# saihv/coloc

Hardware: AMD Instinct MI355X
Metric: Mmatches/s (512-bit Hamming comparisons) at 10k kp/img, describe+match step (higher is better)
Workload: dtype fp4 (+-1) x fp4 -> f32 accumulate, exact integers (matrix pipe); fp32 sample coords

## Files before the change

### coloc_amd/abi.py

```python
import ctypes as C
import os

import numpy as np

_PKG = os.path.dirname(os.path.abspath(__file__))

KP_DTYPE = np.dtype(
    {"names": ["x", "y", "score", "angle", "scale"],
     "formats": ["<i4", "<i4", "u1", "<f4", "u1"],
     "offsets": [0, 4, 8, 12, 16], "itemsize": 20})

CLC_OK, CLC_ERR_BAD_ARG, CLC_ERR_CAPACITY, CLC_ERR_HIP, CLC_ERR_NO_DEVICE, CLC_ERR_STATE = range(6)


class CLCError(RuntimeError):
    def __init__(self, status, msg):
        super().__init__("coloc_hip status %d: %s" % (status, msg))
        self.status = status


class DetectorOptions(C.Structure):
    _fields_ = [("scale_factor", C.c_float), ("scale_levels", C.c_uint8), ("width", C.c_uint32),
                ("height", C.c_uint32), ("maxkp", C.c_uint32), ("thresh", C.c_uint8)]


class MatcherOptions(C.Structure):
    _fields_ = [("distRatio", C.c_float), ("thresh", C.c_int), ("maxkp", C.c_uint32)]


class McShare(C.Structure):
    _fields_ = [("first", C.c_int32), ("second", C.c_int32), ("q_begin", C.c_uint32), ("nq", C.c_uint32), ("out_offset", C.c_uint32)]


class MatchJob(C.Structure):
    _fields_ = [("q_offset", C.c_uint32), ("nq", C.c_uint32), ("t_offset", C.c_uint32), ("nt", C.c_uint32),
                ("out_offset", C.c_uint32), ("threshold", C.c_uint32)]


class PoseJob(C.Structure):
    _fields_ = [("X", C.c_void_p), ("x", C.c_void_p), ("K", C.c_void_p), ("n", C.c_int), ("max_iteration", C.c_int), ("seed", C.c_uint64),
                ("precision", C.c_double), ("refine", C.c_int), ("huber_a", C.c_double),
                ("Rt", C.c_void_p), ("cov", C.c_void_p), ("inlier_mask", C.c_void_p), ("inliers", C.c_void_p),
                ("n_inliers", C.c_int), ("iterations", C.c_int), ("status", C.c_int), ("error_max", C.c_double), ("rmse", C.c_double)]


class CameraK3(C.Structure):
    _fields_ = [("focal", C.c_double), ("ppx", C.c_double), ("ppy", C.c_double), ("k1", C.c_double), ("k2", C.c_double), ("k3", C.c_double)]


class TrackJob(C.Structure):
    _fields_ = [("d_match", C.c_void_p), ("nq", C.c_int), ("d_count", C.c_void_p), ("d_kps", C.c_void_p), ("d_feat", C.c_void_p),
                ("feat_stride", C.c_int), ("cam", CameraK3), ("after_stream", C.c_void_p), ("max_iteration", C.c_int), ("seed", C.c_uint64),
                ("precision", C.c_double), ("refine", C.c_int), ("huber_a", C.c_double),
                ("Rt", C.c_void_p), ("cov", C.c_void_p), ("track_query", C.c_void_p), ("track_map", C.c_void_p), ("inliers", C.c_void_p),
                ("inlier_mask", C.c_void_p), ("n_tracks", C.c_int), ("n_inliers", C.c_int), ("iterations", C.c_int), ("status", C.c_int),
                ("error_max", C.c_double), ("rmse", C.c_double)]


class PairJob(C.Structure):
    _fields_ = [("d_match", C.c_void_p), ("nq", C.c_int), ("nt", C.c_int), ("d_count_a", C.c_void_p), ("d_count_b", C.c_void_p),
                ("d_kps_a", C.c_void_p), ("d_feat_a", C.c_void_p), ("feat_stride_a", C.c_int),
                ("d_kps_b", C.c_void_p), ("d_feat_b", C.c_void_p), ("feat_stride_b", C.c_int),
                ("cam_a", CameraK3), ("cam_b", CameraK3), ("after_stream", C.c_void_p),
                ("img_w", C.c_int), ("img_h", C.c_int), ("max_iteration", C.c_int), ("seed", C.c_uint64), ("precision", C.c_double),
                ("M", C.c_void_p), ("F", C.c_void_p), ("pair_q", C.c_void_p), ("pair_t", C.c_void_p), ("x1", C.c_void_p), ("x2", C.c_void_p),
                ("inliers", C.c_void_p), ("inlier_mask", C.c_void_p),
                ("n_pairs", C.c_int), ("n_inliers", C.c_int), ("iterations", C.c_int), ("status", C.c_int),
                ("error_max", C.c_double), ("min_nfa", C.c_double)]


ABI_VERSION = 4
DESC_CACHE_OFF, DESC_CACHE_VERIFY, DESC_CACHE_TRUST = 0, 1, 2

class DescHandle(C.Structure):
    _fields_ = [("host", C.c_void_p), ("generation", C.c_uint64), ("count", C.c_uint32), ("slot", C.c_uint32)]


class TwoViewJob(C.Structure):
    _fields_ = [("x1", C.c_void_p), ("x2", C.c_void_p), ("K1", C.c_void_p), ("K2", C.c_void_p), ("n", C.c_int), ("img_w", C.c_int), ("img_h", C.c_int),
                ("max_iteration", C.c_int), ("seed", C.c_uint64), ("precision", C.c_double),
                ("E", C.c_void_p), ("F", C.c_void_p), ("inlier_mask", C.c_void_p), ("inliers", C.c_void_p),
                ("n_inliers", C.c_int), ("iterations", C.c_int), ("status", C.c_int), ("error_max", C.c_double), ("min_nfa", C.c_double)]


class InterPoseJob(C.Structure):
    _fields_ = [("tv", TwoViewJob), ("map_index", C.c_void_p), ("map_X", C.c_void_p), ("map_n", C.c_int), ("Rt_source", C.c_void_p), ("huber_a", C.c_double),
                ("d_first_desc", C.c_void_p), ("first_feature", C.c_void_p), ("d_map_desc", C.c_void_p), ("match_threshold", C.c_int),
                ("Rt", C.c_double * 12), ("cov", C.c_double * 36), ("rmse", C.c_double), ("scale", C.c_double),
                ("n_front", C.c_int), ("n_common", C.c_int), ("n_refined", C.c_int), ("stage", C.c_int), ("n_map_matches", C.c_int)]


EXPORTS = [
    "clc_abi_version", "clc_status_string", "clc_ctx_create", "clc_ctx_destroy", "clc_last_error_string",
    "clc_sync", "clc_stream", "clc_pyramid_build", "clc_pyramid_build_dev", "clc_pyramid_level",
    "clc_pyramid_download", "clc_describe", "clc_describe_dev", "clc_keypoints_to_features",
    "clc_match_2nn", "clc_match_2nn_dev", "clc_match_jobs_dev", "clc_set_map", "clc_match_map",
    "clc_pnp_residuals", "clc_pnp_score", "clc_profile_enable", "clc_profile_reset", "clc_profile_read",
    "clc_kernel_name", "clc_detect", "clc_detect_dev", "clc_detect_buffers", "clc_describe_detected_dev",
    "clc_detect_and_describe", "clc_detect_batch_dev", "clc_desc_cache_publish", "clc_desc_cache_clear", "clc_desc_cache_stats", "clc_desc_cache_mode", "clc_desc_handle_live", "clc_detect_and_describe_view", "clc_detect_store_descriptors", "clc_describe_match_pair_dev", "clc_essential_acransac_batch", "clc_inter_pose_batch", "clc_pnp_localize_ac_batch", "clc_match_pairs", "clc_pnp_ransac", "clc_pnp_p3p", "clc_pnp_refine", "clc_pnp_localize", "clc_epipolar_residuals", "clc_epipolar_score", "clc_cov_intersection", "clc_essential_ransac",
    "clc_essential_fivepoint", "clc_describe_batch_dev", "clc_match_map_dev", "clc_k2nn_set_formulation",
    "clc_k2nn_queries_per_block", "clc_k2nn_plan_query", "clc_k2nn_device_info", "clc_pnp_acransac", "clc_pnp_localize_ac", "clc_essential_acransac", "clc_k2nn_clock_check", "clc_ctx_device", "clc_mc_plan", "clc_mc_unique_id",
    "clc_mc_create", "clc_mc_destroy", "clc_mc_last_error_string", "clc_mc_arena", "clc_mc_gather_dev", "clc_mc_match_dev", "clc_mc_virtual_put", "clc_mc_open_peers",
    "clc_mc_gather_enqueue_dev", "clc_mc_match_enqueue_dev", "clc_mc_counts", "clc_mc_set_overlap", "clc_mc_comm_info", "clc_match_jobs_counted_dev",
    "clc_two_view_acransac", "clc_two_view_acransac_batch", "clc_two_view_minimal",
    "clc_match_ratio_2nn", "clc_match_ratio_2nn_dev", "clc_match_ratio_pairs", "clc_match_map_ratio", "clc_match_map_ratio_dev",
    "clc_ratio_matches_to_pairs", "clc_detect_set_selection", "clc_detect_selection",
    "clc_set_map_points", "clc_track_build_dev", "clc_track_localize_dev", "clc_track_localize_batch_dev",
    "clc_pair_build_dev", "clc_pair_filter_dev", "clc_pair_filter_batch_dev",
]
SELECT_FIRST, SELECT_STRONGEST = 0, 1
KERNELS = ["pyramid_kernel", "clatch_kernel", "k2nn_sweep_kernel", "k2nn_merge_kernel", "pnp_residual_kernel",
           "pnp_score_kernel", "detect_kernels"]

_lib = None


def lib_path():
    return os.environ.get("COLOC_HIP_LIB", os.path.join(_PKG, "lib", "libcoloc_hip.so"))


def _share_torch_hip_runtime():
    if os.environ.get("COLOC_HIP_SYSTEM_RUNTIME"):
        return
    import importlib.util
    try:
        spec = importlib.util.find_spec("torch")
    except (ImportError, ValueError):
        spec = None
    if spec is None or not spec.origin:
        return
    cand = os.path.join(os.path.dirname(spec.origin), "lib", "libamdhip64.so")
    if os.path.exists(cand):
        try:
            C.CDLL(cand, mode=C.RTLD_GLOBAL)
        except OSError:
            pass


def load_library():
    global _lib
    if _lib is not None:
        return _lib
    path = lib_path()
    if not os.path.exists(path):
        raise CLCError(-1, "%s not found: build it with `python -c 'import __graft_entry__ as g; g.build()'` "
                           "(hipcc --offload-arch=gfx950); there is no CPU fallback" % path)
    _share_torch_hip_runtime()
    lib = C.CDLL(path)
    got = lib.clc_abi_version() if hasattr(lib, "clc_abi_version") else 0
    if got != ABI_VERSION:
        raise CLCError(-1, "%s reports ABI version %d, this binding needs %d: rebuild it (python -c 'import __graft_entry__ as g; g.build()')"
                       % (path, got, ABI_VERSION))
    lib.clc_status_string.restype = C.c_char_p
    lib.clc_last_error_string.restype = C.c_char_p
    lib.clc_last_error_string.argtypes = [C.c_void_p]
    lib.clc_stream.restype = C.c_void_p
    lib.clc_stream.argtypes = [C.c_void_p]
    lib.clc_ctx_create.argtypes = [C.c_int, C.c_void_p, C.c_void_p, C.POINTER(C.c_void_p)]
    lib.clc_ctx_destroy.argtypes = [C.c_void_p]
    lib.clc_sync.argtypes = [C.c_void_p]
    vp, ci, u32, sz = C.c_void_p, C.c_int, C.c_uint32, C.c_size_t
    lib.clc_pyramid_build.argtypes = [vp, vp, u32, u32]
    lib.clc_pyramid_build_dev.argtypes = [vp, vp, u32, u32, sz, vp]
    lib.clc_pyramid_level.argtypes = [vp, ci, C.POINTER(u32), C.POINTER(u32), C.POINTER(sz), C.POINTER(vp)]
    lib.clc_pyramid_download.argtypes = [vp, ci, vp]
    lib.clc_describe.argtypes = [vp, vp, ci, vp]
    lib.clc_describe_dev.argtypes = [vp, vp, ci, vp, vp]
    lib.clc_describe_batch_dev.argtypes = [vp, ci, vp, C.c_uint32, C.c_uint32, C.c_size_t, vp, vp, vp, vp]
    lib.clc_detect_batch_dev.argtypes = [vp, ci, vp, C.c_uint32, C.c_uint32, C.c_size_t, vp, vp, vp, vp]
    lib.clc_desc_cache_publish.argtypes = [vp, vp, vp, ci, vp]
    lib.clc_desc_handle_live.argtypes = [vp]
    lib.clc_detect_and_describe_view.argtypes = [vp, vp, u32, u32, C.POINTER(vp), C.POINTER(vp), C.POINTER(ci), C.POINTER(ci)]
    lib.clc_detect_store_descriptors.argtypes = [vp, vp, ci, vp]
    lib.clc_desc_cache_clear.argtypes = []
    lib.clc_desc_cache_stats.argtypes = [vp, vp]
    lib.clc_desc_cache_mode.argtypes = [vp, ci]
    lib.clc_essential_acransac_batch.argtypes = [vp, vp, ci]
    lib.clc_inter_pose_batch.argtypes = [vp, vp, ci]
    lib.clc_describe_match_pair_dev.argtypes = [vp, vp, C.c_uint32, C.c_uint32, C.c_size_t, vp, vp, vp, ci, vp, vp]
    lib.clc_pnp_localize_ac_batch.argtypes = [vp, vp, ci]
    lib.clc_keypoints_to_features.argtypes = [vp, ci, vp]
    lib.clc_match_2nn.argtypes = [vp, vp, ci, vp, ci, ci, vp, vp, vp]
    lib.clc_match_2nn_dev.argtypes = [vp, vp, ci, vp, ci, ci, vp, vp]
    lib.clc_match_jobs_dev.argtypes = [vp, vp, vp, ci, vp, vp]
    lib.clc_match_pairs.argtypes = [vp, vp, vp, ci, vp, ci, ci, vp]
    lib.clc_set_map.argtypes = [vp, vp, ci]
    lib.clc_match_map_dev.argtypes = [vp, vp, ci, ci, vp, vp]
    lib.clc_match_map.argtypes = [vp, vp, ci, ci, vp]
    cf = C.c_float
    lib.clc_match_ratio_2nn.argtypes = [vp, vp, ci, vp, ci, cf, vp, vp, vp]
    lib.clc_match_ratio_2nn_dev.argtypes = [vp, vp, ci, vp, ci, cf, vp, vp]
    lib.clc_match_ratio_pairs.argtypes = [vp, vp, vp, ci, vp, vp, ci, cf, vp, vp]
    lib.clc_match_map_ratio.argtypes = [vp, vp, ci, vp, vp, cf, vp, vp]
    lib.clc_match_map_ratio_dev.argtypes = [vp, vp, ci, cf, vp, vp]
    lib.clc_ratio_matches_to_pairs.argtypes = [vp, ci, vp, vp, vp, vp]
    lib.clc_pnp_residuals.argtypes = [vp, vp, ci, vp, vp, ci, vp, vp]
    lib.clc_pnp_score.argtypes = [vp, vp, ci, vp, vp, ci, vp, C.c_double, vp, vp]
    lib.clc_detect.argtypes = [vp, vp, ci, C.POINTER(ci), C.POINTER(ci)]
    lib.clc_detect_dev.argtypes = [vp, vp]
    lib.clc_detect_set_selection.argtypes = [vp, ci]
    lib.clc_detect_selection.argtypes = [vp]
    lib.clc_detect_buffers.argtypes = [vp, C.POINTER(vp), C.POINTER(vp), C.POINTER(vp)]
    lib.clc_describe_detected_dev.argtypes = [vp, vp, vp]
    lib.clc_detect_and_describe.argtypes = [vp, vp, u32, u32, vp, vp, ci, C.POINTER(ci), C.POINTER(ci)]
    lib.clc_pnp_ransac.argtypes = [vp, vp, vp, ci, vp, vp, ci, C.c_uint64, C.c_double, vp, vp, C.POINTER(ci), C.POINTER(C.c_double)]
    lib.clc_pnp_p3p.argtypes = [vp, vp, vp, ci, vp, vp, ci, vp]
    lib.clc_essential_ransac.argtypes = [vp, vp, vp, ci, vp, vp, vp, ci, C.c_uint64, C.c_double, vp, vp, vp, C.POINTER(ci)]
    lib.clc_essential_fivepoint.argtypes = [vp, vp, vp, ci, vp, vp, vp, ci, vp]
    lib.clc_epipolar_residuals.argtypes = [vp, vp, ci, vp, vp, ci, vp]
    lib.clc_epipolar_score.argtypes = [vp, vp, ci, vp, vp, ci, C.c_double, vp, vp]
    lib.clc_pnp_localize.argtypes = [vp, vp, vp, ci, vp, vp, ci, C.c_uint64, C.c_double, C.c_double, vp, vp, vp, C.POINTER(ci),
                                     C.POINTER(C.c_double)]
    lib.clc_pnp_refine.argtypes = [vp, vp, vp, ci, vp, vp, vp, C.c_double, ci, vp, vp, C.POINTER(C.c_double), C.POINTER(ci)]
    lib.clc_profile_enable.argtypes = [vp, ci]
    lib.clc_profile_reset.argtypes = [vp]
    lib.clc_profile_read.argtypes = [vp, ci, C.POINTER(C.c_double), C.POINTER(ci)]
    lib.clc_kernel_name.restype = C.c_char_p
    dp, ip = C.POINTER(C.c_double), C.POINTER(ci)
    lib.clc_pnp_acransac.argtypes = [vp, vp, vp, ci, vp, ci, C.c_uint64, C.c_double, vp, vp, vp, ip, dp, dp, ip]
    lib.clc_pnp_localize_ac.argtypes = [vp, vp, vp, ci, vp, ci, C.c_uint64, C.c_double, C.c_double, vp, vp, vp, vp, ip, dp, dp]
    lib.clc_essential_acransac.argtypes = [vp, vp, vp, ci, vp, vp, ci, ci, ci, C.c_uint64, C.c_double, vp, vp, vp, vp, ip, dp, dp, ip]
    lib.clc_two_view_acransac.argtypes = [vp, ci, vp, vp, ci, vp, vp, ci, ci, ci, C.c_uint64, C.c_double, vp, vp, vp, vp, ip, dp, dp, ip]
    lib.clc_two_view_acransac_batch.argtypes = [vp, ci, vp, ci]
    lib.clc_two_view_minimal.argtypes = [vp, ci, vp, vp, ci, ci, ci, vp, ci, vp]
    lib.clc_mc_plan.argtypes = [vp, ci, ci, ci, ci, vp, ci, ip]
    lib.clc_mc_unique_id.argtypes = [vp]
    lib.clc_mc_create.argtypes = [vp, vp, ci, ci, ci, C.POINTER(vp)]
    lib.clc_mc_destroy.argtypes = [vp]
    lib.clc_mc_last_error_string.argtypes = [vp]
    lib.clc_mc_last_error_string.restype = C.c_char_p
    lib.clc_mc_arena.argtypes = [vp, C.POINTER(vp), ip, ip]
    lib.clc_mc_gather_dev.argtypes = [vp, vp, ci, ci, vp, vp]
    lib.clc_mc_virtual_put.argtypes = [vp, ci, vp, ci, vp]
    lib.clc_mc_open_peers.argtypes = [vp, vp]
    lib.clc_mc_match_dev.argtypes = [vp, ci, vp, ci, vp, ci, ip, vp]
    lib.clc_mc_gather_enqueue_dev.argtypes = [vp, vp, ci, vp, ci, vp]
    lib.clc_mc_match_enqueue_dev.argtypes = [vp, ci, vp, ci, vp, ci, ip, vp]
    lib.clc_mc_counts.argtypes = [vp, vp, vp]
    lib.clc_mc_set_overlap.argtypes = [vp, ci]
    lib.clc_mc_comm_info.argtypes = [vp, ip, ip]
    lib.clc_match_jobs_counted_dev.argtypes = [vp, vp, vp, ci, vp, vp, vp, vp, vp]
    lib.clc_k2nn_clock_check.argtypes = [vp, vp, ci, vp, ci, vp, vp, dp, dp, dp, ip]
    lib.clc_k2nn_set_formulation.argtypes = [vp, ci]
    lib.clc_k2nn_queries_per_block.argtypes = [vp]
    lib.clc_k2nn_plan_query.argtypes = [vp, ci, ci, vp]
    lib.clc_k2nn_device_info.argtypes = [vp, vp, vp]
    lib.clc_set_map_points.argtypes = [vp, vp, ci]
    lib.clc_track_build_dev.argtypes = [vp, vp, vp, vp, vp, vp, vp, vp]
    lib.clc_track_localize_dev.argtypes = [vp, vp]
    lib.clc_track_localize_batch_dev.argtypes = [vp, vp, ci]
    lib.clc_pair_build_dev.argtypes = [vp, vp, vp, vp, vp, vp, vp, vp]
    lib.clc_pair_filter_dev.argtypes = [vp, ci, vp]
    lib.clc_pair_filter_batch_dev.argtypes = [vp, ci, vp, ci]
    _lib = lib
    return lib


def _p(a):
    return None if a is None else C.c_void_p(a.ctypes.data)


def cov_intersection(CA, CB, ca, cb):
    lib = load_library()
    CA = np.ascontiguousarray(CA, dtype=np.float64).reshape(9); CB = np.ascontiguousarray(CB, dtype=np.float64).reshape(9)
    ca = np.ascontiguousarray(ca, dtype=np.float64).reshape(3); cb = np.ascontiguousarray(cb, dtype=np.float64).reshape(3)
    om = C.c_double(); cov = np.zeros(9); pos = np.zeros(3)
    lib.clc_cov_intersection.argtypes = [C.c_void_p] * 4 + [C.POINTER(C.c_double), C.c_void_p, C.c_void_p]
    rc = lib.clc_cov_intersection(_p(CA), _p(CB), _p(ca), _p(cb), C.byref(om), _p(cov), _p(pos))
    if rc != CLC_OK:
        raise CLCError(rc, lib.clc_status_string(rc).decode())
    return om.value, cov.reshape(3, 3), pos


def _xy(xy, n):
    if xy is None:
        return None
    xy = np.ascontiguousarray(xy, dtype=np.float32).reshape(-1, 2)
    if xy.shape[0] != n:
        raise ValueError("positions: %d rows for a set of %d descriptors" % (xy.shape[0], n))
    return xy


def ratio_matches_to_pairs(match, xy_db=None, xy_q=None):
    lib = load_library()
    match = np.ascontiguousarray(match, dtype=np.int32).reshape(-1)
    if xy_db is not None:
        xy_db = np.ascontiguousarray(xy_db, dtype=np.float32).reshape(-1, 2)
    xy_q = _xy(xy_q, match.shape[0])
    out = np.empty((max(match.shape[0], 1), 2), dtype=np.int32)
    n = C.c_int(0)
    rc = lib.clc_ratio_matches_to_pairs(_p(match), match.shape[0], _p(xy_db), _p(xy_q), _p(out), C.byref(n))
    if rc != CLC_OK:
        raise CLCError(rc, "clc_ratio_matches_to_pairs: " + lib.clc_status_string(rc).decode())
    return out[:n.value].copy()


def _two_view_fill(tv, keep, x1, x2, K1, K2, img_wh, max_iteration, seed, precision):
    x1 = np.ascontiguousarray(x1, dtype=np.float64).reshape(-1, 2); x2 = np.ascontiguousarray(x2, dtype=np.float64).reshape(-1, 2)
    K1 = np.ascontiguousarray(K1, dtype=np.float64).reshape(9); K2 = np.ascontiguousarray(K2, dtype=np.float64).reshape(9)
    n = x1.shape[0]
    E, F = np.zeros(9), np.zeros(9)
    mask, inl = np.zeros(max(n, 1), dtype=np.uint8), np.zeros(max(n, 1), dtype=np.int32)
    keep.append((x1, x2, K1, K2, E, F, mask, inl))
    tv.x1, tv.x2, tv.K1, tv.K2, tv.n = x1.ctypes.data, x2.ctypes.data, K1.ctypes.data, K2.ctypes.data, n
    tv.img_w, tv.img_h, tv.max_iteration, tv.seed, tv.precision = int(img_wh[0]), int(img_wh[1]), int(max_iteration), int(seed), float(precision)
    tv.E, tv.F, tv.inlier_mask, tv.inliers = E.ctypes.data, F.ctypes.data, mask.ctypes.data, inl.ctypes.data
    return E, F, mask, inl


def _two_view_result(tv, E, F, mask, inl):
    ok = tv.n_inliers > 0
    return dict(E=E.reshape(3, 3).copy() if ok else None, F=F.reshape(3, 3).copy() if ok else None, mask=mask[:tv.n].astype(bool),
                inliers=inl[:tv.n_inliers].copy(), error_max=tv.error_max, min_nfa=tv.min_nfa, iterations=tv.iterations, status=tv.status)


def essential_acransac_batch(ctxs, problems, max_iteration=256, precision=float("inf")):
    lib = load_library()
    n = len(problems)
    jobs = (TwoViewJob * n)()
    keep, outs = [], []
    for j, (x1, x2, K1, K2, wh, seed) in zip(jobs, problems):
        outs.append(_two_view_fill(j, keep, x1, x2, K1, K2, wh, max_iteration, seed, precision))
    hs = (C.c_void_p * n)(*[c.h for c in ctxs])
    rc = lib.clc_essential_acransac_batch(hs, jobs, n)
    if rc != CLC_OK:
        raise CLCError(rc, lib.clc_status_string(rc).decode())
    return [_two_view_result(j, *o) for j, o in zip(jobs, outs)]


def two_view_acransac_batch(ctxs, model, problems, max_iteration=256, precision=float("inf")):
    lib = load_library()
    n = len(problems)
    jobs = (TwoViewJob * n)()
    keep, outs = [], []
    for j, (x1, x2, K1, K2, wh, seed) in zip(jobs, problems):
        outs.append(_two_view_fill(j, keep, x1, x2, np.eye(3) if K1 is None else K1, np.eye(3) if K2 is None else K2, wh, max_iteration, seed, precision))
    hs = (C.c_void_p * n)(*[c.h for c in ctxs])
    rc = lib.clc_two_view_acransac_batch(hs, ord(model), jobs, n)
    if rc != CLC_OK:
        raise CLCError(rc, lib.clc_status_string(rc).decode())
    return [_two_view_result(j, *o) for j, o in zip(jobs, outs)]


def inter_pose_batch(ctxs, problems, map_X, max_iteration=256, huber_a=16.0):
    lib = load_library()
    n = len(problems)
    jobs = (InterPoseJob * n)()
    map_X = np.ascontiguousarray(map_X, dtype=np.float64).reshape(-1, 3)
    keep, outs = [map_X], []
    for j, p in zip(jobs, problems):
        outs.append(_two_view_fill(j.tv, keep, p["x1"], p["x2"], p["K"], p["K"], p["wh"], max_iteration, p["seed"], float("inf")))
        rs = np.ascontiguousarray(p["Rt_source"], dtype=np.float64).reshape(12)
        keep.append(rs)
        j.map_X, j.map_n, j.Rt_source, j.huber_a = map_X.ctypes.data, int(map_X.shape[0]), rs.ctypes.data, float(huber_a)
        if p.get("d_first_desc") is not None:
            ff = np.ascontiguousarray(p["first_feature"], dtype=np.int32)
            keep.append(ff)
            j.d_first_desc, j.first_feature, j.d_map_desc = int(p["d_first_desc"]), ff.ctypes.data, int(p["d_map_desc"])
            j.match_threshold = int(p.get("match_threshold", 60))
        elif p.get("map_index") is not None:
            mi = np.ascontiguousarray(p["map_index"], dtype=np.int32)
            keep.append(mi)
            j.map_index = mi.ctypes.data
    hs = (C.c_void_p * n)(*[c.h for c in ctxs])
    rc = lib.clc_inter_pose_batch(hs, jobs, n)
    if rc != CLC_OK:
        raise CLCError(rc, lib.clc_status_string(rc).decode())
    res = []
    for j, o in zip(jobs, outs):
        d = _two_view_result(j.tv, *o)
        d.update(Rt=np.array(j.Rt).reshape(3, 4), cov=np.array(j.cov).reshape(6, 6), rmse=j.rmse, scale=j.scale, n_front=j.n_front,
                 n_common=j.n_common, n_refined=j.n_refined, stage=j.stage, n_map_matches=j.n_map_matches)
        res.append(d)
    return res


def mc_plan(counts, world, rank, grain):
    lib = load_library()
    cnt = (C.c_int * len(counts))(*[int(c) for c in counts])
    cap = len(counts) * len(counts) + 2
    out = (McShare * cap)()
    n = C.c_int()
    rc = lib.clc_mc_plan(cnt, len(counts), int(world), int(rank), int(grain), out, cap, C.byref(n))
    if rc != CLC_OK:
        raise CLCError(rc, lib.clc_status_string(rc).decode())
    return [(s.first, s.second, s.q_begin, s.nq, s.out_offset) for s in out[:n.value]]


class MultiCam:

    def __init__(self, ctx, world=1, rank=0, maxkp=10000, unique_id=None):
        self.lib, self.ctx = load_library(), ctx
        h = C.c_void_p()
        idbuf = (C.c_uint8 * 128)(*unique_id) if unique_id is not None else None
        rc = self.lib.clc_mc_create(ctx.h, idbuf, world, rank, maxkp, C.byref(h))
        if rc != CLC_OK:
            raise CLCError(rc, "clc_mc_create: " + self.lib.clc_status_string(rc).decode())
        self.h, self.world, self.maxkp = h, world, maxkp
# ... 46 lines not shown

    def set_overlap(self, on=True):
        self._chk(self.lib.clc_mc_set_overlap(self.h, 1 if on else 0))

    def comm_info(self):
        n, r = C.c_int(), C.c_int()
        self._chk(self.lib.clc_mc_comm_info(self.h, C.byref(n), C.byref(r)))
        return int(n.value), int(r.value)

    def counts(self, stream=None):
        cnt = (C.c_int * self.world)()
        self._chk(self.lib.clc_mc_counts(self.h, cnt, stream))
        return [int(c) for c in cnt]

    def close(self):
        if getattr(self, "h", None):
            self.lib.clc_mc_destroy(self.h)
            self.h = None


def pnp_localize_batch(ctxs, problems, max_iteration=256, seeds=None, precision=float("inf"), refine=True, huber_a=16.0):
    lib = load_library()
    n = len(problems)
    assert len(ctxs) == n
    jobs = (PoseJob * n)()
    keep = []
    for i, (X, x, K) in enumerate(problems):
        X = np.ascontiguousarray(X, dtype=np.float64); x = np.ascontiguousarray(x, dtype=np.float64)
        K = np.ascontiguousarray(K, dtype=np.float64).reshape(9)
        N = X.shape[0]
        Rt, cov = np.zeros(12), np.zeros(36)
        mask, inl = np.zeros(max(N, 1), dtype=np.uint8), np.zeros(max(N, 1), dtype=np.int32)
        keep.append((X, x, K, Rt, cov, mask, inl))
        j = jobs[i]
        j.X, j.x, j.K, j.n = X.ctypes.data, x.ctypes.data, K.ctypes.data, N
        j.max_iteration, j.seed, j.precision = int(max_iteration), int(seeds[i] if seeds is not None else 1), float(precision)
        j.refine, j.huber_a = (1 if refine else 0), float(huber_a)
        j.Rt, j.cov, j.inlier_mask, j.inliers = Rt.ctypes.data, cov.ctypes.data, mask.ctypes.data, inl.ctypes.data
    hs = (C.c_void_p * n)(*[c.h for c in ctxs])
    rc = lib.clc_pnp_localize_ac_batch(hs, jobs, n)
    if rc != CLC_OK:
        raise CLCError(rc, "clc_pnp_localize_ac_batch: " + lib.clc_status_string(rc).decode())
    out = []
    for i in range(n):
        X, x, K, Rt, cov, mask, inl = keep[i]
        j = jobs[i]
        found = j.n_inliers > 0
        out.append(dict(Rt=Rt.reshape(3, 4) if found else None, cov=cov.reshape(6, 6) if (found and refine) else None,
                        mask=mask[:X.shape[0]].astype(bool), inliers=inl[:j.n_inliers].copy(), error_max=j.error_max, rmse=j.rmse,
                        iterations=j.iterations))
    return out


def _track_fill(j, keep, d_match, nq, cam, d_kps=None, d_feat=None, feat_stride=4, d_count=None, after_stream=None, max_iteration=256,
                seed=1, precision=float("inf"), refine=True, huber_a=16.0, outputs=True):
    j.d_match, j.nq, j.d_count, j.d_kps, j.d_feat, j.feat_stride = d_match, int(nq), d_count, d_kps, d_feat, int(feat_stride)
    j.cam = CameraK3(*[float(v) for v in cam])
    j.after_stream = after_stream
    j.max_iteration, j.seed, j.precision, j.refine, j.huber_a = int(max_iteration), int(seed), float(precision), (1 if refine else 0), float(huber_a)
    if not outputs:
        return None
    n = max(int(nq), 1)
    Rt, cov = np.zeros(12), np.zeros(36)
    tq, tm, inl, mask = np.zeros(n, dtype=np.int32), np.zeros(n, dtype=np.int32), np.zeros(n, dtype=np.int32), np.zeros(n, dtype=np.uint8)
    keep.append((Rt, cov, tq, tm, inl, mask))
    j.Rt, j.cov, j.track_query, j.track_map, j.inliers, j.inlier_mask = (a.ctypes.data for a in (Rt, cov, tq, tm, inl, mask))
    return Rt, cov, tq, tm, inl, mask


def _track_result(j, Rt, cov, tq, tm, inl, mask):
    found = j.n_inliers > 0
    nt = max(min(j.n_tracks, len(tq)), 0)
    return dict(Rt=Rt.reshape(3, 4).copy() if found else None, cov=cov.reshape(6, 6).copy() if (found and j.refine) else None,
                n_tracks=j.n_tracks, track_query=tq[:nt].copy(), track_map=tm[:nt].copy(), inliers=inl[:j.n_inliers].copy(),
                mask=mask[:nt].astype(bool), error_max=j.error_max, rmse=j.rmse, iterations=j.iterations, status=j.status)


def track_localize_batch_dev(ctxs, jobs):
    lib = load_library()
    n = len(jobs)
    assert len(ctxs) == n
    arr = (TrackJob * n)()
    keep = []
    outs = [_track_fill(arr[i], keep, **jobs[i]) for i in range(n)]
    hs = (C.c_void_p * n)(*[c.h for c in ctxs])
    rc = lib.clc_track_localize_batch_dev(hs, arr, n)
    if rc != CLC_OK:
        raise CLCError(rc, "clc_track_localize_batch_dev: %s: %s" % (lib.clc_status_string(rc).decode(), lib.clc_last_error_string(ctxs[0].h).decode()))
    return [_track_result(arr[i], *outs[i]) for i in range(n)]


def _pair_fill(j, keep, d_match, nq, nt, cam_a, cam_b, d_kps_a=None, d_feat_a=None, feat_stride_a=4, d_kps_b=None, d_feat_b=None,
               feat_stride_b=4, d_count_a=None, d_count_b=None, after_stream=None, img_wh=(0, 0), max_iteration=256, seed=1,
               precision=float("inf"), outputs=True):
    j.d_match, j.nq, j.nt, j.d_count_a, j.d_count_b = d_match, int(nq), int(nt), d_count_a, d_count_b
    j.d_kps_a, j.d_feat_a, j.feat_stride_a = d_kps_a, d_feat_a, int(feat_stride_a)
    j.d_kps_b, j.d_feat_b, j.feat_stride_b = d_kps_b, d_feat_b, int(feat_stride_b)
    j.cam_a, j.cam_b = CameraK3(*[float(v) for v in cam_a]), CameraK3(*[float(v) for v in cam_b])
    j.after_stream = after_stream
    j.img_w, j.img_h, j.max_iteration, j.seed, j.precision = int(img_wh[0]), int(img_wh[1]), int(max_iteration), int(seed), float(precision)
    if not outputs:
        return None
    n = max(int(nq), 1)
    M, F, x1, x2 = np.zeros(9), np.zeros(9), np.zeros((n, 2)), np.zeros((n, 2))
    pq, pt, inl, mask = np.zeros(n, dtype=np.int32), np.zeros(n, dtype=np.int32), np.zeros(n, dtype=np.int32), np.zeros(n, dtype=np.uint8)
    keep.append((M, F, pq, pt, x1, x2, inl, mask))
    j.M, j.F, j.pair_q, j.pair_t, j.x1, j.x2, j.inliers, j.inlier_mask = (a.ctypes.data for a in (M, F, pq, pt, x1, x2, inl, mask))
    return M, F, pq, pt, x1, x2, inl, mask


def _pair_result(j, M, F, pq, pt, x1, x2, inl, mask):
    found = j.n_inliers > 0
    n = max(min(j.n_pairs, len(pq)), 0)
    return dict(M=M.reshape(3, 3).copy() if found else None, F=F.reshape(3, 3).copy() if found else None, n_pairs=j.n_pairs,
                pair_q=pq[:n].copy(), pair_t=pt[:n].copy(), x1=x1[:n].copy(), x2=x2[:n].copy(), inliers=inl[:j.n_inliers].copy(),
                mask=mask[:n].astype(bool), error_max=j.error_max, min_nfa=j.min_nfa, iterations=j.iterations, status=j.status)


def pair_filter_batch_dev(ctxs, model, jobs):
    lib = load_library()
    n = len(jobs)
    assert len(ctxs) == n
    arr = (PairJob * n)()
    keep = []
    outs = [_pair_fill(arr[i], keep, **jobs[i]) for i in range(n)]
    hs = (C.c_void_p * n)(*[c.h for c in ctxs])
    rc = lib.clc_pair_filter_batch_dev(hs, ord(model), arr, n)
    if rc != CLC_OK:
        raise CLCError(rc, "clc_pair_filter_batch_dev: %s: %s" % (lib.clc_status_string(rc).decode(), lib.clc_last_error_string(ctxs[0].h).decode()))
    return [_pair_result(arr[i], *outs[i]) for i in range(n)]


def desc_handle_live(handle):
    return bool(load_library().clc_desc_handle_live(C.byref(handle)))


def desc_cache_stats():
    lib = load_library()
    h, m = C.c_ulonglong(), C.c_ulonglong()
    lib.clc_desc_cache_stats(C.byref(h), C.byref(m))
    return int(h.value), int(m.value)


def keypoints_to_features(kps):
    lib = load_library()
    kps = np.ascontiguousarray(kps, dtype=KP_DTYPE)
    out = np.zeros((len(kps), 4), dtype=np.float32)
    rc = lib.clc_keypoints_to_features(_p(kps), len(kps), _p(out))
    if rc != CLC_OK:
        raise CLCError(rc, lib.clc_status_string(rc).decode())
    return out


class Context:

    def __init__(self, device=0, width=640, height=480, maxkp=10000, scale_factor=1.2, scale_levels=8,
                 fast_thresh=40, match_thresh=60, detector=True, matcher=True):
        self.lib = load_library()
        self.dopts = DetectorOptions(scale_factor, scale_levels, width, height, maxkp, fast_thresh)
        self.mopts = MatcherOptions(0.8, match_thresh, maxkp)
        h = C.c_void_p()
        rc = self.lib.clc_ctx_create(device, C.byref(self.dopts) if detector else None,
                                     C.byref(self.mopts) if matcher else None, C.byref(h))
        if rc != CLC_OK:
            raise CLCError(rc, "clc_ctx_create: " + self.lib.clc_status_string(rc).decode())
        self.h = h
        self.device = device

    def _chk(self, rc):
        if rc != CLC_OK:
            raise CLCError(rc, "%s: %s" % (self.lib.clc_status_string(rc).decode(),
                                           self.lib.clc_last_error_string(self.h).decode()))

    def close(self):
        if getattr(self, "h", None):
            self.lib.clc_ctx_destroy(self.h)
            self.h = None

    def __del__(self):
        try:
            self.close()
        except Exception:
            pass

    def sync(self):
        self._chk(self.lib.clc_sync(self.h))

    @property
    def stream(self):
        return self.lib.clc_stream(self.h)

    def profile_enable(self, on=True, only=None):
        v = 1 if on else 0
        if on and only:
            v = 0
            for name in only:
                v |= 1 << (KERNELS.index(name) + 1)
        self._chk(self.lib.clc_profile_enable(self.h, v))

    def profile_reset(self):
        self._chk(self.lib.clc_profile_reset(self.h))

    def profile_read(self):
        out = {}
        for k, name in enumerate(KERNELS):
            ms, cnt = C.c_double(), C.c_int()
            self._chk(self.lib.clc_profile_read(self.h, k, C.byref(ms), C.byref(cnt)))
            out[name] = (ms.value, cnt.value)
        return out

    def pyramid_build(self, img):
        img = np.ascontiguousarray(img, dtype=np.uint8)
        self._chk(self.lib.clc_pyramid_build(self.h, _p(img), img.shape[1], img.shape[0]))

    def pyramid_build_dev(self, d_ptr, width, height, pitch, stream=None):
        self._chk(self.lib.clc_pyramid_build_dev(self.h, d_ptr, width, height, pitch, stream))

    def pyramid_level(self, level):
        w, h, p, d = C.c_uint32(), C.c_uint32(), C.c_size_t(), C.c_void_p()
        self._chk(self.lib.clc_pyramid_level(self.h, level, C.byref(w), C.byref(h), C.byref(p), C.byref(d)))
        return w.value, h.value, p.value, d.value

    def pyramid_download(self, level):
        w, h, _, _ = self.pyramid_level(level)
        out = np.zeros((h, w), dtype=np.uint8)
        self._chk(self.lib.clc_pyramid_download(self.h, level, _p(out)))
        return out

    def detect(self, capacity=None):
        cap = int(capacity if capacity is not None else self.dopts.maxkp)
        kps = np.zeros(cap, dtype=KP_DTYPE)
        n, found = C.c_int(), C.c_int()
        self._chk(self.lib.clc_detect(self.h, _p(kps), cap, C.byref(n), C.byref(found)))
        return kps[:n.value], found.value

    def set_keypoint_selection(self, mode):
        self._chk(self.lib.clc_detect_set_selection(self.h, int(mode)))

    @property
    def keypoint_selection(self):
        return self.lib.clc_detect_selection(self.h)

    def detect_dev(self, stream=None):
        self._chk(self.lib.clc_detect_dev(self.h, stream))

    def detect_buffers(self):
        k, c, d = C.c_void_p(), C.c_void_p(), C.c_void_p()
        self._chk(self.lib.clc_detect_buffers(self.h, C.byref(k), C.byref(c), C.byref(d)))
        return k.value, c.value, d.value

    def describe_detected_dev(self, d_desc=None, stream=None):
        self._chk(self.lib.clc_describe_detected_dev(self.h, d_desc, stream))

    def detect_and_describe(self, img, capacity=None):
        img = np.ascontiguousarray(img, dtype=np.uint8)
        cap = int(capacity if capacity is not None else self.dopts.maxkp)
        kps = np.zeros(cap, dtype=KP_DTYPE)
        desc = np.zeros((cap, 64), dtype=np.uint8)
        n, found = C.c_int(), C.c_int()
        self._chk(self.lib.clc_detect_and_describe(self.h, _p(img), img.shape[1], img.shape[0], _p(kps), _p(desc), cap,
                                                   C.byref(n), C.byref(found)))
        return kps[:n.value], desc[:n.value], found.value

    def detect_and_describe_published(self, img):
        img = np.ascontiguousarray(img, dtype=np.uint8)
        pk, pd, n, found = C.c_void_p(), C.c_void_p(), C.c_int(), C.c_int()
        self._chk(self.lib.clc_detect_and_describe_view(self.h, _p(img), img.shape[1], img.shape[0], C.byref(pk), C.byref(pd), C.byref(n), C.byref(found)))
        kps = np.zeros(n.value, dtype=KP_DTYPE)
        if n.value:
            C.memmove(_p(kps), pk, n.value * 20)
        desc = np.zeros((n.value, 64), dtype=np.uint8)
        handle = DescHandle()
        self._chk(self.lib.clc_detect_store_descriptors(self.h, _p(desc) if n.value else None, n.value, C.byref(handle)))
        return kps, desc, found.value, handle

    def detect_batch_dev(self, d_imgs, width, height, pitch, d_kps, d_counts, d_desc=None, stream=None):
        n = len(d_imgs)
        imgs = (C.c_void_p * n)(*d_imgs)
        kps = (C.c_void_p * n)(*d_kps)
        cnt = (C.c_void_p * n)(*d_counts)
        out = (C.c_void_p * n)(*d_desc) if d_desc is not None else None
        self._chk(self.lib.clc_detect_batch_dev(self.h, n, imgs, width, height, pitch, kps, cnt, out, stream))

    def describe_match_pair_dev(self, d_imgs, width, height, pitch, d_kps, counts, d_desc, threshold, d_match, stream=None):
        imgs = (C.c_void_p * 2)(*d_imgs)
        kps = (C.c_void_p * 2)(*d_kps)
        cnt = (C.c_int * 2)(*[int(c) for c in counts])
        out = (C.c_void_p * 2)(*d_desc)
        self._chk(self.lib.clc_describe_match_pair_dev(self.h, imgs, width, height, pitch, kps, cnt, out, int(threshold), d_match, stream))

    def desc_cache_mode(self, mode):
        self._chk(self.lib.clc_desc_cache_mode(self.h, {"off": DESC_CACHE_OFF, "verify": DESC_CACHE_VERIFY, "trust": DESC_CACHE_TRUST}[mode]))

    def desc_cache_publish(self, h_desc, d_src=None):
        assert h_desc.dtype == np.uint8 and h_desc.flags["C_CONTIGUOUS"]
        handle = DescHandle()
        self._chk(self.lib.clc_desc_cache_publish(self.h, d_src, _p(h_desc), int(h_desc.shape[0]), C.byref(handle)))
        return handle

    def describe(self, kps):
        kps = np.ascontiguousarray(kps, dtype=KP_DTYPE)
        desc = np.zeros((len(kps), 64), dtype=np.uint8)
        self._chk(self.lib.clc_describe(self.h, _p(kps), len(kps), _p(desc)))
        return desc

    def describe_dev(self, d_kps, n, d_desc, stream=None):
        self._chk(self.lib.clc_describe_dev(self.h, d_kps, n, d_desc, stream))

    def describe_batch_dev(self, d_imgs, width, height, pitch, d_kps, counts, d_desc, stream=None):
        n = len(d_imgs)
        imgs = (C.c_void_p * n)(*d_imgs)
        kps = (C.c_void_p * n)(*d_kps)
        cnt = (C.c_int * n)(*counts)
        out = (C.c_void_p * n)(*d_desc)
        self._chk(self.lib.clc_describe_batch_dev(self.h, n, imgs, width, height, pitch, kps, cnt, out, stream))

    def set_k2nn_formulation(self, name):
        self._chk(self.lib.clc_k2nn_set_formulation(self.h, {"matrix": 0, "popcount": 1}[name]))

    @property
    def k2nn_queries_per_block(self):
        return int(self.lib.clc_k2nn_queries_per_block(self.h))

    def k2nn_device_info(self):
        info = (C.c_int32 * 8)()
        us = (C.c_float * 4)()
        self._chk(self.lib.clc_k2nn_device_info(self.h, info, us))
        d = dict(zip(("xcds", "cus", "default_target_blocks", "bias_a", "bias_b", "bias_source", "kernel_xcds", "target_blocks_env"), [int(v) for v in info]))
        d["bias_source"] = ("default", "CLC_K2NN_BIAS", "probe")[d["bias_source"]]
        d["probe_us"] = dict(zip(("295:264", "311:256", "326:249", "326:233"), [float(v) for v in us]))
        return d

    def k2nn_plan_query(self, nq, nt):
        info = (C.c_int32 * 8)()
        self._chk(self.lib.clc_k2nn_plan_query(self.h, int(nq), int(nt), info))
        return dict(zip(("qblocks", "splits", "t_per_split", "atomic_merge", "bias_a_tiles", "bias_b_tiles", "queries_per_block", "target_blocks"),
                        [int(v) for v in info]))

    def k2nn_clock_check(self, d_q, nq, d_t, nt, d_match, stream=None):
        med, lo, hi, n = C.c_double(), C.c_double(), C.c_double(), C.c_int()
        self._chk(self.lib.clc_k2nn_clock_check(self.h, d_q, nq, d_t, nt, d_match, stream, C.byref(med), C.byref(lo), C.byref(hi), C.byref(n)))
        return med.value, lo.value, hi.value, n.value

    def match_2nn(self, Q, T, threshold=40, want_dist=False):
        Q = np.ascontiguousarray(Q, dtype=np.uint8).reshape(-1, 64)
        T = np.ascontiguousarray(T, dtype=np.uint8).reshape(-1, 64)
        m = np.full(Q.shape[0], -2, dtype=np.int32)
        b = np.zeros(Q.shape[0], dtype=np.uint16) if want_dist else None
        s = np.zeros(Q.shape[0], dtype=np.uint16) if want_dist else None
        self._chk(self.lib.clc_match_2nn(self.h, _p(Q), Q.shape[0], _p(T), T.shape[0], int(threshold), _p(m), _p(b), _p(s)))
        return (m, b, s) if want_dist else m

    def match_2nn_dev(self, d_q, nq, d_t, nt, threshold, d_match, stream=None):
        self._chk(self.lib.clc_match_2nn_dev(self.h, d_q, nq, d_t, nt, int(threshold), d_match, stream))

    def match_jobs_dev(self, d_desc_base, jobs, d_match, stream=None):
        arr = (MatchJob * len(jobs))(*[MatchJob(*j) for j in jobs])
        self._chk(self.lib.clc_match_jobs_dev(self.h, d_desc_base, arr, len(jobs), d_match, stream))

    def match_jobs_counted_dev(self, d_desc_base, jobs, d_cnt_q, d_cnt_t, q_row0, d_match, stream=None):
        n = len(jobs)
        arr = (MatchJob * n)(*[MatchJob(*j) for j in jobs])
        cq = (C.c_void_p * n)(*d_cnt_q)
        ct = (C.c_void_p * n)(*d_cnt_t)
        r0 = (C.c_uint32 * n)(*q_row0)
        self._chk(self.lib.clc_match_jobs_counted_dev(self.h, d_desc_base, arr, n, cq, ct, r0, d_match, stream))

    def match_pairs(self, descs, pairs, threshold=40):
        descs = [np.ascontiguousarray(d, dtype=np.uint8).reshape(-1, 64) for d in descs]
        counts = (C.c_int * len(descs))(*[d.shape[0] for d in descs])
        dptr = (C.c_void_p * len(descs))(*[d.ctypes.data for d in descs])
        flat = (C.c_int * (2 * len(pairs)))(*[v for p in pairs for v in p])
        outs = [np.full(descs[a].shape[0], -2, dtype=np.int32) for a, _ in pairs]
        optr = (C.c_void_p * len(pairs))(*[o.ctypes.data for o in outs])
        self._chk(self.lib.clc_match_pairs(self.h, dptr, counts, len(descs), flat, len(pairs), int(threshold), optr))
        return outs

    def match_ratio(self, Q, T, ratio=0.8, want_dist=False):
        Q = np.ascontiguousarray(Q, dtype=np.uint8).reshape(-1, 64)
        T = np.ascontiguousarray(T, dtype=np.uint8).reshape(-1, 64)
        m = np.full(Q.shape[0], -2, dtype=np.int32)
        b = np.zeros(Q.shape[0], dtype=np.uint16) if want_dist else None
        s = np.zeros(Q.shape[0], dtype=np.uint16) if want_dist else None
        self._chk(self.lib.clc_match_ratio_2nn(self.h, _p(Q), Q.shape[0], _p(T), T.shape[0], float(ratio), _p(m), _p(b), _p(s)))
        return (m, b, s) if want_dist else m

    def match_ratio_dev(self, d_q, nq, d_t, nt, ratio, d_match, stream=None):
        self._chk(self.lib.clc_match_ratio_2nn_dev(self.h, d_q, nq, d_t, nt, float(ratio), d_match, stream))

    def match_ratio_pairs(self, descs, pairs, ratio=0.8, xys=None):
        descs = [np.ascontiguousarray(d, dtype=np.uint8).reshape(-1, 64) for d in descs]
        ncams = len(descs)
        counts = (C.c_int * ncams)(*[d.shape[0] for d in descs])
        dptr = (C.c_void_p * ncams)(*[d.ctypes.data for d in descs])
        xyp = None
        if xys is not None:
            xys = [_xy(x, d.shape[0]) for x, d in zip(xys, descs)]
            xyp = (C.c_void_p * ncams)(*[None if x is None else x.ctypes.data for x in xys])
        flat = (C.c_int * max(2 * len(pairs), 1))(*[v for p in pairs for v in p])
        outs = [np.empty((max(descs[b].shape[0] if 0 <= b < ncams else 0, 1), 2), dtype=np.int32) for _, b in pairs]
        optr = (C.c_void_p * max(len(pairs), 1))(*[o.ctypes.data for o in outs])
        n = (C.c_int * max(len(pairs), 1))()
        self._chk(self.lib.clc_match_ratio_pairs(self.h, dptr, counts, ncams, xyp, flat, len(pairs), float(ratio), optr, n))
        return [o[:n[p]].copy() for p, o in enumerate(outs)]

    def match_map_ratio(self, Q, ratio=0.8, xy_map=None, xy_q=None):
        Q = np.ascontiguousarray(Q, dtype=np.uint8).reshape(-1, 64)
        xy_map = None if xy_map is None else np.ascontiguousarray(xy_map, dtype=np.float32).reshape(-1, 2)
        xy_q = _xy(xy_q, Q.shape[0])
        out = np.empty((max(Q.shape[0], 1), 2), dtype=np.int32)
        n = C.c_int(0)
        self._chk(self.lib.clc_match_map_ratio(self.h, _p(Q), Q.shape[0], _p(xy_map), _p(xy_q), float(ratio), _p(out), C.byref(n)))
        return out[:n.value].copy()

    def match_map_ratio_dev(self, d_q, nq, ratio, d_match, stream=None):
        self._chk(self.lib.clc_match_map_ratio_dev(self.h, d_q, nq, float(ratio), d_match, stream))

    def set_map(self, desc):
        desc = np.ascontiguousarray(desc, dtype=np.uint8).reshape(-1, 64)
        self._chk(self.lib.clc_set_map(self.h, _p(desc), desc.shape[0]))

    def set_map_points(self, X):
        X = np.ascontiguousarray(X, dtype=np.float64).reshape(-1, 3)
        self._chk(self.lib.clc_set_map_points(self.h, _p(X) if X.shape[0] else None, X.shape[0]))

    def track_build_dev(self, d_X, d_x, d_query, d_map, d_n, stream=None, **job):
        j = TrackJob()
        _track_fill(j, None, outputs=False, **job)
        self._chk(self.lib.clc_track_build_dev(self.h, C.byref(j), d_X, d_x, d_query, d_map, d_n, stream))

    def track_localize_dev(self, **job):
        j = TrackJob()
        keep = []
        out = _track_fill(j, keep, **job)
        self._chk(self.lib.clc_track_localize_dev(self.h, C.byref(j)))
        return _track_result(j, *out)

    def pair_build_dev(self, d_x1, d_x2, d_pair_q, d_pair_t, d_n, stream=None, **job):
        j = PairJob()
        _pair_fill(j, None, outputs=False, **job)
        self._chk(self.lib.clc_pair_build_dev(self.h, C.byref(j), d_x1, d_x2, d_pair_q, d_pair_t, d_n, stream))

    def pair_filter_dev(self, model, **job):
        j = PairJob()
        keep = []
        out = _pair_fill(j, keep, **job)
        self._chk(self.lib.clc_pair_filter_dev(self.h, ord(model), C.byref(j)))
        return _pair_result(j, *out)

    def match_map_dev(self, d_q, nq, threshold, d_match, stream=None):
        self._chk(self.lib.clc_match_map_dev(self.h, d_q, nq, int(threshold), d_match, stream))

    def match_map(self, Q, threshold=60):
        Q = np.ascontiguousarray(Q, dtype=np.uint8).reshape(-1, 64)
        m = np.full(Q.shape[0], -2, dtype=np.int32)
        self._chk(self.lib.clc_match_map(self.h, _p(Q), Q.shape[0], int(threshold), _p(m)))
        return m

    def pnp_residuals(self, Rt, X, x, K):
        Rt = np.ascontiguousarray(Rt, dtype=np.float64).reshape(-1, 12)
        X = np.ascontiguousarray(X, dtype=np.float64).reshape(-1, 3)
        x = np.ascontiguousarray(x, dtype=np.float64).reshape(-1, 2)
        K = np.ascontiguousarray(K, dtype=np.float64).reshape(9)
        err = np.zeros((Rt.shape[0], X.shape[0]), dtype=np.float64)
        self._chk(self.lib.clc_pnp_residuals(self.h, _p(Rt), Rt.shape[0], _p(X), _p(x), X.shape[0], _p(K), _p(err)))
        return err

    def pnp_ransac(self, X, x, K, samples=None, n_samples=256, seed=1, thr2=16.0):
        X = np.ascontiguousarray(X, dtype=np.float64).reshape(-1, 3)
        x = np.ascontiguousarray(x, dtype=np.float64).reshape(-1, 2)
        K = np.ascontiguousarray(K, dtype=np.float64).reshape(9)
        if samples is not None:
            samples = np.ascontiguousarray(samples, dtype=np.int32).reshape(-1, 3)
            n_samples = samples.shape[0]
        Rt = np.zeros(12, dtype=np.float64)
        mask = np.zeros(X.shape[0], dtype=np.uint8)
        n, cost = C.c_int(), C.c_double()
        self._chk(self.lib.clc_pnp_ransac(self.h, _p(X), _p(x), X.shape[0], _p(K), _p(samples), int(n_samples), int(seed),
                                          float(thr2), _p(Rt), _p(mask), C.byref(n), C.byref(cost)))
        return (Rt.reshape(3, 4) if n.value > 0 else None), mask.astype(bool), cost.value

    def essential_ransac(self, x1, x2, K1, K2, samples=None, n_samples=256, seed=1, thr2=4.0):
        x1 = np.ascontiguousarray(x1, dtype=np.float64).reshape(-1, 2)
        x2 = np.ascontiguousarray(x2, dtype=np.float64).reshape(-1, 2)
        K1 = np.ascontiguousarray(K1, dtype=np.float64).reshape(9); K2 = np.ascontiguousarray(K2, dtype=np.float64).reshape(9)
        if samples is not None:
            samples = np.ascontiguousarray(samples, dtype=np.int32).reshape(-1, 5)
            n_samples = samples.shape[0]
        E = np.zeros(9); F = np.zeros(9)
        mask = np.zeros(x1.shape[0], dtype=np.uint8)
# ... 142 lines not shown
```

### coloc_amd/csrc/capi_core.hip

```cpp
#include "clc_ctx.h"
#include "desc_cache.h"

#include <chrono>
#include <cmath>
#include <cstdio>
#include <cstdlib>
#include <cstring>
#include <new>

using namespace clc;

namespace clc {
void prof_mark(Profiler* prof, int kernel, bool begin, hipStream_t stream)
{
    if (!prof || !prof->on || !((prof->mask >> kernel) & 1u)) return;
    if (begin) {
        Profiler::Pair p;
        p.a = prof->get(); p.b = prof->get(); p.kernel = kernel; p.stream = stream; p.open = true;
        if (p.a) (void)hipEventRecord(p.a, stream);
        prof->pending.push_back(p);
    } else {
        for (size_t i = prof->pending.size(); i-- > 0;) {
            Profiler::Pair& p = prof->pending[i];
            if (p.open && p.kernel == kernel && p.stream == stream) {
                if (p.b) (void)hipEventRecord(p.b, stream);
                p.open = false;
                break;
            }
        }
    }
}

int fail(clc_ctx* ctx, int code, const char* what, hipError_t e)
{
    if (ctx) {
        char buf[512];
        if (e != hipSuccess) snprintf(buf, sizeof buf, "%s: %s (%s)", what, hipGetErrorName(e), hipGetErrorString(e));
        else snprintf(buf, sizeof buf, "%s", what);
        ctx->err = buf;
        if (code == CLC_ERR_HIP) ctx->partial_dirty = true;
    }
    return code;
}


int ensure_partial(clc_ctx* ctx, size_t elems)
{
    if (elems <= ctx->partial_cap) return CLC_OK;
    CLC_HIP(ctx, hipStreamSynchronize(ctx->stream));
    if (ctx->d_partial) CLC_HIP(ctx, hipFree(ctx->d_partial));
    ctx->d_partial = nullptr;
    ctx->partial_cap = 0;
    size_t cap = elems + elems / 4;
    CLC_HIP(ctx, hipMalloc((void**)&ctx->d_partial, cap * sizeof(uint2)));
    CLC_HIP(ctx, hipMemsetAsync(ctx->d_partial, 0xFF, cap * sizeof(uint2), ctx->stream));
    CLC_HIP(ctx, hipStreamSynchronize(ctx->stream));
    ctx->partial_cap = cap;
    return CLC_OK;
}

int ensure_pnp(clc_ctx* ctx, size_t doubles)
{
    if (doubles <= ctx->pnp_cap) return CLC_OK;
    CLC_HIP(ctx, hipStreamSynchronize(ctx->stream));
    if (ctx->d_pnp) CLC_HIP(ctx, hipFree(ctx->d_pnp));
    ctx->d_pnp = nullptr;
    ctx->pnp_cap = 0;
    const size_t cap = doubles + doubles / 2;
    CLC_HIP(ctx, hipMalloc((void**)&ctx->d_pnp, cap * sizeof(double)));
    ctx->pnp_cap = cap;
    return CLC_OK;
}

int ensure_pinned(clc_ctx* ctx, size_t bytes)
{
    if (bytes <= ctx->pin_cap) return CLC_OK;
    CLC_HIP(ctx, hipStreamSynchronize(ctx->stream));
    if (ctx->h_pin) CLC_HIP(ctx, hipHostFree(ctx->h_pin));
    ctx->h_pin = nullptr; ctx->pin_cap = 0;
    const size_t cap = bytes + bytes / 2;
    CLC_HIP(ctx, hipHostMalloc(&ctx->h_pin, cap, hipHostMallocDefault));
    ctx->pin_cap = cap;
    return CLC_OK;
}

int ensure_slots(clc_ctx* ctx, int n, hipStream_t st)
{
    if (n <= ctx->arena_slots) return CLC_OK;
    CLC_HIP(ctx, hipStreamSynchronize(ctx->stream));
    if (st != ctx->stream) CLC_HIP(ctx, hipStreamSynchronize(st));
    uint8_t *arena = nullptr, *score = nullptr;
    uint64_t* kpmask = nullptr;
    uint32_t* tcount = nullptr;
    hipError_t e = hipMalloc((void**)&arena, ctx->arena_bytes * (size_t)n);
    if (e == hipSuccess) e = hipMalloc((void**)&score, ctx->arena_bytes * (size_t)n);
    if (e == hipSuccess) e = hipMalloc((void**)&kpmask, (size_t)n * ctx->n_tiles * 16 * sizeof(uint64_t));
    if (e == hipSuccess) e = hipMalloc((void**)&tcount, (size_t)n * ctx->n_tiles * sizeof(uint32_t));
    if (e == hipSuccess) e = hipMemsetAsync(arena, 0, ctx->arena_bytes * (size_t)n, st);
    if (e == hipSuccess) e = hipStreamSynchronize(st);
    if (e != hipSuccess) {
        (void)hipFree(arena); (void)hipFree(score); (void)hipFree(kpmask); (void)hipFree(tcount);
        return fail(ctx, CLC_ERR_HIP, "growing the pyramid arena", e);
    }
    ctx->pyramid_valid = false;
    ctx->detected = false;
    (void)hipFree(ctx->d_arena); (void)hipFree(ctx->d_score); (void)hipFree(ctx->d_kpmask); (void)hipFree(ctx->d_tcount);
    ctx->d_arena = arena; ctx->d_score = score; ctx->d_kpmask = kpmask; ctx->d_tcount = tcount;
    ctx->arena_slots = n;
    return CLC_OK;
}


int ensure_results(clc_ctx* ctx, size_t bytes)
{
    if (bytes <= ctx->res_cap) return CLC_OK;
    CLC_HIP(ctx, hipStreamSynchronize(ctx->stream));
    if (ctx->h_res) CLC_HIP(ctx, hipHostFree(ctx->h_res));
    ctx->h_res = nullptr; ctx->res_cap = 0;
    CLC_HIP(ctx, hipHostMalloc((void**)&ctx->h_res, bytes, hipHostMallocDefault));
    ctx->res_cap = bytes;
    return CLC_OK;
}

}

namespace {

uint32_t align_up(uint32_t v, uint32_t a) { return (v + a - 1) / a * a; }

void plan_pyramid(const clc_detector_opts& o, PyramidDesc& pd, size_t& bytes)
{
    pd.levels = o.scale_levels;
    float f = 1.0f;
    uint32_t off = 0, blk = 0;
    for (int i = 0; i < pd.levels; ++i) {
        if (i) f *= o.scale_factor;
        const uint32_t w = i ? (uint32_t)((float)o.width / f + 0.5f) : o.width;
        const uint32_t h = i ? (uint32_t)((float)o.height / f + 0.5f) : o.height;
        pd.f[i] = f;
        pd.lv[i].w = w;
        pd.lv[i].h = h;
        pd.lv[i].pitch = align_up(w ? w : 1, 64);
        pd.lv[i].offset = off;
        off += align_up(pd.lv[i].pitch * (h ? h : 1), 256);
        pd.blk_begin[i] = blk;
        if (i) blk += (pd.lv[i].pitch / 4 * h + 255) / 256;
    }
    for (int i = pd.levels; i <= CLC_MAX_LEVELS; ++i) pd.blk_begin[i] = blk;
    bytes = off + 256;
}

int cache_mode_default()
{
    const char* v = getenv("CLC_DESC_CACHE");
    if (!v || !v[0]) return CLC_DESC_CACHE_VERIFY;
    if (v[0] == '0' || v[0] == 'o' || v[0] == 'O') return CLC_DESC_CACHE_OFF;
    if (v[0] == 't' || v[0] == 'T' || v[0] == '2') return CLC_DESC_CACHE_TRUST;
    return CLC_DESC_CACHE_VERIFY;
}


__global__ __launch_bounds__(256) void frontend_mirror_kernel(const uint32_t* __restrict__ d_kps, const uint4* __restrict__ d_desc,
                                                              const uint32_t* __restrict__ d_count, uint32_t* __restrict__ h_kps,
                                                              uint4* __restrict__ h_desc, uint32_t* __restrict__ h_count)
{
    const uint32_t n = d_count[0];
    const uint32_t i = blockIdx.x * 256u + threadIdx.x;
    if (i == 0u) { h_count[0] = n; h_count[1] = d_count[1]; }
    if (i < n * 4u) h_desc[i] = d_desc[i];
    if (i < n * 4u) h_kps[i] = d_kps[i];
    if (i < n) h_kps[n * 4u + i] = d_kps[n * 4u + i];
}

static int ensure_stage(clc_ctx* ctx)
{
    if (ctx->h_stage) return CLC_OK;
    const size_t img = ((size_t)ctx->dopts.width * ctx->dopts.height + 255) & ~(size_t)255;
    const size_t kps = ((size_t)ctx->dopts.maxkp * sizeof(clc_keypoint) + 255) & ~(size_t)255;
    const size_t desc = (size_t)ctx->dopts.maxkp * CLC_DESC_BYTES;
    ctx->stage_img = 0; ctx->stage_kps = img; ctx->stage_desc = img + kps; ctx->stage_cnt = img + kps + desc;
    CLC_HIP(ctx, hipHostMalloc((void**)&ctx->h_stage, img + kps + desc + 256, hipHostMallocDefault));
    memset(ctx->h_stage + ctx->stage_cnt, 0, 256);
    return CLC_OK;
}

}

extern "C" {

int clc_abi_version(void) { return CLC_ABI_VERSION; }

const char* clc_status_string(int status)
{
    switch (status) {
        case CLC_OK: return "ok";
        case CLC_ERR_BAD_ARG: return "bad argument";
        case CLC_ERR_CAPACITY: return "capacity exceeded";
        case CLC_ERR_HIP: return "HIP runtime error";
        case CLC_ERR_NO_DEVICE: return "no usable device";
        case CLC_ERR_STATE: return "invalid call order";
        default: return "unknown status";
    }
}

const char* clc_last_error_string(const clc_ctx* ctx) { return ctx ? ctx->err.c_str() : "null context"; }

int clc_ctx_create(int device_id, const clc_detector_opts* dopts, const clc_matcher_opts* mopts, clc_ctx** out_ctx)
{
    if (!out_ctx) return CLC_ERR_BAD_ARG;
    *out_ctx = nullptr;
    if (dopts) {
        if (dopts->scale_levels < 1 || dopts->scale_levels > CLC_MAX_LEVELS || dopts->width < 8 || dopts->height < 8 ||
            !(dopts->scale_factor > 1.0f) || dopts->maxkp == 0)
            return CLC_ERR_BAD_ARG;
        if (dopts->width > CLC_DETECT_MAX_WIDTH) {
            fprintf(stderr, "coloc_hip: DetectorOptions.width %u exceeds CLC_DETECT_MAX_WIDTH %d (the GPU detector keeps a row's pre-test bits in LDS)\n",
                    dopts->width, CLC_DETECT_MAX_WIDTH);
            return CLC_ERR_CAPACITY;
        }
    }
    if (mopts && mopts->maxkp == 0) return CLC_ERR_BAD_ARG;
    int ndev = 0;
    if (hipGetDeviceCount(&ndev) != hipSuccess || device_id < 0 || device_id >= ndev) return CLC_ERR_NO_DEVICE;
    clc_ctx* ctx = new (std::nothrow) clc_ctx;
    if (!ctx) return CLC_ERR_HIP;
    ctx->device = device_id;
#define CREATE_HIP(call)                                     \
    do {                                                     \
        hipError_t e__ = (call);                             \
        if (e__ != hipSuccess) {                             \
            fprintf(stderr, "coloc_hip: %s failed: %s\n", #call, hipGetErrorString(e__)); \
            clc_ctx_destroy(ctx);                            \
            return CLC_ERR_HIP;                              \
        }                                                    \
    } while (0)
    CREATE_HIP(hipSetDevice(device_id));
    CREATE_HIP(hipStreamCreateWithFlags(&ctx->stream, hipStreamNonBlocking));
    {
        int v = 0;
        if (hipDeviceGetAttribute(&v, hipDeviceAttributeMultiprocessorCount, device_id) == hipSuccess && v > 0) ctx->k2dev.n_cu = (uint32_t)v;
        if (hipDeviceGetAttribute(&v, hipDeviceAttributeNumberOfXccs, device_id) == hipSuccess && v > 0) ctx->k2dev.n_xcd = (uint32_t)v;
    }
    if (const char* e = getenv("CLC_K2NN_TARGET_BLOCKS")) {
        const int v = atoi(e);
        if (v > 0) ctx->target_blocks = v;
    }
    if (const char* e = getenv("CLC_K2NN_XCD_MAP")) ctx->xcd_map = atoi(e) != 0;
    ctx->cache_mode = cache_mode_default();
    if (const char* e = getenv("CLC_K2NN_BIAS")) {
        int a = 0, b = 0;
        if (sscanf(e, "%d,%d", &a, &b) == 2 && a >= 0 && b >= 0 && a < 1024 && b < 1024) { ctx->bias_a = a; ctx->bias_b = b; ctx->bias_source = 1; }
    }
    if (const char* e = getenv("CLC_K2NN_FORMULATION"))
        ctx->formulation = (e[0] == 'p' || e[0] == '1') ? K2NN_POPCOUNT : K2NN_MATRIX;
    if (dopts) {
        ctx->has_det = true;
        ctx->dopts = *dopts;
        plan_pyramid(*dopts, ctx->pd, ctx->arena_bytes);
        CREATE_HIP(hipMalloc((void**)&ctx->d_arena, ctx->arena_bytes));
        CREATE_HIP(hipMemsetAsync(ctx->d_arena, 0, ctx->arena_bytes, ctx->stream));
        CREATE_HIP(hipMalloc((void**)&ctx->d_kps, (size_t)dopts->maxkp * sizeof(clc_keypoint)));
        CREATE_HIP(hipMalloc((void**)&ctx->d_desc, (size_t)dopts->maxkp * CLC_DESC_BYTES));
        CREATE_HIP(hipMalloc((void**)&ctx->d_score, ctx->arena_bytes));
        ctx->n_tiles = detect_total_tiles(ctx->pd);
        CREATE_HIP(hipMalloc((void**)&ctx->d_kpmask, (size_t)ctx->n_tiles * 16 * sizeof(uint64_t)));
        CREATE_HIP(hipMalloc((void**)&ctx->d_tcount, (size_t)ctx->n_tiles * sizeof(uint32_t)));
        {
            const size_t sel_bytes = (size_t)CLC_MAX_BATCH * detect_select_words(ctx->pd) * sizeof(uint32_t);
            CREATE_HIP(hipMalloc((void**)&ctx->d_select, sel_bytes));
            CREATE_HIP(hipMemsetAsync(ctx->d_select, 0, sel_bytes, ctx->stream));
        }
        CREATE_HIP(hipMalloc((void**)&ctx->d_count, 4 * sizeof(uint32_t)));
        CREATE_HIP(hipMemsetAsync(ctx->d_count, 0, 4 * sizeof(uint32_t), ctx->stream));
    }
    if (mopts) {
        ctx->has_mat = true;
        ctx->mopts = *mopts;
        const size_t cap = (size_t)mopts->maxkp;
        CREATE_HIP(hipMalloc((void**)&ctx->d_q, cap * CLC_DESC_BYTES));
        CREATE_HIP(hipMalloc((void**)&ctx->d_t, cap * CLC_DESC_BYTES));
        CREATE_HIP(hipMalloc((void**)&ctx->d_m, cap * CLC_DESC_BYTES));
        CREATE_HIP(hipMalloc((void**)&ctx->d_match, cap * sizeof(int32_t)));
        CREATE_HIP(hipMalloc((void**)&ctx->d_best, cap * sizeof(uint16_t)));
        CREATE_HIP(hipMalloc((void**)&ctx->d_second, cap * sizeof(uint16_t)));
    }
    {
        const size_t cap = dopts || mopts ? (size_t)(mopts ? mopts->maxkp : dopts->maxkp) : 16384;
        const size_t elems = ((cap + 63) & ~(size_t)63) * 8 + 4096;
        CREATE_HIP(hipMalloc((void**)&ctx->d_partial, elems * sizeof(uint2)));
        CREATE_HIP(hipMemsetAsync(ctx->d_partial, 0xFF, elems * sizeof(uint2), ctx->stream));
        ctx->partial_cap = elems;
    }
    CREATE_HIP(hipStreamSynchronize(ctx->stream));
#undef CREATE_HIP
    if (ctx->bias_source == 0) k2nn_probe_bias(ctx);
    *out_ctx = ctx;
    return CLC_OK;
}

int clc_ctx_destroy(clc_ctx* ctx)
{
    if (!ctx) return CLC_ERR_BAD_ARG;
    (void)hipSetDevice(ctx->device);
    if (ctx->stream) (void)hipStreamSynchronize(ctx->stream);
    void* bufs[] = { ctx->d_arena, ctx->d_kps, ctx->d_desc, ctx->d_score, ctx->d_kpmask, ctx->d_tcount, ctx->d_select, ctx->d_count, ctx->d_q, ctx->d_t, ctx->d_m, ctx->d_match,
                     ctx->d_best, ctx->d_second, ctx->d_partial, ctx->d_pnp, ctx->d_pairs, ctx->d_map_X, ctx->d_trk, ctx->d_pair };
    for (void* b : bufs)
        if (b) (void)hipFree(b);
    if (ctx->h_trk) (void)hipHostFree(ctx->h_trk);
    if (ctx->h_pair) (void)hipHostFree(ctx->h_pair);
    if (ctx->ev_track) (void)hipEventDestroy(ctx->ev_track);
    desc_drop_owner(ctx);
    if (ctx->h_pin) (void)hipHostFree(ctx->h_pin);
    if (ctx->h_stage) (void)hipHostFree(ctx->h_stage);
    if (ctx->h_res) (void)hipHostFree(ctx->h_res);
    if (ctx->ev_group) (void)hipEventDestroy(ctx->ev_group);
    if (ctx->stream) (void)hipStreamDestroy(ctx->stream);
    delete ctx;
    return CLC_OK;
}

int clc_sync(clc_ctx* ctx)
{
    if (!ctx) return CLC_ERR_BAD_ARG;
    CLC_HIP(ctx, hipSetDevice(ctx->device));
    CLC_HIP(ctx, hipStreamSynchronize(ctx->stream));
    return CLC_OK;
}

void* clc_stream(clc_ctx* ctx) { return ctx ? (void*)ctx->stream : nullptr; }

int clc_ctx_device(const clc_ctx* ctx) { return ctx ? ctx->device : -1; }

int clc_profile_enable(clc_ctx* ctx, int on)
{
    if (!ctx) return CLC_ERR_BAD_ARG;
    (void)hipSetDevice(ctx->device);
    if (!on) ctx->prof.drain();
    ctx->prof.on = on != 0;
    ctx->prof.mask = (on == 1 || on == 0) ? 0xFFFFFFFFu : ((unsigned)on >> 1);
    return CLC_OK;
}

int clc_profile_reset(clc_ctx* ctx)
{
    if (!ctx) return CLC_ERR_BAD_ARG;
    (void)hipSetDevice(ctx->device);
    ctx->prof.drain();
    for (int k = 0; k < CLC_KERNEL_COUNT; ++k) { ctx->prof.total_ms[k] = 0.0; ctx->prof.launches[k] = 0; }
    return CLC_OK;
}

int clc_profile_read(clc_ctx* ctx, int kernel, double* total_ms, int* launches)
{
    if (!ctx || kernel < 0 || kernel >= CLC_KERNEL_COUNT) return CLC_ERR_BAD_ARG;
    (void)hipSetDevice(ctx->device);
    ctx->prof.drain();
    if (total_ms) *total_ms = ctx->prof.total_ms[kernel];
    if (launches) *launches = ctx->prof.launches[kernel];
    return CLC_OK;
}

const char* clc_kernel_name(int kernel)
{
    static const char* names[CLC_KERNEL_COUNT] = { "pyramid_kernel", "clatch_kernel", "k2nn_sweep_kernel",
                                                    "k2nn_merge_kernel", "pnp_residual_kernel", "pnp_score_kernel",
                                                    "detect_kernels" };
    return (kernel >= 0 && kernel < CLC_KERNEL_COUNT) ? names[kernel] : "?";
}


int clc_pyramid_build_dev(clc_ctx* ctx, const void* d_img, uint32_t width, uint32_t height, size_t pitch, void* stream)
{
    if (!ctx || !d_img) return fail(ctx, CLC_ERR_BAD_ARG, "pyramid_build: null argument");
    if (!ctx->has_det) return fail(ctx, CLC_ERR_STATE, "pyramid_build: context created without detector options");
    if (width != ctx->dopts.width || height != ctx->dopts.height || pitch < width)
        return fail(ctx, CLC_ERR_BAD_ARG, "pyramid_build: image size differs from DetectorOptions width/height");
    CLC_HIP(ctx, hipSetDevice(ctx->device));
    hipStream_t st = pick(ctx, stream);
    if (pitch > 0xFFFFFFFFull) return fail(ctx, CLC_ERR_BAD_ARG, "pyramid_build: pitch too large");
    CLC_HIP(ctx, launch_pyramid(ctx->pd, ctx->d_arena, (const uint8_t*)d_img, (uint32_t)pitch, st, &ctx->prof));
    ctx->pyramid_valid = true;
    return CLC_OK;
}

int clc_pyramid_build(clc_ctx* ctx, const uint8_t* h_img, uint32_t width, uint32_t height)
{
    if (!ctx || !h_img) return fail(ctx, CLC_ERR_BAD_ARG, "pyramid_build: null argument");
    if (!ctx->has_det) return fail(ctx, CLC_ERR_STATE, "pyramid_build: context created without detector options");
    if (width != ctx->dopts.width || height != ctx->dopts.height)
        return fail(ctx, CLC_ERR_BAD_ARG, "pyramid_build: image size differs from DetectorOptions width/height");
    CLC_HIP(ctx, hipSetDevice(ctx->device));
    const LevelDesc& L0 = ctx->pd.lv[0];
    CLC_HIP(ctx, hipMemcpy2DAsync(ctx->d_arena + L0.offset, L0.pitch, h_img, width, width, height,
                                  hipMemcpyHostToDevice, ctx->stream));
    CLC_HIP(ctx, launch_pyramid(ctx->pd, ctx->d_arena, ctx->d_arena + L0.offset, L0.pitch, ctx->stream, &ctx->prof));
    CLC_HIP(ctx, hipStreamSynchronize(ctx->stream));
    ctx->pyramid_valid = true;
    return CLC_OK;
}

int clc_pyramid_level(const clc_ctx* ctx, int level, uint32_t* w, uint32_t* h, size_t* pitch, const void** d_ptr)
{
    if (!ctx || !ctx->has_det || level < 0 || level >= ctx->pd.levels) return CLC_ERR_BAD_ARG;
    const LevelDesc& L = ctx->pd.lv[level];
    if (w) *w = L.w;
    if (h) *h = L.h;
    if (pitch) *pitch = L.pitch;
    if (d_ptr) *d_ptr = ctx->d_arena + L.offset;
    return CLC_OK;
}

int clc_pyramid_download(clc_ctx* ctx, int level, uint8_t* h_out)
{
    if (!ctx || !h_out) return fail(ctx, CLC_ERR_BAD_ARG, "pyramid_download: null argument");
    if (!ctx->has_det || level < 0 || level >= ctx->pd.levels) return fail(ctx, CLC_ERR_BAD_ARG, "pyramid_download: bad level");
    if (!ctx->pyramid_valid) return fail(ctx, CLC_ERR_STATE, "pyramid_download before pyramid_build");
    CLC_HIP(ctx, hipSetDevice(ctx->device));
    const LevelDesc& L = ctx->pd.lv[level];
    CLC_HIP(ctx, hipMemcpy2DAsync(h_out, L.w, ctx->d_arena + L.offset, L.pitch, L.w, L.h, hipMemcpyDeviceToHost, ctx->stream));
    CLC_HIP(ctx, hipStreamSynchronize(ctx->stream));
    return CLC_OK;
}


static uint32_t* count_ptr(clc_ctx* ctx) { return ctx->d_count; }
static uint32_t* select_ptr(clc_ctx* ctx) { return ctx->selection == CLC_SELECT_STRONGEST ? ctx->d_select : nullptr; }

int clc_detect_set_selection(clc_ctx* ctx, int mode)
{
    if (!ctx) return CLC_ERR_BAD_ARG;
    if (mode != CLC_SELECT_FIRST && mode != CLC_SELECT_STRONGEST) return fail(ctx, CLC_ERR_BAD_ARG, "detect_set_selection: unknown mode");
    if (!ctx->has_det) return fail(ctx, CLC_ERR_STATE, "detect_set_selection: context created without detector options");
    ctx->selection = mode;
    return CLC_OK;
}

int clc_detect_selection(const clc_ctx* ctx) { return ctx ? ctx->selection : -1; }

int clc_detect_dev(clc_ctx* ctx, void* stream)
{
    if (!ctx) return CLC_ERR_BAD_ARG;
    if (!ctx->has_det) return fail(ctx, CLC_ERR_STATE, "detect: context created without detector options");
    if (!ctx->pyramid_valid) return fail(ctx, CLC_ERR_STATE, "detect before pyramid_build");
    if (ctx->rows_at == ROWS_OWN && ctx->own_rows < 0) ctx->rows_at = ROWS_NONE;
    CLC_HIP(ctx, hipSetDevice(ctx->device));
    clc_keypoint* kps[1] = { ctx->d_kps };
    uint32_t* cnt[1] = { ctx->d_count };
    CLC_HIP(ctx, launch_detect(ctx->pd, ctx->d_arena, ctx->arena_bytes, 1, ctx->d_score, ctx->d_kpmask, ctx->d_tcount, ctx->dopts.thresh,
                               ctx->dopts.maxkp, kps, cnt, pick(ctx, stream), &ctx->prof, select_ptr(ctx), &ctx->select_dirty));
    ctx->detected = true;
    return CLC_OK;
}

int clc_detect_batch_dev(clc_ctx* ctx, int n_images, const void* const* d_imgs, uint32_t width, uint32_t height, size_t pitch,
// ... 260 lines not shown
```

### coloc_amd/csrc/capi_match.hip

```cpp
#include "clc_ctx.h"
#include "desc_cache.h"

#include <algorithm>
#include <cmath>
#include <cstdio>
#include <cstdlib>
#include <cstring>
#include <mutex>
#include <string>
#include <vector>

using namespace clc;

namespace clc {

int default_target_blocks(int formulation, const K2nnDevice& dev) { return (int)((formulation == K2NN_POPCOUNT ? 10u : 3u) * dev.n_cu); }

int run_jobs(clc_ctx* ctx, std::vector<K2nnJobDev>& jobs, hipStream_t st, bool probe)
{
    const int target = ctx->target_blocks > 0 ? ctx->target_blocks : default_target_blocks(ctx->formulation, ctx->k2dev);
    const K2nnPlan plan = k2nn_plan(jobs.data(), (int)jobs.size(), target, ctx->xcd_map, ctx->formulation, ctx->bias_a, ctx->bias_b, ctx->k2dev);
    const int rc = ensure_partial(ctx, plan.partial_elems);
    if (rc != CLC_OK) return rc;
    if (!plan.atomic_merge) ctx->partial_dirty = true;
    else if (ctx->partial_dirty) {
        CLC_HIP(ctx, hipMemsetAsync(ctx->d_partial, 0xFF, ctx->partial_cap * sizeof(uint2), st));
        ctx->partial_dirty = false;
    }
    const hipError_t e = launch_k2nn(jobs.data(), (int)jobs.size(), ctx->d_partial, st, probe ? nullptr : &ctx->prof, ctx->formulation, nullptr, probe);
    if (e != hipSuccess) { ctx->partial_dirty = true; return fail(ctx, CLC_ERR_HIP, "launch_k2nn", e); }
    return CLC_OK;
}


__global__ void k2nn_probe_fill_kernel(uint32_t* p, const size_t n, const uint32_t salt)
{
    const size_t i = (size_t)blockIdx.x * blockDim.x + threadIdx.x;
    if (i >= n) return;
    uint32_t x = (uint32_t)i * 2654435761u + salt;
    x ^= x >> 16; x *= 0x7feb352du; x ^= x >> 15; x *= 0x846ca68bu; x ^= x >> 16;
    p[i] = x;
}
struct K2nnProbeCache { std::mutex mu; bool done[64] = {}; int a[64] = {}, b[64] = {}; float us[64][4] = {}; };
static K2nnProbeCache& probe_cache() { static K2nnProbeCache c; return c; }
static constexpr int kProbeCand[4][2] = { { 295, 264 }, { 311, 256 }, { 326, 249 }, { 326, 233 } };

void k2nn_probe_bias(clc_ctx* ctx)
{
    const int N = 10000;
    if (!ctx->has_mat || ctx->mopts.maxkp < (uint32_t)N || ctx->formulation == K2NN_POPCOUNT || ctx->device < 0 || ctx->device >= 64) return;
    if (ctx->k2dev.n_xcd != kK2nnXcds || ctx->target_blocks > 0) return;
    if (const char* e = getenv("CLC_K2NN_PROBE")) if (e[0] == '0') return;
    K2nnProbeCache& pc = probe_cache();
    std::lock_guard<std::mutex> lk(pc.mu);
    const int d = ctx->device;
    if (!pc.done[d]) {
        pc.done[d] = true; pc.a[d] = ctx->bias_a; pc.b[d] = ctx->bias_b;
        hipEvent_t e0 = nullptr, e1 = nullptr;
        if (hipEventCreate(&e0) != hipSuccess || hipEventCreate(&e1) != hipSuccess) { if (e0) (void)hipEventDestroy(e0); return; }
        const size_t words = (size_t)N * CLC_DESC_BYTES / 4;
        hipLaunchKernelGGL(k2nn_probe_fill_kernel, dim3((unsigned)((words + 255) / 256)), dim3(256), 0, ctx->stream, (uint32_t*)ctx->d_q, words, 1u);
        hipLaunchKernelGGL(k2nn_probe_fill_kernel, dim3((unsigned)((words + 255) / 256)), dim3(256), 0, ctx->stream, (uint32_t*)ctx->d_t, words, 2u);
        std::vector<K2nnJobDev> jobs(1);
        auto sweep = [&](const int a, const int b, const int reps) -> bool {
            const int sa = ctx->bias_a, sb = ctx->bias_b;
            ctx->bias_a = a; ctx->bias_b = b;
            bool ok = true;
            for (int r = 0; r < reps && ok; ++r) {
                jobs[0] = K2nnJobDev{};
                jobs[0].q = (const uint4*)ctx->d_q; jobs[0].t = (const uint4*)ctx->d_t; jobs[0].out = ctx->d_match;
                jobs[0].nq = (uint32_t)N; jobs[0].nt = (uint32_t)N; jobs[0].thr = 40u;
                ok = run_jobs(ctx, jobs, ctx->stream, true) == CLC_OK;
            }
            ctx->bias_a = sa; ctx->bias_b = sb;
            return ok;
        };
        bool ok = sweep(ctx->bias_a, ctx->bias_b, 160);
        float best = 0.f; int best_i = -1;
        for (int pass = 0; pass < 2 && ok; ++pass)
            for (int c = 0; c < 4 && ok; ++c) {
                ok = hipEventRecord(e0, ctx->stream) == hipSuccess && sweep(kProbeCand[c][0], kProbeCand[c][1], 40) && hipEventRecord(e1, ctx->stream) == hipSuccess &&
                     hipEventSynchronize(e1) == hipSuccess;
                float ms = 0.f;
                if (ok && hipEventElapsedTime(&ms, e0, e1) == hipSuccess) {
                    const float us = ms * 1000.f / 40.f;
                    if (pc.us[d][c] == 0.f || us < pc.us[d][c]) pc.us[d][c] = us;
                }
            }
        if (ok)
            for (int c = 0; c < 4; ++c) if (pc.us[d][c] > 0.f && (best_i < 0 || pc.us[d][c] < best)) { best = pc.us[d][c]; best_i = c; }
        if (ok && best_i >= 0 && pc.us[d][2] > 0.f && best < 0.99f * pc.us[d][2]) { pc.a[d] = kProbeCand[best_i][0]; pc.b[d] = kProbeCand[best_i][1]; }
        (void)hipStreamSynchronize(ctx->stream);
        (void)hipEventDestroy(e0); (void)hipEventDestroy(e1);
        if (!ok) { ctx->partial_dirty = true; for (int c = 0; c < 4; ++c) pc.us[d][c] = 0.f; }
    }
    ctx->bias_a = pc.a[d]; ctx->bias_b = pc.b[d];
    for (int c = 0; c < 4; ++c) ctx->bias_probe_us[c] = pc.us[d][c];
    if (pc.us[d][0] > 0.f) ctx->bias_source = 2;
}


}

extern "C" {

int clc_k2nn_set_formulation(clc_ctx* ctx, int formulation)
{
    if (!ctx || (formulation != CLC_K2NN_MATRIX && formulation != CLC_K2NN_POPCOUNT))
        return fail(ctx, CLC_ERR_BAD_ARG, "k2nn_set_formulation: bad argument");
    ctx->formulation = formulation == CLC_K2NN_POPCOUNT ? K2NN_POPCOUNT : K2NN_MATRIX;
    return CLC_OK;
}

int clc_k2nn_queries_per_block(const clc_ctx* ctx)
{
    return k2nn_queries_per_block(ctx ? ctx->formulation : K2NN_MATRIX);
}

int clc_k2nn_plan_query(const clc_ctx* ctx, int nq, int nt, int32_t* info)
{
    if (!ctx || nq < 0 || nt < 0 || !info) return CLC_ERR_BAD_ARG;
    K2nnJobDev jb{};
    jb.nq = (uint32_t)nq; jb.nt = (uint32_t)nt;
    const int target = ctx->target_blocks > 0 ? ctx->target_blocks : default_target_blocks(ctx->formulation, ctx->k2dev);
    const K2nnPlan plan = k2nn_plan(&jb, 1, target, ctx->xcd_map, ctx->formulation, ctx->bias_a, ctx->bias_b, ctx->k2dev);
    info[0] = (int32_t)jb.qblocks; info[1] = (int32_t)jb.splits; info[2] = (int32_t)jb.t_per_split; info[3] = plan.atomic_merge ? 1 : 0;
    info[4] = (int32_t)jb.bias_a; info[5] = (int32_t)jb.bias_b; info[6] = k2nn_queries_per_block(ctx->formulation); info[7] = target;
    return CLC_OK;
}

int clc_k2nn_device_info(const clc_ctx* ctx, int32_t* info, float* probe_us)
{
    if (!ctx || !info) return CLC_ERR_BAD_ARG;
    info[0] = (int32_t)ctx->k2dev.n_xcd; info[1] = (int32_t)ctx->k2dev.n_cu; info[2] = default_target_blocks(ctx->formulation, ctx->k2dev);
    info[3] = ctx->bias_a; info[4] = ctx->bias_b; info[5] = ctx->bias_source; info[6] = (int32_t)kK2nnXcds; info[7] = ctx->target_blocks;
    if (probe_us) for (int c = 0; c < 4; ++c) probe_us[c] = ctx->bias_probe_us[c];
    return CLC_OK;
}

int clc_k2nn_clock_check(clc_ctx* ctx, const void* d_q, int nq, const void* d_t, int nt, int32_t* d_match, void* stream,
                         double* ghz_median, double* ghz_min, double* ghz_max, int* workgroups)
{
    if (!ctx || nq <= 0 || nt <= 0 || !d_q || !d_t || !d_match) return fail(ctx, CLC_ERR_BAD_ARG, "k2nn_clock_check: bad argument");
    if (((uintptr_t)d_q & 15u) || ((uintptr_t)d_t & 15u)) return fail(ctx, CLC_ERR_BAD_ARG, "k2nn_clock_check: misaligned device pointer");
    if (ctx->formulation == K2NN_POPCOUNT) return fail(ctx, CLC_ERR_STATE, "k2nn_clock_check: matrix formulation only");
    CLC_HIP(ctx, hipSetDevice(ctx->device));
    hipStream_t st = pick(ctx, stream);
    std::vector<K2nnJobDev> jobs(1);
    jobs[0] = K2nnJobDev{};
    jobs[0].q = (const uint4*)d_q; jobs[0].t = (const uint4*)d_t; jobs[0].out = d_match;
    jobs[0].nq = (uint32_t)nq; jobs[0].nt = (uint32_t)nt; jobs[0].thr = 40u;
    const int target = ctx->target_blocks > 0 ? ctx->target_blocks : default_target_blocks(ctx->formulation, ctx->k2dev);
    const K2nnPlan plan = k2nn_plan(jobs.data(), 1, target, ctx->xcd_map, ctx->formulation, ctx->bias_a, ctx->bias_b, ctx->k2dev);
    if (!plan.atomic_merge) return fail(ctx, CLC_ERR_CAPACITY, "k2nn_clock_check: train set too large");
    int rc = ensure_partial(ctx, plan.partial_elems);
    if (rc != CLC_OK) return rc;
    if (ctx->partial_dirty) {
        CLC_HIP(ctx, hipMemsetAsync(ctx->d_partial, 0xFF, ctx->partial_cap * sizeof(uint2), st));
        ctx->partial_dirty = false;
    }
    const size_t nwg = (size_t)((jobs[0].qblocks + 7u) & ~7u) * jobs[0].splits;
    uint64_t* d_stamps = nullptr;
    CLC_HIP(ctx, hipMalloc((void**)&d_stamps, nwg * 8 * sizeof(uint64_t)));
    std::vector<uint64_t> h(nwg * 8);
    hipError_t e = hipMemsetAsync(d_stamps, 0, nwg * 8 * sizeof(uint64_t), st);
    if (e == hipSuccess) e = launch_k2nn(jobs.data(), 1, ctx->d_partial, st, nullptr, ctx->formulation, d_stamps);
    if (e == hipSuccess) e = hipMemcpyAsync(h.data(), d_stamps, nwg * 8 * sizeof(uint64_t), hipMemcpyDeviceToHost, st);
    if (e == hipSuccess) e = hipStreamSynchronize(st);
    (void)hipFree(d_stamps);
    if (e != hipSuccess) return fail(ctx, CLC_ERR_HIP, "k2nn_clock_check", e);
    if (const char* dump = getenv("CLC_K2NN_STAMP_DUMP")) {
        if (FILE* f = fopen(dump, "wb")) { fwrite(h.data(), sizeof(uint64_t), h.size(), f); fclose(f); }
    }
    std::vector<double> ghz;
    for (size_t w = 0; w < nwg; ++w) {
        const uint64_t dc = h[8 * w + 2] - h[8 * w], dr = h[8 * w + 3] - h[8 * w + 1];
        if (dr > 20) ghz.push_back((double)dc / (double)dr * 0.1);
    }
    if (ghz.empty()) return fail(ctx, CLC_ERR_STATE, "k2nn_clock_check: sweep too short to stamp");
    std::sort(ghz.begin(), ghz.end());
    if (ghz_median) *ghz_median = ghz[ghz.size() / 2];
    if (ghz_min) *ghz_min = ghz.front();
    if (ghz_max) *ghz_max = ghz.back();
    if (workgroups) *workgroups = (int)ghz.size();
    return CLC_OK;
}

}

namespace {

struct Rule {
    uint32_t rule = K2NN_RULE_K2NN;
    uint32_t thr = 0;
    float    r2 = 0.f;
    void apply(K2nnJobDev& jb) const { jb.rule = rule; jb.thr = thr; jb.r2 = r2; }
};
Rule k2nn_rule(int threshold) { Rule r; r.thr = (uint32_t)(uint8_t)threshold; return r; }
Rule ratio_rule(float ratio) { Rule r; r.rule = K2NN_RULE_RATIO; r.r2 = ratio * ratio; return r; }
bool bad_ratio(float ratio) { return !(ratio > 0.f) || !std::isfinite(ratio); }

int match_dev(clc_ctx* ctx, const void* d_q, int nq, const void* d_t, int nt, const Rule& rule, int32_t* d_match, void* stream)
{
    if (nq == 0) return CLC_OK;
    CLC_HIP(ctx, hipSetDevice(ctx->device));
    std::vector<K2nnJobDev> jobs(1);
    jobs[0] = K2nnJobDev{};
    jobs[0].q = (const uint4*)d_q;
    jobs[0].t = (const uint4*)d_t;
    jobs[0].out = d_match;
    jobs[0].nq = (uint32_t)nq;
    jobs[0].nt = (uint32_t)nt;
    rule.apply(jobs[0]);
    return run_jobs(ctx, jobs, pick(ctx, stream));
}

}

extern "C" {

int clc_match_2nn_dev(clc_ctx* ctx, const void* d_q, int nq, const void* d_t, int nt, int threshold,
                      int32_t* d_match, void* stream)
{
    if (!ctx || nq < 0 || nt < 0 || (nq > 0 && (!d_q || !d_match)) || (nt > 0 && !d_t))
        return fail(ctx, CLC_ERR_BAD_ARG, "match_2nn: bad argument");
    if (((uintptr_t)d_q & 15u) || ((uintptr_t)d_t & 15u) || ((uintptr_t)d_match & 3u))
        return fail(ctx, CLC_ERR_BAD_ARG, "match_2nn: device pointers must be 16-byte aligned");
    return match_dev(ctx, d_q, nq, d_t, nt, k2nn_rule(threshold), d_match, stream);
}

int clc_match_ratio_2nn_dev(clc_ctx* ctx, const void* d_q, int nq, const void* d_t, int nt, float ratio, int32_t* d_match, void* stream)
{
    if (!ctx || nq < 0 || nt < 0 || (nq > 0 && (!d_q || !d_match)) || (nt > 0 && !d_t) || bad_ratio(ratio))
        return fail(ctx, CLC_ERR_BAD_ARG, "match_ratio_2nn: bad argument");
    if (((uintptr_t)d_q & 15u) || ((uintptr_t)d_t & 15u) || ((uintptr_t)d_match & 3u))
        return fail(ctx, CLC_ERR_BAD_ARG, "match_ratio_2nn: device pointers must be 16-byte aligned");
    return match_dev(ctx, d_q, nq, d_t, nt, ratio_rule(ratio), d_match, stream);
}

int clc_describe_match_pair_dev(clc_ctx* ctx, const void* const* d_imgs, uint32_t width, uint32_t height, size_t pitch,
                                const clc_keypoint* const* d_kps, const int* counts, void* const* d_desc, int threshold,
                                int32_t* d_match, void* stream)
{
    if (ctx) rows_leave(ctx);
    if (!ctx || !d_imgs || !d_kps || !counts || !d_desc || !d_imgs[0] || !d_imgs[1] || counts[0] < 0 || counts[1] < 0 ||
        (counts[0] > 0 && (!d_kps[0] || !d_desc[0] || !d_match)) || (counts[1] > 0 && (!d_kps[1] || !d_desc[1])))
        return fail(ctx, CLC_ERR_BAD_ARG, "describe_match_pair: bad argument");
    if (!ctx->has_det) return fail(ctx, CLC_ERR_STATE, "describe_match_pair: context created without detector options");
    if (width != ctx->dopts.width || height != ctx->dopts.height || pitch < width || pitch > 0xFFFFFFFFull)
        return fail(ctx, CLC_ERR_BAD_ARG, "describe_match_pair: image size differs from DetectorOptions width/height");
    for (int b = 0; b < 2; ++b)
        if (((uintptr_t)d_desc[b] & 15u) || ((uintptr_t)d_kps[b] & 3u)) return fail(ctx, CLC_ERR_BAD_ARG, "describe_match_pair: misaligned device pointer");
    if ((uintptr_t)d_match & 3u) return fail(ctx, CLC_ERR_BAD_ARG, "describe_match_pair: misaligned device pointer");
    CLC_HIP(ctx, hipSetDevice(ctx->device));
    hipStream_t st = pick(ctx, stream);
    { const int rc = ensure_slots(ctx, 2, st); if (rc != CLC_OK) return rc; }
    const uint8_t* srcs[2] = { (const uint8_t*)d_imgs[1], (const uint8_t*)d_imgs[0] };
    ClatchBatch batch{};
    batch.kps[0] = d_kps[1]; batch.desc[0] = (uint64_t*)d_desc[1]; batch.n[0] = counts[1];
    batch.kps[1] = d_kps[0]; batch.desc[1] = (uint64_t*)d_desc[0]; batch.n[1] = counts[0];
    ctx->pyramid_valid = false;
    CLC_HIP(ctx, launch_pyramid_batch(ctx->pd, ctx->d_arena, ctx->arena_bytes, srcs, 2, (uint32_t)pitch, st, &ctx->prof));
    ctx->pyramid_valid = true;
    CLC_HIP(ctx, launch_clatch_batch(ctx->pd, ctx->d_arena, ctx->arena_bytes, batch, 2, st, &ctx->prof));
    if (counts[0] == 0) return CLC_OK;
    std::vector<K2nnJobDev> jobs(1);
    jobs[0] = K2nnJobDev{};
    jobs[0].q = (const uint4*)d_desc[0]; jobs[0].t = (const uint4*)d_desc[1]; jobs[0].out = d_match;
    jobs[0].nq = (uint32_t)counts[0]; jobs[0].nt = (uint32_t)counts[1]; jobs[0].thr = (uint32_t)(uint8_t)threshold;
    return run_jobs(ctx, jobs, st);
}

int clc_match_jobs_dev(clc_ctx* ctx, const void* d_desc_base, const clc_match_job* h_jobs, int njobs,
                       int32_t* d_match, void* stream)
{
    if (!ctx || njobs < 0 || (njobs > 0 && (!d_desc_base || !h_jobs || !d_match)))
        return fail(ctx, CLC_ERR_BAD_ARG, "match_jobs: bad argument");
    if (((uintptr_t)d_desc_base & 15u) || ((uintptr_t)d_match & 3u))
        return fail(ctx, CLC_ERR_BAD_ARG, "match_jobs: device pointers must be 16-byte aligned");
    if (njobs == 0) return CLC_OK;
    CLC_HIP(ctx, hipSetDevice(ctx->device));
    std::vector<K2nnJobDev> jobs;
    jobs.reserve(njobs);
    for (int j = 0; j < njobs; ++j) {
        if (h_jobs[j].nq == 0) continue;
        K2nnJobDev jb{};
        jb.q = (const uint4*)((const uint8_t*)d_desc_base + (size_t)h_jobs[j].q_offset * CLC_DESC_BYTES);
        jb.t = (const uint4*)((const uint8_t*)d_desc_base + (size_t)h_jobs[j].t_offset * CLC_DESC_BYTES);
        jb.out = d_match + h_jobs[j].out_offset;
        jb.nq = h_jobs[j].nq;
        jb.nt = h_jobs[j].nt;
        jb.thr = (uint32_t)(uint8_t)h_jobs[j].threshold;
        jobs.push_back(jb);
    }
    if (jobs.empty()) return CLC_OK;
    return run_jobs(ctx, jobs, pick(ctx, stream));
}

int clc_match_jobs_counted_dev(clc_ctx* ctx, const void* d_desc_base, const clc_match_job* h_jobs, int njobs,
                               const int32_t* const* d_cnt_q, const int32_t* const* d_cnt_t, const uint32_t* q_row0,
                               int32_t* d_match, void* stream)
{
    if (!ctx || njobs < 0 || (njobs > 0 && (!d_desc_base || !h_jobs || !d_match || !d_cnt_q || !d_cnt_t || !q_row0)))
        return fail(ctx, CLC_ERR_BAD_ARG, "match_jobs_counted: bad argument");
    if (((uintptr_t)d_desc_base & 15u) || ((uintptr_t)d_match & 3u))
        return fail(ctx, CLC_ERR_BAD_ARG, "match_jobs_counted: device pointers must be 16-byte aligned");
// ... 384 lines not shown
```

### coloc_amd/csrc/clc_ctx.h

```cpp
#ifndef CLC_CTX_H
#define CLC_CTX_H

#include "clc_internal.h"

#include <string>
#include <vector>

namespace clc {
struct Profiler {
    bool on = false;
    unsigned mask = 0xFFFFFFFFu;
    struct Pair { hipEvent_t a = nullptr, b = nullptr; int kernel = 0; hipStream_t stream = nullptr; bool open = false; };
    std::vector<Pair> pending;
    std::vector<hipEvent_t> pool;
    double total_ms[CLC_KERNEL_COUNT] = {};
    int launches[CLC_KERNEL_COUNT] = {};
    hipEvent_t get()
    {
        if (!pool.empty()) { hipEvent_t e = pool.back(); pool.pop_back(); return e; }
        hipEvent_t e = nullptr;
        if (hipEventCreateWithFlags(&e, hipEventDisableSystemFence) != hipSuccess) (void)hipEventCreate(&e);
        return e;
    }
    void drain()
    {
        for (Pair& p : pending) {
            if (!p.a || !p.b || p.open) continue;
            (void)hipEventSynchronize(p.b);
            float ms = 0.f;
            if (hipEventElapsedTime(&ms, p.a, p.b) == hipSuccess) { total_ms[p.kernel] += ms; launches[p.kernel] += 1; }
            pool.push_back(p.a);
            pool.push_back(p.b);
        }
        pending.clear();
    }
    ~Profiler()
    {
        for (Pair& p : pending) { if (p.a) (void)hipEventDestroy(p.a); if (p.b) (void)hipEventDestroy(p.b); }
        for (hipEvent_t e : pool) (void)hipEventDestroy(e);
    }
};
}

namespace clc {
struct DescEntry;
enum { ROWS_NONE = 0, ROWS_STAGED = 1, ROWS_OWN = 2 };
}

struct clc_ctx {
    int device = 0;
    std::vector<float> acr_lg;
    hipStream_t stream = nullptr;
    std::string err;
    bool has_det = false, has_mat = false;
    clc_detector_opts dopts{};
    clc_matcher_opts mopts{};
    clc::PyramidDesc pd{};
    uint8_t* d_arena = nullptr;
    size_t arena_bytes = 0;
    int arena_slots = 1;
    bool pyramid_valid = false;
    clc_keypoint* d_kps = nullptr;
    uint64_t* d_desc = nullptr;
    uint8_t* d_score = nullptr;
    uint64_t* d_kpmask = nullptr;
    uint32_t* d_tcount = nullptr;
    uint32_t* d_count = nullptr;
    uint32_t n_tiles = 0;
    int selection = CLC_SELECT_FIRST;
    uint32_t* d_select = nullptr;
    bool select_dirty = false;
    bool detected = false;
    uint8_t* d_q = nullptr;
    uint8_t* d_t = nullptr;
    uint8_t* d_m = nullptr;
    int map_n = -1;
    int32_t* d_match = nullptr;
    uint16_t* d_best = nullptr;
    uint16_t* d_second = nullptr;
    uint2* d_partial = nullptr;
    size_t partial_cap = 0;
    bool partial_dirty = false;
    int formulation = clc::K2NN_MATRIX;
    int target_blocks = 0;
    int bias_a = 326, bias_b = 249;
    bool xcd_map = true;
    clc::K2nnDevice k2dev{};
    int bias_source = 0;
    float bias_probe_us[4] = {};
    hipEvent_t ev_group = nullptr;
    int cache_mode = CLC_DESC_CACHE_VERIFY;
    uint8_t* d_pairs = nullptr;
    size_t pairs_cap = 0;
    double* d_pnp = nullptr;
    size_t pnp_cap = 0;
    void* h_pin = nullptr;
    size_t pin_cap = 0;
    double* d_map_X = nullptr;
    int map_X_n = -1, map_X_cap = 0;
    uint8_t* d_trk = nullptr;
    uint8_t* h_trk = nullptr;
    size_t trk_cap = 0;
    hipEvent_t ev_track = nullptr;
    uint8_t* d_pair = nullptr;
    uint8_t* h_pair = nullptr;
    size_t pair_cap = 0;
    uint8_t* h_stage = nullptr;
    size_t stage_img = 0, stage_kps = 0, stage_desc = 0, stage_cnt = 0;
    clc::DescEntry* desc_pending = nullptr;
    int staged_n = -1;
    int rows_at = clc::ROWS_NONE;
    int own_rows = 0;
    uint8_t* h_res = nullptr;
    size_t res_cap = 0;
    clc::Profiler prof;
};

namespace clc {

int fail(clc_ctx* ctx, int code, const char* what, hipError_t e = hipSuccess);

inline bool pose_K_ok(const double* K) { return K[3] == 0.0 && K[6] == 0.0 && K[7] == 0.0 && K[8] == 1.0; }

#define CLC_HIP(ctx, call)                                                      \
    do {                                                                        \
        hipError_t e__ = (call);                                                \
        if (e__ != hipSuccess) return ::clc::fail((ctx), CLC_ERR_HIP, #call, e__);     \
    } while (0)

inline hipStream_t pick(clc_ctx* ctx, void* stream) { return stream ? (hipStream_t)stream : ctx->stream; }

int ensure_partial(clc_ctx* ctx, size_t elems);
int ensure_pnp(clc_ctx* ctx, size_t doubles);
int ensure_pinned(clc_ctx* ctx, size_t bytes);
int ensure_slots(clc_ctx* ctx, int n, hipStream_t st);
int ensure_results(clc_ctx* ctx, size_t bytes);

void rows_leave(clc_ctx* ctx);

int default_target_blocks(int formulation, const K2nnDevice& dev = K2nnDevice{});
int run_jobs(clc_ctx* ctx, std::vector<K2nnJobDev>& jobs, hipStream_t st, bool probe = false);
void k2nn_probe_bias(clc_ctx* ctx);

int acr_two_view_batch(clc_ctx* const* ctxs, clc_two_view_job* const* jobs, int n_jobs, int kind );
int check_batch_contexts(clc_ctx* const* ctxs, int n_jobs, const char* what);

}
#endif
```

### coloc_amd/csrc/clc_internal.h

```cpp
#ifndef CLC_INTERNAL_H
#define CLC_INTERNAL_H

#include <hip/hip_runtime.h>
#include <stdint.h>
#include <stddef.h>

#include "../../include/coloc_hip.h"

namespace clc {

struct Profiler;
void prof_mark(Profiler* prof, int kernel, bool begin, hipStream_t stream);

struct LevelDesc {
    uint32_t w, h;
    uint32_t pitch;
    uint32_t offset;
};
struct PyramidDesc {
    LevelDesc lv[CLC_MAX_LEVELS];
    float     f[CLC_MAX_LEVELS];
    uint32_t  blk_begin[CLC_MAX_LEVELS + 1];
    int       levels;
};

hipError_t launch_pyramid(const PyramidDesc& pd, uint8_t* arena, const uint8_t* d_src, uint32_t src_pitch,
                          hipStream_t stream, Profiler* prof = nullptr);
static constexpr int kMaxBatch = CLC_MAX_BATCH;
hipError_t launch_pyramid_batch(const PyramidDesc& pd, uint8_t* arena, size_t slot_stride, const uint8_t* const* d_src,
                                int n_img, uint32_t src_pitch, hipStream_t stream, Profiler* prof = nullptr);

hipError_t launch_clatch(const PyramidDesc& pd, const uint8_t* arena, const clc_keypoint* d_kps,
                         int n, uint64_t* d_desc, hipStream_t stream, Profiler* prof = nullptr);
struct ClatchBatch {
    const clc_keypoint* kps[kMaxBatch];
    uint64_t*           desc[kMaxBatch];
    int                 n[kMaxBatch];
};
hipError_t launch_clatch_batch(const PyramidDesc& pd, const uint8_t* arena, size_t slot_stride, const ClatchBatch& batch,
                               int n_img, hipStream_t stream, Profiler* prof = nullptr);

hipError_t launch_detect(const PyramidDesc& pd, const uint8_t* arena, size_t slot_stride, int n_img, uint8_t* score, uint64_t* d_mask,
                         uint32_t* d_tcount, uint32_t threshold, uint32_t maxkp, clc_keypoint* const* d_kps, uint32_t* const* d_count,
                         hipStream_t stream, Profiler* prof = nullptr, uint32_t* d_select = nullptr, bool* select_dirty = nullptr);
uint32_t detect_select_words(const PyramidDesc& pd);
uint32_t detect_total_tiles(const PyramidDesc& pd);
hipError_t launch_clatch_counted(const PyramidDesc& pd, const uint8_t* arena, const clc_keypoint* d_kps,
                                 const uint32_t* d_count, int max_n, uint64_t* d_desc, hipStream_t stream,
                                 Profiler* prof = nullptr);
hipError_t launch_clatch_counted_batch(const PyramidDesc& pd, const uint8_t* arena, size_t slot_stride, const ClatchBatch& batch,
                                       const uint32_t* const* d_count, int n_img, hipStream_t stream, Profiler* prof = nullptr);

struct K2nnJobDev {
    const uint4* q;
    const uint4* t;
    int32_t*     out;
    uint16_t*    best_out;
    uint16_t*    second_out;
    uint32_t     nq, nt;
    uint32_t     thr;
    uint32_t     qblocks;
    uint32_t     splits;
    uint32_t     t_per_split;
    uint32_t     partial_off;
    uint32_t     nq_pad;
    uint32_t     atomic_merge;
    uint32_t     cnt_off;
    const int32_t* cnt_q;
    const int32_t* cnt_t;
    uint32_t     q_row0;
    uint32_t     xcd_rot;
    uint32_t     bias_a, bias_b;
    uint32_t     bias_magic;
    uint32_t     slot_wgs;
    uint32_t     rule;
    float        r2;
};
enum { K2NN_RULE_K2NN = 0, K2NN_RULE_RATIO = 1 };
static constexpr uint32_t kK2nnXcds = 8;
struct K2nnDevice {
    uint32_t n_xcd = kK2nnXcds;
    uint32_t n_cu = 256;
};
__device__ __forceinline__ uint32_t k2nn_job_nq(const K2nnJobDev& job)
{
    if (!job.cnt_q) return job.nq;
    const int left = *job.cnt_q - (int)job.q_row0;
    return left <= 0 ? 0u : ((uint32_t)left < job.nq ? (uint32_t)left : job.nq);
}
__device__ __forceinline__ uint32_t k2nn_job_nt(const K2nnJobDev& job)
{
    if (!job.cnt_t) return job.nt;
    const int c = *job.cnt_t;
    return c <= 0 ? 0u : ((uint32_t)c < job.nt ? (uint32_t)c : job.nt);
}
static constexpr int kK2nnJobsPerLaunch = 16;
struct K2nnJobList {
    K2nnJobDev j[kK2nnJobsPerLaunch];
    uint32_t bias_tab[128];
};
static_assert(sizeof(K2nnJobList) <= 4096, "K2nnJobList is passed as a kernel argument: it must stay within the 4 KB kernarg segment");
struct K2nnPlan {
    size_t   partial_elems;
    bool     atomic_merge;
};
enum { K2NN_MATRIX = 0, K2NN_POPCOUNT = 1 };
K2nnPlan k2nn_plan(K2nnJobDev* jobs, int njobs, int target_blocks, bool xcd_map = true, int formulation = K2NN_MATRIX, int bias_a = 0, int bias_b = 0,
                   K2nnDevice dev = K2nnDevice{});
hipError_t launch_k2nn(const K2nnJobDev* jobs, int njobs, uint2* d_partial, hipStream_t stream,
                       Profiler* prof = nullptr, int formulation = K2NN_MATRIX, uint64_t* d_stamps = nullptr, bool probe = false);
int k2nn_queries_per_block(int formulation);

hipError_t launch_pnp_residuals(const double* d_Rt, int H, const double* d_X, const double* d_x,
                                int N, const double* d_K, double* d_err, hipStream_t stream,
                                Profiler* prof = nullptr);
hipError_t launch_pnp_score(const double* d_Rt, int H, const double* d_X, const double* d_x, int N,
                            const double* d_K, double thr2, int32_t* d_count, double* d_cost,
                            hipStream_t stream, Profiler* prof = nullptr);

struct PnpResult {
    double Rt[12];
    double cost;
    int32_t h;
    int32_t count;
};
struct EpiResult {
    double E[9];
    double F[9];
    double cost;
    int32_t h;
    int32_t count;
};
struct RefineOut {
    double Rt[12];
    double cov[36];
    double cost;
    double rmse;
    int32_t iterations;
    int32_t n_used;
    int32_t ready;
    int32_t pad_;
};

struct PnpHostStage {
    const double* src;
    int           n_doubles;
    uint8_t*      h_mask;
    void*         h_result;
};
hipError_t launch_pnp_ransac(const double* d_X, const double* d_x, int N, const double* d_K, const int32_t* d_samples,
                             int S, double thr2, double* d_Rt, int32_t* d_count, double* d_cost, uint8_t* d_mask,
                             void* d_result, hipStream_t stream, Profiler* prof = nullptr, const PnpHostStage* hs = nullptr);
hipError_t launch_essential_ransac(const double* d_x1, const double* d_x2, int N, const double* d_K1, const double* d_K2,
                                   const int32_t* d_samples, int S, double thr2, double* d_FE, int32_t* d_count, double* d_cost,
                                   uint8_t* d_mask, void* d_result, hipStream_t stream, Profiler* prof = nullptr);
hipError_t launch_epipolar(const double* d_F, int H, const double* d_x1, const double* d_x2, int N, double thr2, double* d_err,
                           int32_t* d_count, double* d_cost, hipStream_t stream, Profiler* prof = nullptr);
hipError_t launch_pnp_refine(const double* d_Rt_in, const double* d_X, const double* d_x, const uint8_t* d_mask, int N,
                             const double* d_K, double huber_a, int max_iter, void* d_out, hipStream_t stream,
                             Profiler* prof = nullptr, const int32_t* d_valid = nullptr, void* h_out = nullptr);

static constexpr int kAcrMaxBatch = 128;
static constexpr int kAcrMaxN = 16384;
static constexpr size_t kAcrMaxLds = (size_t)kAcrMaxN * 8;
struct AcrProblem {
    int kind;
    int n, m, max_models, model_doubles;
    int batch_cap;
    const double* a;
    const double* b;
    const double* K1;
    const double* K2;
    const float* logc_n;
    const float* logc_k;
    double loge0, logalpha0, mult, max_threshold;
    double norm;
    uint64_t seed;
    double K1v[9];
};
struct AcrState {
    double min_nfa, error_max;
    double model[18];
    int32_t n_inliers, best_iter;
    int32_t iter, n_iter, reserve;
    int32_t n_index, index_all, ac_mode;
    int32_t rounds, last_batch;
    int32_t cur_batch;
    int32_t grow;
    int32_t rounds_eval;
    int32_t evaluated;
};
struct AcrResult {
    double model[18];
    double min_nfa;
    double error_max;
    int32_t n_inliers;
    int32_t valid;
    int32_t iterations, rounds;
};
struct AcrHyp {
    double nfa;
    double e_k;
    int32_t k;
    int32_t n_le;
};
struct AcrFinish {
    uint8_t* d_mask; AcrResult* d_res;
    uint8_t* h_mask; int32_t* h_inliers; AcrResult* h_res;
};
struct AcrChain {
    AcrProblem pb;
    AcrState* states; AcrHyp* hyps; uint32_t* sorted; double* models;
    uint32_t* best_inliers; uint32_t* index_set;
    unsigned long long* h_word;
    AcrFinish fin;
};
struct AcrChains { AcrChain c[kMaxBatch]; };
hipError_t launch_acr_round(const AcrChains& chains, int n_chains, int par, int batch_bound, hipStream_t stream);
hipError_t launch_acr_stage(const double* const* h_pinned, double* const* d_dst, const size_t* n_doubles , int n_chains,
                            hipStream_t stream, const double* const* d_a = nullptr, const double* const* d_b = nullptr,
                            const int* n_corr = nullptr, const int* a_width = nullptr, const double (*cond)[3] = nullptr);

struct TrackJobDev {
    const int32_t* match; const uint32_t* count; const clc_keypoint* kps; const float* feat;
    double* X; double* x; int32_t* query; int32_t* map; int32_t* n;
    uint32_t* h_n; int32_t* h_query; int32_t* h_map;
    int nq, feat_stride, cap;
    double focal, ppx, ppy, k1, k2, k3;
};
struct TrackJobs {
    TrackJobDev j[kMaxBatch];
    const double* map_X; int map_n;
    float scale[CLC_MAX_LEVELS];
};
hipError_t launch_track_build(TrackJobs& jobs, int n_jobs, hipStream_t stream);
int track_job_inputs(clc_ctx* ctx_map, const clc_track_job& job, TrackJobDev& out, const char* who);
int ensure_track(clc_ctx* ctx, size_t cap);

struct PairSideDev {
    const uint32_t* count; const clc_keypoint* kps; const float* feat;
    int feat_stride;
    double focal, ppx, ppy, k1, k2, k3;
};
struct PairJobDev {
    const int32_t* match;
    PairSideDev a, b;
    double* x1; double* x2; int32_t* pair_q; int32_t* pair_t; int32_t* n;
    uint32_t* h_n; int32_t* h_q; int32_t* h_t; double* h_x1; double* h_x2;
    int nq, nt, cap;
};
struct PairJobs {
    PairJobDev j[kMaxBatch];
    float scale[CLC_MAX_LEVELS];
};
hipError_t launch_pair_build(PairJobs& jobs, int n_jobs, hipStream_t stream);
int pair_job_inputs(clc_ctx* ctx, const clc_pair_job& job, PairJobDev& out, const char* who);
int ensure_pair(clc_ctx* ctx, size_t cap);
hipError_t launch_twoview_minimal(int kind, const double* d_x1, const double* d_x2, int N, const int32_t* d_samples, int S, double* d_out, hipStream_t stream);

}
#endif
// ... 1 lines not shown
```

### coloc_amd/csrc/k2nn.hip

```cpp
#include "clc_internal.h"
#include <algorithm>

namespace clc {

static constexpr int kR = 2;
static constexpr int kWaves = 8;
static constexpr int kQPerBlock = 64 * kR;
static constexpr uint32_t kKeyShift = 22;
static constexpr uint32_t kIdxMask = (1u << kKeyShift) - 1u;
static constexpr uint32_t kEmpty = 0xFFFFFFFFu;

typedef uint32_t u32x4 __attribute__((ext_vector_type(4)));
typedef uint32_t u32x2 __attribute__((ext_vector_type(2)));
typedef const u32x4 __attribute__((address_space(4)))* const_u4_ptr;
typedef const u32x4 __attribute__((address_space(1)))* global_cu4_ptr;
typedef u32x2 __attribute__((address_space(1)))* global_u2_ptr;

static constexpr int kMxQT = 2;
static constexpr int kMxWaves = 4;
static constexpr int kMxQPerBlock = 32 * kMxQT * kMxWaves;
static constexpr uint32_t kMxIdxBits = 13;
static constexpr uint32_t kMxMaxSplit = 1u << kMxIdxBits;
static constexpr uint32_t kMxMagic = 0x4B000000u;
static constexpr uint32_t kMxInf = 0x7F800000u;
static constexpr uint32_t kMxResident = 3;
static_assert((kK2nnXcds & (kK2nnXcds - 1u)) == 0u && kK2nnXcds == 8u, "k2nn_sweep_mx_kernel's id -> (query block, split) map is written with & 7 / >> 3");
static constexpr uint32_t kBiasQlBits = 5, kBiasQlMask = (1u << kBiasQlBits) - 1u;
static constexpr uint32_t kBiasBeginShift = kBiasQlBits, kBiasBeginBits = 18, kBiasBeginMask = (1u << kBiasBeginBits) - 1u;
static constexpr uint32_t kBiasSizeShift = kBiasBeginShift + kBiasBeginBits, kBiasSizeMax = (1u << (32u - kBiasSizeShift)) - 1u;
static_assert(kBiasSizeMax >= kMxMaxSplit / 32u, "a split of 256 tiles must fit the size field");
static_assert(((kIdxMask + 1u) >> 5) <= kBiasBeginMask + 1u, "every tile of an atomically folded train set must fit the begin field");

int k2nn_queries_per_block(int formulation) { return formulation == K2NN_POPCOUNT ? kQPerBlock : kMxQPerBlock; }

template <int R>
__device__ __forceinline__ void sweep_one(const uint32_t (&q)[R][16], const u32x4 a, const u32x4 b,
                                          const u32x4 c, const u32x4 d, const uint32_t t_rel,
                                          uint32_t (&best)[R], uint32_t (&second)[R])
{
#define K2NN_PAIR(t, q, accin) "v_xor_b32 %1, " t ", " q "\n\tv_bcnt_u32_b32 %0, %1, " accin "\n\ts_nop 0\n\t"
#pragma unroll
    for (int r = 0; r < R; ++r) {
        uint32_t acc, tmp;
        asm volatile(K2NN_PAIR("%10", "%2", "0") K2NN_PAIR("%11", "%3", "%0") K2NN_PAIR("%12", "%4", "%0") K2NN_PAIR("%13", "%5", "%0")
                     K2NN_PAIR("%14", "%6", "%0") K2NN_PAIR("%15", "%7", "%0") K2NN_PAIR("%16", "%8", "%0") K2NN_PAIR("%17", "%9", "%0")
                     : "=&v"(acc), "=&v"(tmp)
                     : "v"(q[r][0]), "v"(q[r][1]), "v"(q[r][2]), "v"(q[r][3]), "v"(q[r][4]), "v"(q[r][5]), "v"(q[r][6]), "v"(q[r][7]),
                       "s"(a.x), "s"(a.y), "s"(a.z), "s"(a.w), "s"(b.x), "s"(b.y), "s"(b.z), "s"(b.w));
        asm volatile(K2NN_PAIR("%12", "%4", "%0") K2NN_PAIR("%13", "%5", "%0") K2NN_PAIR("%14", "%6", "%0") K2NN_PAIR("%15", "%7", "%0")
                     K2NN_PAIR("%16", "%8", "%0") K2NN_PAIR("%17", "%9", "%0") K2NN_PAIR("%18", "%10", "%0") K2NN_PAIR("%19", "%11", "%0")
                     "v_lshl_add_u32 %1, %0, 22, %20\n\tv_med3_u32 %3, %2, %3, %1\n\tv_min_u32 %2, %2, %1"
                     : "+v"(acc), "=&v"(tmp), "+v"(best[r]), "+v"(second[r])
                     : "v"(q[r][8]), "v"(q[r][9]), "v"(q[r][10]), "v"(q[r][11]), "v"(q[r][12]), "v"(q[r][13]), "v"(q[r][14]), "v"(q[r][15]),
                       "s"(c.x), "s"(c.y), "s"(c.z), "s"(c.w), "s"(d.x), "s"(d.y), "s"(d.z), "s"(d.w), "s"(t_rel));
    }
#undef K2NN_PAIR
}

template <bool RATIO>
__device__ __forceinline__ bool accept(const K2nnJobDev& job, const int best_i, const int best_v, const int second_v)
{
    if (best_i < 0) return false;
    if (RATIO) return second_v <= 512 && (float)best_v < job.r2 * (float)second_v;
    return second_v - best_v > (int)job.thr;
}

template <bool RATIO>
__device__ __forceinline__ void emit_result(const K2nnJobDev& job, const uint32_t qi, const uint32_t bkey, const uint32_t skey)
{
    int best_v = 100000, second_v = 200000, best_i = -1;
    if (bkey != kEmpty) {
        best_v = (int)(bkey >> kKeyShift);
        best_i = (int)(bkey & kIdxMask);
        second_v = skey == kEmpty ? 100000 : (int)(skey >> kKeyShift);
    }
    job.out[qi] = accept<RATIO>(job, best_i, best_v, second_v) ? best_i : -1;
    if (job.best_out) job.best_out[qi] = (uint16_t)min(best_v, 65535);
    if (job.second_out) job.second_out[qi] = (uint16_t)min(second_v, 65535);
}

template <int R, bool RATIO = false>
__global__ __launch_bounds__(64 * kWaves) void k2nn_sweep_kernel(const K2nnJobList jobs,
                                                                  uint2* __restrict__ partial)
{
    __shared__ uint32_t s_best[kWaves - 1][R][64], s_second[kWaves - 1][R][64];
    const K2nnJobDev& job = jobs.j[blockIdx.y];
    const uint32_t job_nq = k2nn_job_nq(job), job_nt = k2nn_job_nt(job);
    const uint32_t nblk = job.qblocks * job.splits;
    if (blockIdx.x >= nblk) return;
    const uint32_t qblock = blockIdx.x / job.splits;
    const uint32_t split = blockIdx.x - qblock * job.splits;

    const uint32_t lane = threadIdx.x & 63u;
    const uint32_t wave = __builtin_amdgcn_readfirstlane(threadIdx.x >> 6);
    const uint32_t qbase = qblock * (64u * R) + lane;

    uint32_t q[R][16];
#pragma unroll
    for (int r = 0; r < R; ++r) {
        uint32_t qi = qbase + 64u * r;
        if (qi >= job_nq) qi = job_nq ? job_nq - 1u : 0u;
        const global_cu4_ptr qp = (global_cu4_ptr)(uintptr_t)job.q + (size_t)qi * 4u;
#pragma unroll
        for (int k = 0; k < 4; ++k) {
            const u32x4 v = qp[k];
            q[r][4 * k + 0] = v.x; q[r][4 * k + 1] = v.y; q[r][4 * k + 2] = v.z; q[r][4 * k + 3] = v.w;
        }
    }
    uint32_t best[R], second[R];
#pragma unroll
    for (int r = 0; r < R; ++r) { best[r] = kEmpty; second[r] = kEmpty; }

    const uint32_t s0 = min(split * job.t_per_split, job_nt);
    const uint32_t s1 = min(s0 + job.t_per_split, job_nt);
    const uint32_t per_wave = (s1 - s0 + kWaves - 1) / kWaves;
    const uint32_t t0 = min(s0 + wave * per_wave, s1);
    const uint32_t t1 = min(t0 + per_wave, s1);

    const_u4_ptr tp = (const_u4_ptr)(uintptr_t)job.t + (size_t)t0 * 4u;
    if (t0 < t1) {
        const uint32_t n = t1 - t0;
        u32x4 a0 = tp[0], b0 = tp[1], c0 = tp[2], d0 = tp[3];
        uint32_t t = t0;
        for (uint32_t pair = 0; pair < (n >> 1); ++pair, t += 2) {
            __builtin_amdgcn_s_waitcnt(0xC07F);
            __builtin_amdgcn_sched_barrier(0);
            const u32x4 a1 = tp[4], b1 = tp[5], c1 = tp[6], d1 = tp[7];
            __builtin_amdgcn_sched_barrier(0);
            sweep_one<R>(q, a0, b0, c0, d0, t - s0, best, second);
            __builtin_amdgcn_sched_barrier(0);
            __builtin_amdgcn_s_waitcnt(0xC07F);
            __builtin_amdgcn_sched_barrier(0);
            const_u4_ptr np = (t + 2 < t1) ? tp + 8 : tp;
            a0 = np[0]; b0 = np[1]; c0 = np[2]; d0 = np[3];
            __builtin_amdgcn_sched_barrier(0);
            sweep_one<R>(q, a1, b1, c1, d1, t + 1 - s0, best, second);
            __builtin_amdgcn_sched_barrier(0);
            tp += 8;
        }
        if (n & 1u) sweep_one<R>(q, a0, b0, c0, d0, t - s0, best, second);
    }

    if (wave != 0) {
#pragma unroll
        for (int r = 0; r < R; ++r) { s_best[wave - 1][r][lane] = best[r]; s_second[wave - 1][r][lane] = second[r]; }
    }
    __syncthreads();
    if (wave != 0) return;
#pragma unroll
    for (int w = 0; w < kWaves - 1; ++w) {
#pragma unroll
        for (int r = 0; r < R; ++r) {
            const uint32_t ob = s_best[w][r][lane], os = s_second[w][r][lane];
            second[r] = min(min(second[r], os), max(best[r], ob));
            best[r] = min(best[r], ob);
        }
    }

    if (job.atomic_merge) {
        unsigned int* top = reinterpret_cast<unsigned int*>(partial + job.partial_off);
        uint32_t seen = 0;
#pragma unroll
        for (int r = 0; r < R; ++r) {
            const uint32_t qi = qbase + 64u * r;
            if (qi < job_nq && best[r] != kEmpty) {
                const uint32_t bkey = best[r] + s0;
                const uint32_t skey = second[r] == kEmpty ? kEmpty : second[r] + s0;
                const uint32_t old = atomicMin(top + 2u * qi, bkey);
                const uint32_t cand = bkey < old ? min(old, skey) : bkey;
                seen |= old;
                if (cand != kEmpty) seen |= atomicMin(top + 2u * qi + 1u, cand);
            }
        }
        asm volatile("s_waitcnt vmcnt(0)" : "+v"(seen) : : "memory");
        unsigned int* cnt = reinterpret_cast<unsigned int*>(partial) + job.cnt_off + qblock;
        uint32_t arrival = 0;
        if (lane == 0) arrival = atomicAdd(cnt, 1u) + 1u;
        arrival = __builtin_amdgcn_readfirstlane(arrival);
        if (arrival != job.splits - 1u) return;
        if (lane == 0) atomicExch(cnt, kEmpty);
#pragma unroll
        for (int r = 0; r < R; ++r) {
            const uint32_t qi = qbase + 64u * r;
            if (qi < job.nq) {
                const uint32_t bkey = atomicExch(top + 2u * qi, kEmpty);
                const uint32_t skey = atomicExch(top + 2u * qi + 1u, kEmpty);
                emit_result<RATIO>(job, qi, bkey, skey);
            }
        }
        return;
    }
    const global_u2_ptr prow = (global_u2_ptr)(uintptr_t)partial + job.partial_off + (size_t)split * job.nq_pad;
#pragma unroll
    for (int r = 0; r < R; ++r) {
        const uint32_t qi = qbase + 64u * r;
        if (qi < job.nq) prow[qi] = qi < job_nq ? u32x2{ best[r], second[r] } : u32x2{ kEmpty, kEmpty };
    }
}

typedef int mx_v4i __attribute__((ext_vector_type(4)));
typedef int mx_v8i __attribute__((ext_vector_type(8)));
typedef float mx_v16f __attribute__((ext_vector_type(16)));
typedef const uint32_t __attribute__((address_space(1)))* global_cu32_ptr;
typedef const u32x2 __attribute__((address_space(1)))* global_cu2_ptr;

__device__ __forceinline__ u32x4 mx_expand(const uint32_t x)
{
    u32x4 y;
    y.x = ((x << 3) & 0x88888888u) | 0x22222222u;
    y.y = ((x << 2) & 0x88888888u) | 0x22222222u;
    y.z = ((x << 1) & 0x88888888u) | 0x22222222u;
    y.w = (x & 0x88888888u) | 0x22222222u;
    return y;
}
__device__ __forceinline__ u32x4 mx_expand_not(const uint32_t x)
{
    u32x4 y;
    y.x = (~(x << 3) & 0x88888888u) | 0x22222222u;
    y.y = (~(x << 2) & 0x88888888u) | 0x22222222u;
    y.z = (~(x << 1) & 0x88888888u) | 0x22222222u;
    y.w = (~x & 0x88888888u) | 0x22222222u;
    return y;
}
__device__ __forceinline__ float mx_med3(const float a, const float b, const float c) { return __builtin_amdgcn_fmed3f(a, b, c); }

__device__ __forceinline__ uint32_t mx_decode(const uint32_t bits, const uint32_t t0)
{
    const uint32_t rel = bits - kMxMagic;
    const uint32_t d = rel >> kMxIdxBits;
    if (bits == kMxInf || d > 512u) return kEmpty;
    return (d << kKeyShift) | (t0 + (rel & (kMxMaxSplit - 1u)));
}

__device__ __forceinline__ uint32_t mx_decode_rel(const uint32_t bits, const uint32_t end)
{
    if (bits == kMxInf) return kEmpty;
    const int v = (int)__uint_as_float(bits) - 8388608 + (int)kMxMaxSplit;
    const uint32_t d = (uint32_t)v >> kMxIdxBits;
    if (d > 512u) return kEmpty;
    return (d << kKeyShift) | (end - kMxMaxSplit + ((uint32_t)v & (kMxMaxSplit - 1u)));
}

template <bool STAMP, bool GLOBAL = false, bool PROBE = false, bool RATIO = false>
__global__ __launch_bounds__(64 * kMxWaves) void k2nn_sweep_mx_kernel(const K2nnJobList jobs, uint2* __restrict__ partial,
                                                                      uint64_t* __restrict__ stamps)
{
    constexpr int QT = kMxQT;
    constexpr int kStride = 65;
    constexpr int kQRow = 17;
    constexpr int kStageDw = kMxWaves * QT * 32 * kQRow;
    constexpr int kTileDw = 2 * 8 * kStride * 4;
    __shared__ __attribute__((aligned(16))) uint32_t s_mem[kStageDw > kTileDw ? kStageDw : kTileDw];
    u32x4 (*s_a)[8 * kStride] = reinterpret_cast<u32x4 (*)[8 * kStride]>(s_mem);
    __shared__ uint32_t s_best[kMxQPerBlock], s_second[kMxQPerBlock];
    __shared__ uint32_t s_arrival;
    const K2nnJobDev& job = jobs.j[blockIdx.y];
    const uint32_t job_nq = k2nn_job_nq(job), job_nt = k2nn_job_nt(job);
    uint64_t st_entry = 0;
    if (STAMP) st_entry = __builtin_amdgcn_s_memrealtime();
    const uint32_t within = blockIdx.x >> 3;
    const bool biased = job.bias_a != 0u;
    constexpr bool global_order = GLOBAL;
    const uint32_t bias_k = global_order ? (uint32_t)__builtin_amdgcn_readfirstlane((int)__umulhi(blockIdx.x, job.bias_magic)) : 0u;
    const uint32_t bias_q = blockIdx.x - bias_k * job.qblocks;
    const uint32_t bias_e = biased ? jobs.bias_tab[global_order ? (bias_q & 127u) : (within < 96u ? within : 95u)] : 0u;
    const uint32_t qblock = global_order ? bias_q
                          : (biased ? ((blockIdx.x + 8u - job.xcd_rot) & 7u) + 8u * (bias_e & kBiasQlMask)
                                    : ((blockIdx.x + 8u - job.xcd_rot) & 7u) + 8u * (within / job.splits));
    const uint32_t split = global_order ? bias_k : (biased ? (STAMP ? within / (job.qblocks >> 3) : 0u) : within % job.splits);
    if (qblock >= job.qblocks || (global_order && split >= job.splits) || (biased && !global_order && within >= (job.qblocks >> 3) * job.splits)) return;
    const uint32_t tid = threadIdx.x, lane = tid & 63u;
    const uint32_t wave = __builtin_amdgcn_readfirstlane(tid >> 6);

    mx_v4i b[QT][8];
    {
        uint32_t* stage = s_mem + wave * (QT * 32 * kQRow);
        const global_cu4_ptr qbase = (global_cu4_ptr)(uintptr_t)job.q;
#pragma unroll
        for (int i = 0; i < 2 * QT; ++i) {
            const uint32_t idx = (uint32_t)i * 64u + lane;
            const uint32_t r_local = idx >> 2, chunk = idx & 3u;
            uint32_t row = qblock * kMxQPerBlock + wave * (QT * 32u) + r_local;
            if (row >= job_nq) row = job_nq ? job_nq - 1u : 0u;
            const u32x4 v = qbase[(size_t)row * 4u + chunk];
            uint32_t* d = stage + r_local * kQRow + chunk * 4u;
            d[0] = v.x; d[1] = v.y; d[2] = v.z; d[3] = v.w;
        }
        __builtin_amdgcn_fence(__ATOMIC_ACQ_REL, "wavefront");
        __builtin_amdgcn_wave_barrier();
#pragma unroll
        for (int qt = 0; qt < QT; ++qt) {
            const uint32_t* src = stage + ((uint32_t)qt * 32u + (lane & 31u)) * kQRow + (lane >> 5);
#pragma unroll
            for (int j = 0; j < 8; ++j) {
                const u32x4 v = mx_expand(src[2 * j]);
                b[qt][j] = mx_v4i{ (int)v.x, (int)v.y, (int)v.z, (int)v.w };
            }
        }
    }
    __syncthreads();
    float cinit[16];
#pragma unroll
    for (int i = 0; i < 16; ++i) cinit[i] = 8388608.0f + 2097152.0f + (float)(8 * (i >> 2) + 4 * (int)(lane >> 5) + (i & 3));
    float best[QT], second[QT];
#pragma unroll
    for (int qt = 0; qt < QT; ++qt) { best[qt] = __uint_as_float(kMxInf); second[qt] = __uint_as_float(kMxInf); }

    uint32_t s0 = min(split * job.t_per_split, job_nt);
    uint32_t s1 = min(s0 + job.t_per_split, job_nt);
    if (biased && !global_order) {
        s0 = min(((bias_e >> kBiasBeginShift) & kBiasBeginMask) * 32u, job_nt);
        s1 = min(s0 + (bias_e >> kBiasSizeShift) * 32u, job_nt);
    }
    if (global_order) {
        const uint32_t n0 = bias_e & 0xFFu, n1 = (bias_e >> 8) & 0xFFu, c = (bias_e >> 16) & 0xFFu, extra = bias_e >> 24;
        const uint32_t k0 = min(split, n0), k1 = min(split - k0, n1), k2 = split - k0 - k1;
        const uint32_t begin = k0 * job.bias_a + k1 * job.bias_b + k2 * c + min(k2, extra);
        const uint32_t size = split < n0 ? job.bias_a : (split < n0 + n1 ? job.bias_b : c + (k2 < extra ? 1u : 0u));
        s0 = min(begin * 32u, job_nt);
        s1 = split + 1u == job.splits ? job_nt : min(s0 + size * 32u, job_nt);
    }
    if (global_order) {
        s0 = (uint32_t)__builtin_amdgcn_readfirstlane((int)s0);
        s1 = (uint32_t)__builtin_amdgcn_readfirstlane((int)s1);
    }
    const uint32_t ntiles = (s1 - s0 + 31u) >> 5;
    const int scale_a = 0x8B8B8B8B, scale_b = 0x7F7F7F7F;
    const uint32_t my_row = tid >> 3, my_j = tid & 7u;
    const uint32_t dst = my_j * kStride + my_row;
    const global_cu2_ptr tbase = (global_cu2_ptr)(uintptr_t)job.t + (size_t)my_j;
    const uint32_t last_row = job_nt ? job_nt - 1u : 0u;
    auto load_bits = [&](const uint32_t tile) -> u32x2 {
        const uint32_t row = min(s0 + tile * 32u + my_row, last_row);
        return tbase[(size_t)row * 8u];
    };
    u32x2 r0 = u32x2{ 0u, 0u }, r1 = u32x2{ 0u, 0u };
    if (ntiles) { r0 = load_bits(0u); r1 = load_bits(min(1u, ntiles - 1u)); }
    mx_v16f acc0, acc1;
#pragma unroll
    for (int i = 0; i < 16; ++i) { acc0[i] = __uint_as_float(kMxInf); acc1[i] = __uint_as_float(kMxInf); }
    uint64_t st_clk = 0, st_real = 0;
    if (STAMP) { st_clk = __builtin_amdgcn_s_memtime(); st_real = __builtin_amdgcn_s_memrealtime(); }
    for (uint32_t t = 0; t < ntiles; ++t) {
        const uint32_t buf = t & 1u;
        s_a[buf][dst] = mx_expand_not(r0.x);
        s_a[buf][dst + 32] = mx_expand_not(r0.y);
        r0 = r1;
        __syncthreads();
        if (t + 2u < ntiles) r1 = load_bits(t + 2u);
        if (t + 1u == ntiles && ((s1 - s0) & 31u)) {
            const uint32_t valid = (s1 - s0) & 31u;
#pragma unroll
            for (int i = 0; i < 16; ++i)
                if ((uint32_t)(8 * (i >> 2) + 4 * (int)(lane >> 5) + (i & 3)) >= valid) cinit[i] += 4194304.0f + 8192.0f;
        }
        static_assert(QT == 2, "the pipelined loop is written for two chains");
#ifndef CLC_K2NN_AHEAD
#define CLC_K2NN_AHEAD 3
#endif
        constexpr int kAhead = CLC_K2NN_AHEAD;
        u32x4 ring[kAhead];
#pragma unroll
        for (int k = 0; k < kAhead; ++k) ring[k] = s_a[buf][k * kStride + lane];
#pragma unroll
        for (int st = 0; st < 16; ++st) {
            const int c = st >> 3, j = st & 7;
            const u32x4 av = ring[st % kAhead];
            const mx_v8i a8 = { (int)av.x, (int)av.y, (int)av.z, (int)av.w, 0, 0, 0, 0 };
            const mx_v8i b8 = { b[c][j].x, b[c][j].y, b[c][j].z, b[c][j].w, 0, 0, 0, 0 };
            if (st + kAhead < 16) ring[st % kAhead] = s_a[buf][((st + kAhead) & 7) * kStride + lane];
            mx_v16f& acc = c ? acc1 : acc0;
            const mx_v16f& prev = c ? acc0 : acc1;
            const int pq = c ? 0 : 1;
            mx_v16f ci;
            if (j == 0) {
#pragma unroll
                for (int i = 0; i < 16; ++i) ci[i] = cinit[i];
            } else ci = acc;
            acc = __builtin_amdgcn_mfma_scale_f32_32x32x64_f8f6f4(a8, b8, ci, 4, 4, 0, scale_a, 0, scale_b);
#pragma unroll
            for (int i = 2 * j; i < 2 * j + 2; ++i) {
                second[pq] = mx_med3(best[pq], second[pq], prev[i]);
                best[pq] = mx_med3(best[pq], prev[i], 0.0f);
            }
            if (j == 7) { best[pq] -= 32.0f; second[pq] -= 32.0f; }
            __builtin_amdgcn_sched_barrier(0);
        }
    }
    {
#pragma unroll
        for (int i = 0; i < 16; ++i) {
            second[1] = mx_med3(best[1], second[1], acc1[i]);
            best[1] = mx_med3(best[1], acc1[i], 0.0f);
        }
        best[1] -= 32.0f; second[1] -= 32.0f;
    }

    if (STAMP) {
        const uint64_t en_clk = __builtin_amdgcn_s_memtime(), en_real = __builtin_amdgcn_s_memrealtime();
        if (tid == 0) {
            uint64_t* o = stamps + 8u * ((size_t)blockIdx.y * gridDim.x + blockIdx.x);
            o[0] = st_clk; o[1] = st_real; o[2] = en_clk; o[3] = en_real; o[4] = st_entry;
        }
    }
#pragma unroll
    for (int qt = 0; qt < QT; ++qt) {
        const uint32_t mb = __float_as_uint(best[qt]), ms = __float_as_uint(second[qt]);
        const uint32_t ob = __shfl_xor(mb, 32), os = __shfl_xor(ms, 32);
        if (lane < 32u) {
            const uint32_t slot = (wave * QT + qt) * 32u + lane;
            const uint32_t end = (job.atomic_merge ? s0 : 0u) + 32u * ntiles;
            s_best[slot] = mx_decode_rel(min(mb, ob), end);
            s_second[slot] = mx_decode_rel(min(min(ms, os), max(mb, ob)), end);
        }
    }
    __syncthreads();
    const uint32_t qi = qblock * kMxQPerBlock + tid;
    const uint32_t bkey_l = s_best[tid], skey_l = s_second[tid];
    if (!job.atomic_merge) {
        const global_u2_ptr prow = (global_u2_ptr)(uintptr_t)partial + job.partial_off + (size_t)split * job.nq_pad;
        if (qi < job.nq) prow[qi] = qi < job_nq ? u32x2{ bkey_l, skey_l } : u32x2{ kEmpty, kEmpty };
        return;
    }
    unsigned int* top = reinterpret_cast<unsigned int*>(partial + job.partial_off);
    uint32_t seen = 0;
    if (qi < job_nq && bkey_l != kEmpty) {
        const uint32_t old = atomicMin(top + 2u * qi, bkey_l);
        const uint32_t cand = bkey_l < old ? min(old, skey_l) : bkey_l;
        seen |= old;
        if (cand != kEmpty) seen |= atomicMin(top + 2u * qi + 1u, cand);
    }
    asm volatile("s_waitcnt vmcnt(0)" : "+v"(seen) : : "memory");
    __syncthreads();
    unsigned int* cnt = reinterpret_cast<unsigned int*>(partial) + job.cnt_off + qblock;
    if (tid == 0) s_arrival = atomicAdd(cnt, 1u) + 1u;
    __syncthreads();
    if (STAMP && tid == 0) {
        uint64_t* o = stamps + 8u * ((size_t)blockIdx.y * gridDim.x + blockIdx.x);
        o[5] = __builtin_amdgcn_s_memrealtime();
        o[6] = ((uint64_t)qblock << 32) | split;
        o[7] = (uint64_t)__builtin_amdgcn_s_getreg((20 << 0) | (0 << 6) | ((4 - 1) << 11)) |
               ((uint64_t)__builtin_amdgcn_s_getreg((4 << 0) | (0 << 6) | ((32 - 1) << 11)) << 8);
    }
    if (s_arrival != job.splits - 1u) return;
    if (tid == 0) atomicExch(cnt, kEmpty);
    if (qi < job.nq) {
        const uint32_t bkey = atomicExch(top + 2u * qi, kEmpty);
        const uint32_t skey = atomicExch(top + 2u * qi + 1u, kEmpty);
        emit_result<RATIO>(job, qi, bkey, skey);
    }
}

__global__ __launch_bounds__(256) void k2nn_nomatch_kernel(const K2nnJobList jobs)
{
    const K2nnJobDev& job = jobs.j[blockIdx.y];
    const uint32_t qi = blockIdx.x * 256u + threadIdx.x;
    if (job.nt != 0u || qi >= job.nq) return;
    emit_result<false>(job, qi, kEmpty, kEmpty);
}

static constexpr int kMergeQ = 32;
static constexpr int kMergeGroups = 8;

struct Top2 { int best_v, second_v, best_i; };

__device__ __forceinline__ void fold(Top2& a, const uint32_t bk, const uint32_t sk, const uint32_t t0)
{
    if (bk == kEmpty) return;
    const int b_best = (int)(bk >> kKeyShift);
    const int b_idx = (int)(t0 + (bk & kIdxMask));
    const int b_second = sk == kEmpty ? 100000 : (int)(sk >> kKeyShift);
    if (b_best < a.best_v) {
        a.second_v = min(a.best_v, b_second);
        a.best_v = b_best;
        a.best_i = b_idx;
    } else {
        a.second_v = min(a.second_v, b_best);
    }
}

__global__ __launch_bounds__(kMergeQ * kMergeGroups) void k2nn_merge_kernel(const K2nnJobList jobs,
                                                                             const uint2* __restrict__ partial)
{
    __shared__ Top2 sh[kMergeGroups][kMergeQ];
    const K2nnJobDev& job = jobs.j[blockIdx.y];
    const uint32_t qx = threadIdx.x & (kMergeQ - 1);
    const uint32_t g = threadIdx.x / kMergeQ;
    const uint32_t qi = blockIdx.x * kMergeQ + qx;
    if (blockIdx.x * kMergeQ >= job.nq) return;
    const uint32_t nsplit = job.nt ? job.splits : 0u;
    const uint32_t per_g = (nsplit + kMergeGroups - 1) / kMergeGroups;
    const uint32_t s0 = min(g * per_g, nsplit), s1 = min(s0 + per_g, nsplit);
    Top2 a{ 100000, 200000, -1 };
    if (qi < job.nq) {
        const uint2* p = partial + job.partial_off + (size_t)s0 * job.nq_pad + qi;
        uint32_t s = s0;
        for (; s + 4 <= s1; s += 4, p += 4 * (size_t)job.nq_pad) {
            const uint2 e0 = p[0], e1 = p[job.nq_pad], e2 = p[2 * (size_t)job.nq_pad], e3 = p[3 * (size_t)job.nq_pad];
            fold(a, e0.x, e0.y, s * job.t_per_split);
            fold(a, e1.x, e1.y, (s + 1) * job.t_per_split);
            fold(a, e2.x, e2.y, (s + 2) * job.t_per_split);
            fold(a, e3.x, e3.y, (s + 3) * job.t_per_split);
        }
        for (; s < s1; ++s, p += job.nq_pad) {
            const uint2 e = *p;
            fold(a, e.x, e.y, s * job.t_per_split);
        }
    }
    sh[g][qx] = a;
    __syncthreads();
    if (g != 0 || qi >= job.nq) return;
    for (int k = 1; k < kMergeGroups; ++k) {
        const Top2 b = sh[k][qx];
        if (b.best_i < 0) continue;
        if (b.best_v < a.best_v) {
            a.second_v = min(a.best_v, b.second_v);
            a.best_v = b.best_v;
            a.best_i = b.best_i;
        } else {
            a.second_v = min(a.second_v, b.best_v);
        }
    }
    const bool ok = job.rule == K2NN_RULE_RATIO ? accept<true>(job, a.best_i, a.best_v, a.second_v) : accept<false>(job, a.best_i, a.best_v, a.second_v);
    job.out[qi] = ok ? a.best_i : -1;
    if (job.best_out) job.best_out[qi] = (uint16_t)min(a.best_v, 65535);
    if (job.second_out) job.second_out[qi] = (uint16_t)min(a.second_v, 65535);
}

K2nnPlan k2nn_plan(K2nnJobDev* jobs, int njobs, int target_blocks, bool xcd_map, int formulation, int bias_a, int bias_b, K2nnDevice dev)
{
    const bool xcd_known = dev.n_xcd == kK2nnXcds && dev.n_cu % kK2nnXcds == 0u;
    const uint32_t cu_x = dev.n_cu / kK2nnXcds;
    const uint32_t slots = kMxResident * dev.n_cu;

    const bool mx = formulation != K2NN_POPCOUNT;
    const uint32_t qpb = mx ? kMxQPerBlock : kQPerBlock;
    K2nnPlan plan{0, true};
    for (int j = 0; j < njobs; ++j)
        if (jobs[j].nt > kIdxMask + 1u) plan.atomic_merge = false;
    uint32_t total_qblocks = 0;
    for (int j = 0; j < njobs; ++j) {
        jobs[j].qblocks = (jobs[j].nq + qpb - 1) / qpb;
        total_qblocks += jobs[j].qblocks;
    }
    if (total_qblocks == 0) total_qblocks = 1;
    uint32_t want = mx ? (uint32_t)target_blocks / total_qblocks : ((uint32_t)target_blocks + total_qblocks - 1) / total_qblocks;
    if (mx) {
        const uint32_t per_xcd = (total_qblocks + kK2nnXcds - 1u) / kK2nnXcds;
        const uint32_t fit = (uint32_t)target_blocks / kK2nnXcds / per_xcd;
        if (xcd_known && fit < want) want = fit;
    }
    if (want < 1) want = 1;
    size_t off = 0;
    uint32_t rot = 0;
    for (int j = 0; j < njobs; ++j) {
        K2nnJobDev& jb = jobs[j];
        jb.xcd_rot = mx ? rot : 0u;
        rot = (rot + jb.qblocks) & (kK2nnXcds - 1u);
        uint32_t splits = want;
        const uint32_t min_per = mx ? 64u : 16u * kWaves;
        const uint32_t max_splits = jb.nt / min_per > 0 ? jb.nt / min_per : 1u;
        if (splits > max_splits) splits = max_splits;
        if (!mx && xcd_map && splits >= 8u) splits = (splits + 4u) / 8u * 8u > max_splits ? splits / 8u * 8u : (splits + 4u) / 8u * 8u;
        uint32_t per = jb.nt ? (jb.nt + splits - 1) / splits : 1u;
        if (mx) {
            per = (per + 31u) & ~31u;
            if (per > kMxMaxSplit) per = kMxMaxSplit;
        }
        if (per > kIdxMask + 1u) per = kIdxMask + 1u;
        splits = jb.nt ? (jb.nt + per - 1) / per : 1u;
        jb.splits = splits;
        jb.t_per_split = per;
        jb.bias_a = jb.bias_b = jb.bias_magic = 0u;
        jb.slot_wgs = 0u;
        jb.nq_pad = (jb.nq + 63u) & ~63u;
        jb.partial_off = (uint32_t)off;
        jb.atomic_merge = plan.atomic_merge ? 1u : 0u;
        off += plan.atomic_merge ? (size_t)jb.nq_pad : (size_t)splits * jb.nq_pad;
        if (plan.atomic_merge) {
            jb.cnt_off = (uint32_t)(2u * off);
            off += (jb.qblocks + 1u) / 2u;
        }
    }
    if (mx && njobs == 1 && plan.atomic_merge && bias_a > 0 && bias_b > 0 && xcd_known && kMxResident * cu_x <= 96u) {
        K2nnJobDev& jb = jobs[0];
        const uint32_t per_xcd = (jb.qblocks >> 3) * jb.splits;
        const uint32_t nt_tiles = (jb.nt + 31u) >> 5;
        const uint32_t mean = jb.splits ? nt_tiles / jb.splits : 0u;
        if ((jb.qblocks & 7u) == 0u && jb.qblocks >= 24u && per_xcd > 2u * cu_x && per_xcd <= 3u * cu_x && !jb.cnt_q && !jb.cnt_t && jb.splits >= 6u && mean >= 8u) {
            const uint32_t den = jb.splits * 256u;
            const uint32_t a = bias_a < 64 ? (uint32_t)bias_a : (nt_tiles * (uint32_t)bias_a + den / 2u) / den;
            const uint32_t b = bias_b < 64 ? (uint32_t)bias_b : (nt_tiles * (uint32_t)bias_b + den / 2u) / den;
            const uint32_t nqx = jb.qblocks >> 3;
            bool ok = a >= 1u && b >= 1u && a <= 255u && b <= 255u && nqx <= kBiasQlMask + 1u && nt_tiles <= kBiasBeginMask;
            for (uint32_t ql = 0; ok && ql < nqx; ++ql) {
                const uint32_t n0 = std::min((cu_x - ql + nqx - 1u) / nqx, jb.splits);
                const uint32_t n1 = std::min((2u * cu_x - ql + nqx - 1u) / nqx, jb.splits) - n0;
                const uint32_t n2 = jb.splits - n0 - n1;
                const uint32_t used = n0 * a + n1 * b;
                ok = n2 >= 1u && used < nt_tiles && (nt_tiles - used + n2 - 1u) / n2 <= 255u && (nt_tiles - used) / n2 >= 2u;
            }
            if (ok) { jb.bias_a = a; jb.bias_b = b; jb.bias_magic = 0u; jb.slot_wgs = cu_x; }
        }
        const uint32_t QB = jb.qblocks;
        uint32_t sp = QB ? (uint32_t)target_blocks / QB : 0u;
        if (sp > nt_tiles / 8u) sp = nt_tiles / 8u;
        if (jb.bias_a == 0u && (QB & 7u) != 0u && QB >= 24u && QB <= 128u && sp >= 6u && QB * sp > 2u * dev.n_cu && QB * sp <= slots && !jb.cnt_q && !jb.cnt_t &&
            (uint32_t)target_blocks == slots) {
            const uint32_t den = sp * 256u;
            const uint32_t a = bias_a < 64 ? (uint32_t)bias_a : (nt_tiles * (uint32_t)bias_a + den / 2u) / den;
            const uint32_t b = bias_b < 64 ? (uint32_t)bias_b : (nt_tiles * (uint32_t)bias_b + den / 2u) / den;
            bool ok = a >= 1u && b >= 1u && a <= 255u && b <= 255u;
            for (uint32_t q = 0; ok && q < QB; ++q) {
                const uint32_t n0 = std::min((dev.n_cu - q + QB - 1u) / QB, sp);
                const uint32_t n1 = std::min((2u * dev.n_cu - q + QB - 1u) / QB, sp) - n0;
                const uint32_t n2 = sp - n0 - n1;
                const uint32_t used = n0 * a + n1 * b;
                ok = n2 >= 1u && used < nt_tiles && (nt_tiles - used + n2 - 1u) / n2 <= 255u && (nt_tiles - used) / n2 >= 2u;
            }
            if (ok) {
                jb.bias_a = a; jb.bias_b = b;
                jb.bias_magic = (uint32_t)((0x100000000ull + QB - 1u) / QB);
                jb.slot_wgs = dev.n_cu;
                jb.splits = sp;
                jb.t_per_split = ((nt_tiles + sp - 1u) / sp) * 32u;
            }
        }
    }
    plan.partial_elems = off;
    return plan;
}

hipError_t launch_k2nn(const K2nnJobDev* jobs, int njobs, uint2* d_partial, hipStream_t stream, Profiler* prof, int formulation,
                       uint64_t* d_stamps, bool probe)
{
    for (int base = 0, cnt = 0; base < njobs; base += cnt) {
        cnt = 1;
        while (cnt < kK2nnJobsPerLaunch && base + cnt < njobs && jobs[base + cnt].rule == jobs[base].rule) ++cnt;
        const bool ratio = jobs[base].rule == K2NN_RULE_RATIO;
        K2nnJobList list;
        uint32_t grid_x = 0, max_nq = 0, max_nq_empty = 0;
        for (int j = 0; j < cnt; ++j) {
            list.j[j] = jobs[base + j];
            const uint32_t qb = formulation == K2NN_POPCOUNT ? list.j[j].qblocks : ((list.j[j].qblocks + 7u) & ~7u);
            const uint32_t gx = list.j[j].nt ? qb * list.j[j].splits : 0u;
            if (gx > grid_x) grid_x = gx;
            if (list.j[j].nq > max_nq) max_nq = list.j[j].nq;
            if (list.j[j].nt == 0u && list.j[j].nq > max_nq_empty) max_nq_empty = list.j[j].nq;
        }
        for (int j = cnt; j < kK2nnJobsPerLaunch; ++j) list.j[j] = K2nnJobDev{};
        for (uint32_t& e : list.bias_tab) e = 0u;
        if (cnt == 1 && list.j[0].bias_a != 0u && list.j[0].bias_magic != 0u && formulation != K2NN_POPCOUNT) {
            const K2nnJobDev& jb = list.j[0];
            const uint32_t QB = jb.qblocks, nt_tiles = (jb.nt + 31u) >> 5;
            for (uint32_t q = 0; q < QB && q < 128u; ++q) {
                const uint32_t n0 = std::min((jb.slot_wgs - q + QB - 1u) / QB, jb.splits);
                const uint32_t n1 = std::min((2u * jb.slot_wgs - q + QB - 1u) / QB, jb.splits) - n0;
                const uint32_t n2 = jb.splits - n0 - n1;
                const uint32_t used = n0 * jb.bias_a + n1 * jb.bias_b;
                const uint32_t rest = nt_tiles > used ? nt_tiles - used : 0u;
                const uint32_t c = n2 ? rest / n2 : 0u, extra = n2 ? rest - c * n2 : 0u;
                list.bias_tab[q] = n0 | (n1 << 8) | (std::min(c, 255u) << 16) | (std::min(extra, 255u) << 24);
            }
            grid_x = QB * jb.splits;
        } else
        if (cnt == 1 && list.j[0].bias_a != 0u && formulation != K2NN_POPCOUNT) {
            const K2nnJobDev& jb = list.j[0];
            const uint32_t nqx = jb.qblocks >> 3, nt_tiles = (jb.nt + 31u) >> 5;
            for (uint32_t w = 0; w < nqx * jb.splits && w < 96u; ++w) {
                const uint32_t ql = w % nqx, k = w / nqx;
                const uint32_t n0 = std::min((jb.slot_wgs - ql + nqx - 1u) / nqx, jb.splits);
                const uint32_t n1 = std::min((2u * jb.slot_wgs - ql + nqx - 1u) / nqx, jb.splits) - n0;
                const uint32_t n2 = jb.splits - n0 - n1;
                const uint32_t used = n0 * jb.bias_a + n1 * jb.bias_b;
                const uint32_t rest = nt_tiles > used ? nt_tiles - used : 0u;
                const uint32_t c = n2 ? rest / n2 : 0u, extra = n2 ? rest - c * n2 : 0u;
                const uint32_t k0 = std::min(k, n0), k1 = std::min(k - k0, n1), k2 = k - k0 - k1;
                const uint32_t begin = k0 * jb.bias_a + k1 * jb.bias_b + k2 * c + std::min(k2, extra);
                uint32_t size = k < n0 ? jb.bias_a : (k < n0 + n1 ? jb.bias_b : c + (k2 < extra ? 1u : 0u));
                if (k + 1u == jb.splits) size = nt_tiles > begin ? nt_tiles - begin : 0u;
                list.bias_tab[w] = (ql & kBiasQlMask) | (std::min(begin, kBiasBeginMask) << kBiasBeginShift) | (std::min(size, kBiasSizeMax) << kBiasSizeShift);
            }
        }
        if (max_nq == 0) continue;
        if (grid_x > 0) {
            prof_mark(prof, CLC_KERNEL_K2NN_SWEEP, true, stream);
            if (formulation == K2NN_POPCOUNT && ratio)
                hipLaunchKernelGGL((k2nn_sweep_kernel<kR, true>), dim3(grid_x, cnt), dim3(64 * kWaves), 0, stream, list, d_partial);
            else if (formulation == K2NN_POPCOUNT)
                hipLaunchKernelGGL(k2nn_sweep_kernel<kR>, dim3(grid_x, cnt), dim3(64 * kWaves), 0, stream, list, d_partial);
            else if (ratio && cnt == 1 && list.j[0].bias_a != 0u && list.j[0].bias_magic != 0u)
                hipLaunchKernelGGL((k2nn_sweep_mx_kernel<false, true, false, true>), dim3(grid_x, cnt), dim3(64 * kMxWaves), 0, stream, list, d_partial,
                                   (uint64_t*)nullptr);
            else if (ratio)
                hipLaunchKernelGGL((k2nn_sweep_mx_kernel<false, false, false, true>), dim3(grid_x, cnt), dim3(64 * kMxWaves), 0, stream, list, d_partial,
                                   (uint64_t*)nullptr);
            else if (cnt == 1 && list.j[0].bias_a != 0u && list.j[0].bias_magic != 0u && d_stamps)
                hipLaunchKernelGGL((k2nn_sweep_mx_kernel<true, true>), dim3(grid_x, cnt), dim3(64 * kMxWaves), 0, stream, list, d_partial, d_stamps);
            else if (cnt == 1 && list.j[0].bias_a != 0u && list.j[0].bias_magic != 0u)
                hipLaunchKernelGGL((k2nn_sweep_mx_kernel<false, true>), dim3(grid_x, cnt), dim3(64 * kMxWaves), 0, stream, list, d_partial,
                                   (uint64_t*)nullptr);
            else if (d_stamps)
                hipLaunchKernelGGL((k2nn_sweep_mx_kernel<true>), dim3(grid_x, cnt), dim3(64 * kMxWaves), 0, stream, list, d_partial, d_stamps);
            else if (probe)
                hipLaunchKernelGGL((k2nn_sweep_mx_kernel<false, false, true>), dim3(grid_x, cnt), dim3(64 * kMxWaves), 0, stream, list, d_partial,
                                   (uint64_t*)nullptr);
            else
                hipLaunchKernelGGL((k2nn_sweep_mx_kernel<false>), dim3(grid_x, cnt), dim3(64 * kMxWaves), 0, stream, list, d_partial,
                                   (uint64_t*)nullptr);
            prof_mark(prof, CLC_KERNEL_K2NN_SWEEP, false, stream);
        }
        if (list.j[0].atomic_merge) {
            if (max_nq_empty)
                hipLaunchKernelGGL(k2nn_nomatch_kernel, dim3((max_nq_empty + 255) / 256, cnt), dim3(256), 0, stream, list);
        } else {
            prof_mark(prof, CLC_KERNEL_K2NN_MERGE, true, stream);
            hipLaunchKernelGGL(k2nn_merge_kernel, dim3((max_nq + kMergeQ - 1) / kMergeQ, cnt), dim3(kMergeQ * kMergeGroups),
                               0, stream, list, (const uint2*)d_partial);
            prof_mark(prof, CLC_KERNEL_K2NN_MERGE, false, stream);
        }
    }
    return hipGetLastError();
}

}
```

### include/coloc_hip.h

```cpp
#ifndef COLOC_HIP_H
#define COLOC_HIP_H

#include <stddef.h>
#include <stdint.h>

#ifdef __cplusplus
extern "C" {
#endif

#define CLC_ABI_VERSION 4
#define CLC_DESC_BYTES 64
#define CLC_MAX_LEVELS 8
#define CLC_MAX_BATCH 8
#define CLC_DETECT_MAX_WIDTH 4096

enum {
    CLC_OK = 0,
    CLC_ERR_BAD_ARG = 1,
    CLC_ERR_CAPACITY = 2,
    CLC_ERR_HIP = 3,
    CLC_ERR_NO_DEVICE = 4,
    CLC_ERR_STATE = 5
};

typedef struct clc_detector_opts {
    float    scale_factor;
    uint8_t  scale_levels;
    uint32_t width;
    uint32_t height;
    uint32_t maxkp;
    uint8_t  thresh;
} clc_detector_opts;

typedef struct clc_matcher_opts {
    float    distRatio;
    int      thresh;
    uint32_t maxkp;
} clc_matcher_opts;

typedef struct clc_keypoint {
    int32_t x;
    int32_t y;
    uint8_t score;
    float   angle;
    uint8_t scale;
} clc_keypoint;

typedef struct clc_ctx clc_ctx;

typedef struct clc_match_job {
    uint32_t q_offset;
    uint32_t nq;
    uint32_t t_offset;
    uint32_t nt;
    uint32_t out_offset;
    uint32_t threshold;
} clc_match_job;

typedef struct clc_desc_handle {
    const void* host;
    uint64_t    generation;
    uint32_t    count;
    uint32_t    slot;
} clc_desc_handle;


int clc_abi_version(void);
const char* clc_status_string(int status);

int clc_ctx_create(int device_id, const clc_detector_opts* dopts, const clc_matcher_opts* mopts,
                   clc_ctx** out_ctx);
int clc_ctx_destroy(clc_ctx* ctx);
const char* clc_last_error_string(const clc_ctx* ctx);
int clc_sync(clc_ctx* ctx);
void* clc_stream(clc_ctx* ctx);
int clc_ctx_device(const clc_ctx* ctx);

enum {
    CLC_KERNEL_PYRAMID = 0,
    CLC_KERNEL_CLATCH = 1,
    CLC_KERNEL_K2NN_SWEEP = 2,
    CLC_KERNEL_K2NN_MERGE = 3,
    CLC_KERNEL_PNP_RESIDUALS = 4,
    CLC_KERNEL_PNP_SCORE = 5,
    CLC_KERNEL_DETECT = 6,
    CLC_KERNEL_COUNT = 7
};
int clc_profile_enable(clc_ctx* ctx, int on);
int clc_profile_reset(clc_ctx* ctx);
int clc_profile_read(clc_ctx* ctx, int kernel, double* total_ms, int* launches);
const char* clc_kernel_name(int kernel);


int clc_pyramid_build(clc_ctx* ctx, const uint8_t* h_img, uint32_t width, uint32_t height);
int clc_pyramid_build_dev(clc_ctx* ctx, const void* d_img, uint32_t width, uint32_t height,
                          size_t pitch, void* stream);
int clc_pyramid_level(const clc_ctx* ctx, int level, uint32_t* w, uint32_t* h, size_t* pitch,
                      const void** d_ptr);
int clc_pyramid_download(clc_ctx* ctx, int level, uint8_t* h_out);

enum { CLC_SELECT_FIRST = 0, CLC_SELECT_STRONGEST = 1 };
int clc_detect_set_selection(clc_ctx* ctx, int mode);
int clc_detect_selection(const clc_ctx* ctx);
int clc_detect(clc_ctx* ctx, clc_keypoint* h_kps, int capacity, int* n_written, int* n_found);
int clc_detect_dev(clc_ctx* ctx, void* stream);
int clc_detect_buffers(clc_ctx* ctx, const clc_keypoint** d_kps, const uint32_t** d_count, void** d_desc);
int clc_describe_detected_dev(clc_ctx* ctx, void* d_desc, void* stream);
int clc_detect_and_describe(clc_ctx* ctx, const uint8_t* h_img, uint32_t width, uint32_t height,
                            clc_keypoint* h_kps, uint8_t* h_desc, int capacity, int* n_written, int* n_found);
int clc_detect_and_describe_view(clc_ctx* ctx, const uint8_t* h_img, uint32_t width, uint32_t height, const clc_keypoint** h_kps,
                                 const uint8_t** h_desc, int* n_written, int* n_found);
int clc_detect_store_descriptors(clc_ctx* ctx, void* h_dst, int n, clc_desc_handle* handle );

int clc_detect_batch_dev(clc_ctx* ctx, int n_images, const void* const* d_imgs, uint32_t width, uint32_t height, size_t pitch,
                         clc_keypoint* const* d_kps, uint32_t* const* d_counts, void* const* d_desc, void* stream);


int clc_describe(clc_ctx* ctx, const clc_keypoint* h_kps, int n, uint8_t* h_desc);
int clc_describe_dev(clc_ctx* ctx, const clc_keypoint* d_kps, int n, void* d_desc, void* stream);
int clc_describe_batch_dev(clc_ctx* ctx, int n_images, const void* const* d_imgs, uint32_t width, uint32_t height,
                           size_t pitch, const clc_keypoint* const* d_kps, const int* counts, void* const* d_desc,
                           void* stream);
int clc_keypoints_to_features(const clc_keypoint* h_kps, int n, float* h_feat4);


int clc_match_2nn(clc_ctx* ctx, const void* h_q, int nq, const void* h_t, int nt, int threshold,
                  int32_t* h_match, uint16_t* h_best, uint16_t* h_second);
enum { CLC_DESC_CACHE_OFF = 0, CLC_DESC_CACHE_VERIFY = 1, CLC_DESC_CACHE_TRUST = 2 };
int clc_desc_cache_mode(clc_ctx* ctx, int mode);
int clc_desc_cache_publish(clc_ctx* ctx, const void* d_src, const void* h_desc, int n, clc_desc_handle* handle );
int clc_desc_handle_live(const clc_desc_handle* handle);
int clc_desc_cache_clear(void);
int clc_desc_cache_stats(unsigned long long* hits, unsigned long long* misses);
int clc_match_2nn_dev(clc_ctx* ctx, const void* d_q, int nq, const void* d_t, int nt,
                      int threshold, int32_t* d_match, void* stream);
int clc_describe_match_pair_dev(clc_ctx* ctx, const void* const* d_imgs, uint32_t width, uint32_t height, size_t pitch,
                                const clc_keypoint* const* d_kps, const int* counts, void* const* d_desc, int threshold,
                                int32_t* d_match, void* stream);
int clc_match_jobs_dev(clc_ctx* ctx, const void* d_desc_base, const clc_match_job* h_jobs,
                       int njobs, int32_t* d_match, void* stream);
int clc_match_jobs_counted_dev(clc_ctx* ctx, const void* d_desc_base, const clc_match_job* h_jobs, int njobs,
                               const int32_t* const* d_cnt_q, const int32_t* const* d_cnt_t, const uint32_t* q_row0,
                               int32_t* d_match, void* stream);

enum { CLC_K2NN_MATRIX = 0, CLC_K2NN_POPCOUNT = 1 };
int clc_k2nn_set_formulation(clc_ctx* ctx, int formulation);
int clc_k2nn_queries_per_block(const clc_ctx* ctx);
int clc_k2nn_plan_query(const clc_ctx* ctx, int nq, int nt, int32_t* info);
int clc_k2nn_device_info(const clc_ctx* ctx, int32_t* info, float* probe_us);

int clc_k2nn_clock_check(clc_ctx* ctx, const void* d_q, int nq, const void* d_t, int nt, int32_t* d_match, void* stream,
                         double* ghz_median, double* ghz_min, double* ghz_max, int* workgroups);

int clc_match_pairs(clc_ctx* ctx, const void* const* h_desc, const int* counts, int ncams,
                    const int* pairs , int npairs, int threshold,
                    int32_t* const* h_match);

int clc_set_map(clc_ctx* ctx, const void* h_desc, int n);
int clc_match_map(clc_ctx* ctx, const void* h_q, int nq, int threshold, int32_t* h_match);
int clc_match_map_dev(clc_ctx* ctx, const void* d_q, int nq, int threshold, int32_t* d_match, void* stream);

int clc_match_ratio_2nn(clc_ctx* ctx, const void* h_q, int nq, const void* h_t, int nt, float ratio,
                        int32_t* h_match, uint16_t* h_best, uint16_t* h_second);
int clc_match_ratio_2nn_dev(clc_ctx* ctx, const void* d_q, int nq, const void* d_t, int nt, float ratio, int32_t* d_match, void* stream);
int clc_match_ratio_pairs(clc_ctx* ctx, const void* const* h_desc, const int* counts, int ncams, const float* const* h_xy,
                          const int* pairs , int npairs, float ratio,
                          int32_t* const* h_pairs_out, int* n_out);
int clc_match_map_ratio(clc_ctx* ctx, const void* h_q, int nq, const float* xy_map, const float* xy_q, float ratio,
                        int32_t* h_pairs, int* n_out);
int clc_match_map_ratio_dev(clc_ctx* ctx, const void* d_q, int nq, float ratio, int32_t* d_match, void* stream);
int clc_ratio_matches_to_pairs(const int32_t* match, int nq, const float* xy_db, const float* xy_q, int32_t* pairs, int* n);


int clc_pnp_residuals(clc_ctx* ctx, const double* h_Rt, int H, const double* h_X,
                      const double* h_x, int N, const double* h_K, double* h_err);
int clc_pnp_score(clc_ctx* ctx, const double* h_Rt, int H, const double* h_X, const double* h_x,
                  int N, const double* h_K, double thr2, int32_t* h_count, double* h_cost);

int clc_epipolar_residuals(clc_ctx* ctx, const double* h_F, int H, const double* h_x1, const double* h_x2,
                           int N, double* h_err);
int clc_epipolar_score(clc_ctx* ctx, const double* h_F, int H, const double* h_x1, const double* h_x2, int N,
                       double thr2, int32_t* h_count, double* h_cost);

int clc_essential_ransac(clc_ctx* ctx, const double* h_x1, const double* h_x2, int N, const double* h_K1,
                         const double* h_K2, const int32_t* h_samples, int S, uint64_t seed, double thr2,
                         double* h_E, double* h_F, uint8_t* h_inlier_mask, int* n_inliers);
int clc_essential_fivepoint(clc_ctx* ctx, const double* h_x1, const double* h_x2, int N, const double* h_K1,
                            const double* h_K2, const int32_t* h_samples, int S, double* h_E_out);

int clc_pnp_ransac(clc_ctx* ctx, const double* h_X, const double* h_x, int N, const double* h_K,
                   const int32_t* h_samples, int S, uint64_t seed, double thr2, double* h_Rt,
                   uint8_t* h_inlier_mask, int* n_inliers, double* cost);
int clc_pnp_refine(clc_ctx* ctx, const double* h_X, const double* h_x, int N, const double* h_K,
                   const uint8_t* h_inlier_mask, const double* h_Rt_in, double huber_a, int max_iter,
                   double* h_Rt_out, double* h_cov, double* rmse, int* iterations);

int clc_pnp_localize(clc_ctx* ctx, const double* h_X, const double* h_x, int N, const double* h_K,
                     const int32_t* h_samples, int S, uint64_t seed, double thr2, double huber_a,
                     double* h_Rt, double* h_cov, uint8_t* h_inlier_mask, int* n_inliers, double* rmse);

int clc_pnp_p3p(clc_ctx* ctx, const double* h_X, const double* h_x, int N, const double* h_K,
                const int32_t* h_samples, int S, double* h_Rt_out);

#define CLC_MC_ID_BYTES 128
enum { CLC_MC_RCCL = 0, CLC_MC_PEER_COPY = 1 };
typedef struct clc_mc clc_mc;
typedef struct clc_mc_share {
    int32_t  first, second;
    uint32_t q_begin, nq;
    uint32_t out_offset;
} clc_mc_share;
int clc_mc_plan(const int* counts, int ncams, int world, int rank, int grain, clc_mc_share* out, int capacity, int* n_out);
int clc_mc_unique_id(uint8_t id[CLC_MC_ID_BYTES]);
int clc_mc_create(clc_ctx* ctx, const uint8_t id[CLC_MC_ID_BYTES], int world, int rank, int maxkp, clc_mc** out);
int clc_mc_virtual_put(clc_mc* mc, int other_rank, const void* d_desc, int count, void* stream);
int clc_mc_open_peers(clc_mc* mc, void* stream);
int clc_mc_destroy(clc_mc* mc);
const char* clc_mc_last_error_string(const clc_mc* mc);
int clc_mc_arena(const clc_mc* mc, void** d_arena, int* world, int* maxkp);
int clc_mc_gather_dev(clc_mc* mc, const void* d_my_desc, int my_count, int mode, int* h_counts_out, void* stream);
int clc_mc_match_dev(clc_mc* mc, int threshold, int32_t* d_match, int match_capacity, clc_mc_share* h_shares,
                     int share_capacity, int* n_shares, void* stream);
int clc_mc_gather_enqueue_dev(clc_mc* mc, const void* d_my_desc, int my_count, const int32_t* d_my_count, int mode, void* stream);
int clc_mc_match_enqueue_dev(clc_mc* mc, int threshold, int32_t* d_match, int match_capacity, clc_mc_share* h_shares,
                             int share_capacity, int* n_shares, void* stream);
int clc_mc_counts(clc_mc* mc, int* h_counts_out, void* stream);
int clc_mc_set_overlap(clc_mc* mc, int on);
int clc_mc_comm_info(const clc_mc* mc, int* n_ranks, int* user_rank);

int clc_pnp_acransac(clc_ctx* ctx, const double* h_X, const double* h_x, int N, const double* h_K, int max_iteration,
                     uint64_t seed, double precision, double* h_Rt, uint8_t* h_inlier_mask, int32_t* h_inliers,
                     int* n_inliers, double* error_max, double* min_nfa, int* iterations);
int clc_pnp_localize_ac(clc_ctx* ctx, const double* h_X, const double* h_x, int N, const double* h_K, int max_iteration,
                        uint64_t seed, double precision, double huber_a, double* h_Rt, double* h_cov,
                        uint8_t* h_inlier_mask, int32_t* h_inliers, int* n_inliers, double* error_max, double* rmse);
typedef struct clc_pose_job {
    const double* X;
    const double* x;
    const double* K;
    int           n;
    int           max_iteration;
    uint64_t      seed;
    double        precision;
    int           refine;
    double        huber_a;
    double*       Rt;
    double*       cov;
    uint8_t*      inlier_mask;
    int32_t*      inliers;
    int           n_inliers;
    int           iterations;
    int           status;
    double        error_max;
    double        rmse;
} clc_pose_job;
int clc_pnp_localize_ac_batch(clc_ctx* const* ctxs, clc_pose_job* jobs, int n_jobs);

int clc_essential_acransac(clc_ctx* ctx, const double* h_x1, const double* h_x2, int N, const double* h_K1,
                           const double* h_K2, int img_w, int img_h, int max_iteration, uint64_t seed, double precision,
                           double* h_E, double* h_F, uint8_t* h_inlier_mask, int32_t* h_inliers, int* n_inliers,
                           double* error_max, double* min_nfa, int* iterations);

typedef struct clc_two_view_job {
    const double* x1;
    const double* x2;
    const double* K1;
    const double* K2;
    int           n, img_w, img_h, max_iteration;
    uint64_t      seed;
    double        precision;
    double*       E;
    double*       F;
    uint8_t*      inlier_mask;
    int32_t*      inliers;
    int           n_inliers, iterations, status;
    double        error_max, min_nfa;
} clc_two_view_job;
int clc_essential_acransac_batch(clc_ctx* const* ctxs, clc_two_view_job* jobs, int n_jobs);

enum { CLC_MODEL_ESSENTIAL = 'E', CLC_MODEL_FUNDAMENTAL = 'F', CLC_MODEL_HOMOGRAPHY = 'H' };
int clc_two_view_acransac(clc_ctx* ctx, int model, const double* h_x1, const double* h_x2, int N, const double* h_K1,
                          const double* h_K2, int img_w, int img_h, int max_iteration, uint64_t seed, double precision,
                          double* h_M, double* h_F, uint8_t* h_inlier_mask, int32_t* h_inliers, int* n_inliers,
                          double* error_max, double* min_nfa, int* iterations);
int clc_two_view_acransac_batch(clc_ctx* const* ctxs, int model, clc_two_view_job* jobs, int n_jobs);
int clc_two_view_minimal(clc_ctx* ctx, int model, const double* h_x1, const double* h_x2, int N, int img_w, int img_h,
                         const int32_t* h_samples, int S, double* h_models);

enum { CLC_INTER_OK = 0, CLC_INTER_NO_MODEL = 1 , CLC_INTER_NO_RELATIVE_POSE = 2 ,
       CLC_INTER_NO_SCALE = 3 , CLC_INTER_NO_REFINEMENT = 4 };
typedef struct clc_inter_pose_job {
    clc_two_view_job tv;
    const int32_t* map_index;
    const double*  map_X;
    int            map_n;
    const double*  Rt_source;
    double         huber_a;
    const void*    d_first_desc;
    const int32_t* first_feature;
    const void*    d_map_desc;
    int            match_threshold;
// ... 78 lines not shown
```

Before: 1.255 million.

## Add co-resident k2nn planning mode and fuse top-2 update into paired med3

```diff
diff --git a/coloc_amd/abi.py b/coloc_amd/abi.py
--- a/coloc_amd/abi.py
+++ b/coloc_amd/abi.py
@@ -99,7 +99,7 @@
     "clc_kernel_name", "clc_detect", "clc_detect_dev", "clc_detect_buffers", "clc_describe_detected_dev",
     "clc_detect_and_describe", "clc_detect_batch_dev", "clc_desc_cache_publish", "clc_desc_cache_clear", "clc_desc_cache_stats", "clc_desc_cache_mode", "clc_desc_handle_live", "clc_detect_and_describe_view", "clc_detect_store_descriptors", "clc_describe_match_pair_dev", "clc_essential_acransac_batch", "clc_inter_pose_batch", "clc_pnp_localize_ac_batch", "clc_match_pairs", "clc_pnp_ransac", "clc_pnp_p3p", "clc_pnp_refine", "clc_pnp_localize", "clc_epipolar_residuals", "clc_epipolar_score", "clc_cov_intersection", "clc_essential_ransac",
     "clc_essential_fivepoint", "clc_describe_batch_dev", "clc_match_map_dev", "clc_k2nn_set_formulation",
-    "clc_k2nn_queries_per_block", "clc_k2nn_plan_query", "clc_k2nn_device_info", "clc_pnp_acransac", "clc_pnp_localize_ac", "clc_essential_acransac", "clc_k2nn_clock_check", "clc_ctx_device", "clc_mc_plan", "clc_mc_unique_id",
+    "clc_k2nn_queries_per_block", "clc_k2nn_plan_query", "clc_k2nn_plan_table", "clc_k2nn_device_info", "clc_pnp_acransac", "clc_pnp_localize_ac", "clc_essential_acransac", "clc_k2nn_clock_check", "clc_ctx_device", "clc_mc_plan", "clc_mc_unique_id",
     "clc_mc_create", "clc_mc_destroy", "clc_mc_last_error_string", "clc_mc_arena", "clc_mc_gather_dev", "clc_mc_match_dev", "clc_mc_virtual_put", "clc_mc_open_peers",
     "clc_mc_gather_enqueue_dev", "clc_mc_match_enqueue_dev", "clc_mc_counts", "clc_mc_set_overlap", "clc_mc_comm_info", "clc_match_jobs_counted_dev",
     "clc_two_view_acransac", "clc_two_view_acransac_batch", "clc_two_view_minimal",
@@ -244,6 +244,7 @@
     lib.clc_k2nn_set_formulation.argtypes = [vp, ci]
     lib.clc_k2nn_queries_per_block.argtypes = [vp]
     lib.clc_k2nn_plan_query.argtypes = [vp, ci, ci, vp]
+    lib.clc_k2nn_plan_table.argtypes = [vp, ci, ci, vp, ci]
     lib.clc_k2nn_device_info.argtypes = [vp, vp, vp]
     lib.clc_set_map_points.argtypes = [vp, vp, ci]
     lib.clc_track_build_dev.argtypes = [vp, vp, vp, vp, vp, vp, vp, vp]
@@ -596,6 +597,27 @@
     return out
 
 
+_PLAN_KEYS = ("qblocks", "splits", "t_per_split", "atomic_merge", "bias_a_tiles", "bias_b_tiles", "queries_per_block", "target_blocks")
+
+
+def k2nn_plan_query_host(nq, nt):
+    info = (C.c_int32 * 8)()
+    rc = load_library().clc_k2nn_plan_query(None, int(nq), int(nt), info)
+    if rc != 0:
+        raise CLCError(rc, "clc_k2nn_plan_query")
+    return dict(zip(_PLAN_KEYS, [int(v) for v in info]))
+
+
+def k2nn_plan_table(nq, nt, handle=None):
+    lib = load_library()
+    cap = 1 << 16
+    rows = np.zeros((cap, 3), np.int32)
+    n = lib.clc_k2nn_plan_table(handle, int(nq), int(nt), rows.ctypes.data_as(C.c_void_p), cap)
+    if n < 0 or n > cap:
+        raise CLCError(-n if n < 0 else 2, "clc_k2nn_plan_table")
+    return rows[:n].copy()
+
+
 class Context:
 
     def __init__(self, device=0, width=640, height=480, maxkp=10000, scale_factor=1.2, scale_levels=8,
@@ -771,7 +793,11 @@
         us = (C.c_float * 4)()
         self._chk(self.lib.clc_k2nn_device_info(self.h, info, us))
         d = dict(zip(("xcds", "cus", "default_target_blocks", "bias_a", "bias_b", "bias_source", "kernel_xcds", "target_blocks_env"), [int(v) for v in info]))
-        d["bias_source"] = ("default", "CLC_K2NN_BIAS", "probe")[d["bias_source"]]
+        packed = d["bias_source"]
+        d["bias_source"] = ("default", "CLC_K2NN_BIAS", "probe")[packed & 0xFF]
+        d["resident"] = (packed >> 8) & 0xFF
+        d["resident_env"] = (packed >> 16) & 0xF
+        d["bias2"] = (packed >> 20) & 0x3FF
         d["probe_us"] = dict(zip(("295:264", "311:256", "326:249", "326:233"), [float(v) for v in us]))
         return d
 
@@ -780,6 +806,9 @@
         self._chk(self.lib.clc_k2nn_plan_query(self.h, int(nq), int(nt), info))
         return dict(zip(("qblocks", "splits", "t_per_split", "atomic_merge", "bias_a_tiles", "bias_b_tiles", "queries_per_block", "target_blocks"),
                         [int(v) for v in info]))
+
+    def k2nn_plan_table(self, nq, nt):
+        return k2nn_plan_table(nq, nt, self.h)
 
     def k2nn_clock_check(self, d_q, nq, d_t, nt, d_match, stream=None):
         med, lo, hi, n = C.c_double(), C.c_double(), C.c_double(), C.c_int()
diff --git a/coloc_amd/csrc/capi_core.hip b/coloc_amd/csrc/capi_core.hip
--- a/coloc_amd/csrc/capi_core.hip
+++ b/coloc_amd/csrc/capi_core.hip
@@ -1,6 +1,7 @@
 #include "clc_ctx.h"
 #include "desc_cache.h"
 
+#include <atomic>
 #include <chrono>
 #include <cmath>
 #include <cstdio>
@@ -183,6 +184,14 @@
     memset(ctx->h_stage + ctx->stage_cnt, 0, 256);
     return CLC_OK;
 }
+
+}
+
+namespace clc {
+
+static std::atomic<int> g_live[64];
+static void live_count(const int device, const int d) { if (device >= 0 && device < 64) g_live[device].fetch_add(d, std::memory_order_relaxed); }
+int live_contexts(const int device) { return device >= 0 && device < 64 ? g_live[device].load(std::memory_order_relaxed) : 0; }
 
 }
 
@@ -251,6 +260,15 @@
         int a = 0, b = 0;
         if (sscanf(e, "%d,%d", &a, &b) == 2 && a >= 0 && b >= 0 && a < 1024 && b < 1024) { ctx->bias_a = a; ctx->bias_b = b; ctx->bias_source = 1; }
     }
+    if (const char* e = getenv("CLC_K2NN_RESIDENT")) {
+        const int v = atoi(e);
+        if (v == 2 || v == 3) ctx->resident = v;
+        else if (e[0] == 'a') ctx->resident = 1;
+    }
+    if (const char* e = getenv("CLC_K2NN_BIAS2")) {
+        const int v = atoi(e);
+        if (v > 0 && v < 1024) ctx->bias2 = v;
+    }
     if (const char* e = getenv("CLC_K2NN_FORMULATION"))
         ctx->formulation = (e[0] == 'p' || e[0] == '1') ? K2NN_POPCOUNT : K2NN_MATRIX;
     if (dopts) {
@@ -294,6 +312,8 @@
     CREATE_HIP(hipStreamSynchronize(ctx->stream));
 #undef CREATE_HIP
     if (ctx->bias_source == 0) k2nn_probe_bias(ctx);
+    live_count(ctx->device, +1);
+    ctx->counted = true;
     *out_ctx = ctx;
     return CLC_OK;
 }
@@ -301,6 +321,7 @@
 int clc_ctx_destroy(clc_ctx* ctx)
 {
     if (!ctx) return CLC_ERR_BAD_ARG;
+    if (ctx->counted) live_count(ctx->device, -1);
     (void)hipSetDevice(ctx->device);
     if (ctx->stream) (void)hipStreamSynchronize(ctx->stream);
     void* bufs[] = { ctx->d_arena, ctx->d_kps, ctx->d_desc, ctx->d_score, ctx->d_kpmask, ctx->d_tcount, ctx->d_select, ctx->d_count, ctx->d_q, ctx->d_t, ctx->d_m, ctx->d_match,
diff --git a/coloc_amd/csrc/capi_match.hip b/coloc_amd/csrc/capi_match.hip
--- a/coloc_amd/csrc/capi_match.hip
+++ b/coloc_amd/csrc/capi_match.hip
@@ -16,10 +16,40 @@
 
 int default_target_blocks(int formulation, const K2nnDevice& dev) { return (int)((formulation == K2NN_POPCOUNT ? 10u : 3u) * dev.n_cu); }
 
+int k2nn_resident(const clc_ctx* ctx)
+{
+    if (ctx->formulation == K2NN_POPCOUNT) return 3;
+    if (ctx->resident != 1) return ctx->resident == 2 ? 2 : 3;
+    return ctx->bias_source != 1 && live_contexts(ctx->device) > 1 ? 2 : 3;
+}
+
+K2nnPlan k2nn_plan_ctx(const clc_ctx* ctx, K2nnJobDev* jobs, const int njobs, const bool probe, int* resident_used, int* target_used)
+{
+    int res = probe ? 3 : k2nn_resident(ctx);
+    int target = ctx->target_blocks > 0 ? ctx->target_blocks : default_target_blocks(ctx->formulation, ctx->k2dev);
+    K2nnPlan plan{};
+    if (res == 2) {
+        std::vector<K2nnJobDev> tri(jobs, jobs + njobs);
+        const int target2 = ctx->target_blocks > 0 ? ctx->target_blocks : 2 * (int)ctx->k2dev.n_cu;
+        const int a2 = ctx->bias_a > 0 && ctx->bias_b > 0 ? ctx->bias2 : 0;
+        plan = k2nn_plan(tri.data(), njobs, target2, ctx->xcd_map, ctx->formulation, a2, a2, ctx->k2dev, 2);
+        uint64_t wgs = 0;
+        for (int j = 0; j < njobs; ++j)
+            if (tri[j].nt) wgs += (uint64_t)(tri[j].bias_magic ? tri[j].qblocks : ((tri[j].qblocks + 7u) & ~7u)) * tri[j].splits;
+        if (wgs <= 2u * (uint64_t)ctx->k2dev.n_cu) {
+            std::copy(tri.begin(), tri.end(), jobs);
+            target = target2;
+        } else res = 3;
+    }
+    if (res != 2) plan = k2nn_plan(jobs, njobs, target, ctx->xcd_map, ctx->formulation, ctx->bias_a, ctx->bias_b, ctx->k2dev, 3);
+    if (resident_used) *resident_used = res;
+    if (target_used) *target_used = target;
+    return plan;
+}
+
 int run_jobs(clc_ctx* ctx, std::vector<K2nnJobDev>& jobs, hipStream_t st, bool probe)
 {
-    const int target = ctx->target_blocks > 0 ? ctx->target_blocks : default_target_blocks(ctx->formulation, ctx->k2dev);
-    const K2nnPlan plan = k2nn_plan(jobs.data(), (int)jobs.size(), target, ctx->xcd_map, ctx->formulation, ctx->bias_a, ctx->bias_b, ctx->k2dev);
+    const K2nnPlan plan = k2nn_plan_ctx(ctx, jobs.data(), (int)jobs.size(), probe);
     const int rc = ensure_partial(ctx, plan.partial_elems);
     if (rc != CLC_OK) return rc;
     if (!plan.atomic_merge) ctx->partial_dirty = true;
@@ -117,13 +147,37 @@
     return k2nn_queries_per_block(ctx ? ctx->formulation : K2NN_MATRIX);
 }
 
-int clc_k2nn_plan_query(const clc_ctx* ctx, int nq, int nt, int32_t* info)
-{
-    if (!ctx || nq < 0 || nt < 0 || !info) return CLC_ERR_BAD_ARG;
+static clc_ctx* planning_ctx(const clc_ctx* ctx, clc_ctx& tmp)
+{
+    if (ctx) return const_cast<clc_ctx*>(ctx);
+    tmp.device = -1;
+    if (const char* e = getenv("CLC_K2NN_RESIDENT")) { const int v = atoi(e); if (v == 2 || v == 3) tmp.resident = v; else if (e[0] == 'a') tmp.resident = 1; }
+    if (const char* e = getenv("CLC_K2NN_BIAS2")) { const int v = atoi(e); if (v > 0 && v < 1024) tmp.bias2 = v; }
+    if (const char* e = getenv("CLC_K2NN_TARGET_BLOCKS")) { const int v = atoi(e); if (v > 0) tmp.target_blocks = v; }
+    return &tmp;
+}
+
+int clc_k2nn_plan_table(const clc_ctx* ctx_in, int nq, int nt, int32_t* rows, int cap)
+{
+    if (nq <= 0 || nt <= 0 || !rows || cap < 0) return -CLC_ERR_BAD_ARG;
+    clc_ctx tmp;
+    const clc_ctx* ctx = planning_ctx(ctx_in, tmp);
+    if (ctx->formulation == K2NN_POPCOUNT) return -CLC_ERR_STATE;
     K2nnJobDev jb{};
     jb.nq = (uint32_t)nq; jb.nt = (uint32_t)nt;
-    const int target = ctx->target_blocks > 0 ? ctx->target_blocks : default_target_blocks(ctx->formulation, ctx->k2dev);
-    const K2nnPlan plan = k2nn_plan(&jb, 1, target, ctx->xcd_map, ctx->formulation, ctx->bias_a, ctx->bias_b, ctx->k2dev);
+    (void)k2nn_plan_ctx(ctx, &jb, 1);
+    return k2nn_plan_table(jb, rows, cap);
+}
+
+int clc_k2nn_plan_query(const clc_ctx* ctx_in, int nq, int nt, int32_t* info)
+{
+    if (nq < 0 || nt < 0 || !info) return CLC_ERR_BAD_ARG;
+    clc_ctx tmp;
+    const clc_ctx* ctx = planning_ctx(ctx_in, tmp);
+    K2nnJobDev jb{};
+    jb.nq = (uint32_t)nq; jb.nt = (uint32_t)nt;
+    int target = 0;
+    const K2nnPlan plan = k2nn_plan_ctx(ctx, &jb, 1, false, nullptr, &target);
     info[0] = (int32_t)jb.qblocks; info[1] = (int32_t)jb.splits; info[2] = (int32_t)jb.t_per_split; info[3] = plan.atomic_merge ? 1 : 0;
     info[4] = (int32_t)jb.bias_a; info[5] = (int32_t)jb.bias_b; info[6] = k2nn_queries_per_block(ctx->formulation); info[7] = target;
     return CLC_OK;
@@ -133,7 +187,9 @@
 {
     if (!ctx || !info) return CLC_ERR_BAD_ARG;
     info[0] = (int32_t)ctx->k2dev.n_xcd; info[1] = (int32_t)ctx->k2dev.n_cu; info[2] = default_target_blocks(ctx->formulation, ctx->k2dev);
-    info[3] = ctx->bias_a; info[4] = ctx->bias_b; info[5] = ctx->bias_source; info[6] = (int32_t)kK2nnXcds; info[7] = ctx->target_blocks;
+    info[3] = ctx->bias_a; info[4] = ctx->bias_b;
+    info[5] = ctx->bias_source | (k2nn_resident(ctx) << 8) | (ctx->resident << 16) | (ctx->bias2 << 20);
+    info[6] = (int32_t)kK2nnXcds; info[7] = ctx->target_blocks;
     if (probe_us) for (int c = 0; c < 4; ++c) probe_us[c] = ctx->bias_probe_us[c];
     return CLC_OK;
 }
@@ -150,8 +206,7 @@
     jobs[0] = K2nnJobDev{};
     jobs[0].q = (const uint4*)d_q; jobs[0].t = (const uint4*)d_t; jobs[0].out = d_match;
     jobs[0].nq = (uint32_t)nq; jobs[0].nt = (uint32_t)nt; jobs[0].thr = 40u;
-    const int target = ctx->target_blocks > 0 ? ctx->target_blocks : default_target_blocks(ctx->formulation, ctx->k2dev);
-    const K2nnPlan plan = k2nn_plan(jobs.data(), 1, target, ctx->xcd_map, ctx->formulation, ctx->bias_a, ctx->bias_b, ctx->k2dev);
+    const K2nnPlan plan = k2nn_plan_ctx(ctx, jobs.data(), 1);
     if (!plan.atomic_merge) return fail(ctx, CLC_ERR_CAPACITY, "k2nn_clock_check: train set too large");
     int rc = ensure_partial(ctx, plan.partial_elems);
     if (rc != CLC_OK) return rc;
diff --git a/coloc_amd/csrc/clc_ctx.h b/coloc_amd/csrc/clc_ctx.h
--- a/coloc_amd/csrc/clc_ctx.h
+++ b/coloc_amd/csrc/clc_ctx.h
@@ -84,6 +84,9 @@
     int formulation = clc::K2NN_MATRIX;
     int target_blocks = 0;
     int bias_a = 326, bias_b = 249;
+    int resident = 3;
+    int bias2 = 314;
+    bool counted = false;
     bool xcd_map = true;
     clc::K2nnDevice k2dev{};
     int bias_source = 0;
@@ -140,6 +143,9 @@
 
 int default_target_blocks(int formulation, const K2nnDevice& dev = K2nnDevice{});
 int run_jobs(clc_ctx* ctx, std::vector<K2nnJobDev>& jobs, hipStream_t st, bool probe = false);
+int live_contexts(int device);
+int k2nn_resident(const clc_ctx* ctx);
+K2nnPlan k2nn_plan_ctx(const clc_ctx* ctx, K2nnJobDev* jobs, int njobs, bool probe = false, int* resident_used = nullptr, int* target_used = nullptr);
 void k2nn_probe_bias(clc_ctx* ctx);
 
 int acr_two_view_batch(clc_ctx* const* ctxs, clc_two_view_job* const* jobs, int n_jobs, int kind );
diff --git a/coloc_amd/csrc/clc_internal.h b/coloc_amd/csrc/clc_internal.h
--- a/coloc_amd/csrc/clc_internal.h
+++ b/coloc_amd/csrc/clc_internal.h
@@ -73,6 +73,7 @@
     uint32_t     bias_a, bias_b;
     uint32_t     bias_magic;
     uint32_t     slot_wgs;
+    uint32_t     slot_n;
     uint32_t     rule;
     float        r2;
 };
@@ -106,7 +107,8 @@
 };
 enum { K2NN_MATRIX = 0, K2NN_POPCOUNT = 1 };
 K2nnPlan k2nn_plan(K2nnJobDev* jobs, int njobs, int target_blocks, bool xcd_map = true, int formulation = K2NN_MATRIX, int bias_a = 0, int bias_b = 0,
-                   K2nnDevice dev = K2nnDevice{});
+                   K2nnDevice dev = K2nnDevice{}, int resident = 3);
+int k2nn_plan_table(const K2nnJobDev& job, int32_t* rows, int cap);
 hipError_t launch_k2nn(const K2nnJobDev* jobs, int njobs, uint2* d_partial, hipStream_t stream,
                        Profiler* prof = nullptr, int formulation = K2NN_MATRIX, uint64_t* d_stamps = nullptr, bool probe = false);
 int k2nn_queries_per_block(int formulation);
diff --git a/coloc_amd/csrc/k2nn.hip b/coloc_amd/csrc/k2nn.hip
--- a/coloc_amd/csrc/k2nn.hip
+++ b/coloc_amd/csrc/k2nn.hip
@@ -24,6 +24,7 @@
 static constexpr uint32_t kMxMagic = 0x4B000000u;
 static constexpr uint32_t kMxInf = 0x7F800000u;
 static constexpr uint32_t kMxResident = 3;
+static constexpr uint32_t kMxCoResident = 2;
 static_assert((kK2nnXcds & (kK2nnXcds - 1u)) == 0u && kK2nnXcds == 8u, "k2nn_sweep_mx_kernel's id -> (query block, split) map is written with & 7 / >> 3");
 static constexpr uint32_t kBiasQlBits = 5, kBiasQlMask = (1u << kBiasQlBits) - 1u;
 static constexpr uint32_t kBiasBeginShift = kBiasQlBits, kBiasBeginBits = 18, kBiasBeginMask = (1u << kBiasBeginBits) - 1u;
@@ -223,6 +224,12 @@
     return y;
 }
 __device__ __forceinline__ float mx_med3(const float a, const float b, const float c) { return __builtin_amdgcn_fmed3f(a, b, c); }
+__device__ __forceinline__ void mx_top2_pair(float& best, float& second, const float a, const float b)
+{
+    const float m = mx_med3(best, a, b);
+    best = __builtin_fminf(__builtin_fminf(best, a), b);
+    second = __builtin_fminf(second, m);
+}
 
 __device__ __forceinline__ uint32_t mx_decode(const uint32_t bits, const uint32_t t0)
 {
@@ -378,21 +385,14 @@
                 for (int i = 0; i < 16; ++i) ci[i] = cinit[i];
             } else ci = acc;
             acc = __builtin_amdgcn_mfma_scale_f32_32x32x64_f8f6f4(a8, b8, ci, 4, 4, 0, scale_a, 0, scale_b);
-#pragma unroll
-            for (int i = 2 * j; i < 2 * j + 2; ++i) {
-                second[pq] = mx_med3(best[pq], second[pq], prev[i]);
-                best[pq] = mx_med3(best[pq], prev[i], 0.0f);
-            }
+            mx_top2_pair(best[pq], second[pq], prev[2 * j], prev[2 * j + 1]);
             if (j == 7) { best[pq] -= 32.0f; second[pq] -= 32.0f; }
             __builtin_amdgcn_sched_barrier(0);
         }
     }
     {
 #pragma unroll
-        for (int i = 0; i < 16; ++i) {
-            second[1] = mx_med3(best[1], second[1], acc1[i]);
-            best[1] = mx_med3(best[1], acc1[i], 0.0f);
-        }
+        for (int i = 0; i < 16; i += 2) mx_top2_pair(best[1], second[1], acc1[i], acc1[i + 1]);
         best[1] -= 32.0f; second[1] -= 32.0f;
     }
 
@@ -527,11 +527,12 @@
     if (job.second_out) job.second_out[qi] = (uint16_t)min(a.second_v, 65535);
 }
 
-K2nnPlan k2nn_plan(K2nnJobDev* jobs, int njobs, int target_blocks, bool xcd_map, int formulation, int bias_a, int bias_b, K2nnDevice dev)
+K2nnPlan k2nn_plan(K2nnJobDev* jobs, int njobs, int target_blocks, bool xcd_map, int formulation, int bias_a, int bias_b, K2nnDevice dev, int resident)
 {
     const bool xcd_known = dev.n_xcd == kK2nnXcds && dev.n_cu % kK2nnXcds == 0u;
     const uint32_t cu_x = dev.n_cu / kK2nnXcds;
-    const uint32_t slots = kMxResident * dev.n_cu;
+    const uint32_t res = resident == (int)kMxCoResident ? kMxCoResident : kMxResident;
+    const uint32_t slots = res * dev.n_cu;
 
     const bool mx = formulation != K2NN_POPCOUNT;
     const uint32_t qpb = mx ? kMxQPerBlock : kQPerBlock;
@@ -573,6 +574,7 @@
         jb.t_per_split = per;
         jb.bias_a = jb.bias_b = jb.bias_magic = 0u;
         jb.slot_wgs = 0u;
+        jb.slot_n = res;
         jb.nq_pad = (jb.nq + 63u) & ~63u;
         jb.partial_off = (uint32_t)off;
         jb.atomic_merge = plan.atomic_merge ? 1u : 0u;
@@ -583,43 +585,44 @@
         }
     }
     if (mx && njobs == 1 && plan.atomic_merge && bias_a > 0 && bias_b > 0 && xcd_known && kMxResident * cu_x <= 96u) {
+        const uint32_t s1_end = (res - 1u) * cu_x;
         K2nnJobDev& jb = jobs[0];
         const uint32_t per_xcd = (jb.qblocks >> 3) * jb.splits;
         const uint32_t nt_tiles = (jb.nt + 31u) >> 5;
         const uint32_t mean = jb.splits ? nt_tiles / jb.splits : 0u;
-        if ((jb.qblocks & 7u) == 0u && jb.qblocks >= 24u && per_xcd > 2u * cu_x && per_xcd <= 3u * cu_x && !jb.cnt_q && !jb.cnt_t && jb.splits >= 6u && mean >= 8u) {
+        if ((jb.qblocks & 7u) == 0u && jb.qblocks >= 24u && per_xcd > (res - 1u) * cu_x && per_xcd <= res * cu_x && !jb.cnt_q && !jb.cnt_t && jb.splits >= 6u && mean >= 8u) {
             const uint32_t den = jb.splits * 256u;
-            const uint32_t a = bias_a < 64 ? (uint32_t)bias_a : (nt_tiles * (uint32_t)bias_a + den / 2u) / den;
-            const uint32_t b = bias_b < 64 ? (uint32_t)bias_b : (nt_tiles * (uint32_t)bias_b + den / 2u) / den;
+            const uint32_t a = bias_a < 64 ? (uint32_t)bias_a : std::min((nt_tiles * (uint32_t)bias_a + den / 2u) / den, 255u);
+            const uint32_t b = res == 2u ? 1u : bias_b < 64 ? (uint32_t)bias_b : (nt_tiles * (uint32_t)bias_b + den / 2u) / den;
             const uint32_t nqx = jb.qblocks >> 3;
             bool ok = a >= 1u && b >= 1u && a <= 255u && b <= 255u && nqx <= kBiasQlMask + 1u && nt_tiles <= kBiasBeginMask;
             for (uint32_t ql = 0; ok && ql < nqx; ++ql) {
                 const uint32_t n0 = std::min((cu_x - ql + nqx - 1u) / nqx, jb.splits);
-                const uint32_t n1 = std::min((2u * cu_x - ql + nqx - 1u) / nqx, jb.splits) - n0;
+                const uint32_t n1 = std::min((s1_end - ql + nqx - 1u) / nqx, jb.splits) - n0;
                 const uint32_t n2 = jb.splits - n0 - n1;
                 const uint32_t used = n0 * a + n1 * b;
                 ok = n2 >= 1u && used < nt_tiles && (nt_tiles - used + n2 - 1u) / n2 <= 255u && (nt_tiles - used) / n2 >= 2u;
             }
-            if (ok) { jb.bias_a = a; jb.bias_b = b; jb.bias_magic = 0u; jb.slot_wgs = cu_x; }
+            if (ok) { jb.bias_a = a; jb.bias_b = res == 2u ? 0u : b; jb.bias_magic = 0u; jb.slot_wgs = cu_x; }
         }
         const uint32_t QB = jb.qblocks;
         uint32_t sp = QB ? (uint32_t)target_blocks / QB : 0u;
         if (sp > nt_tiles / 8u) sp = nt_tiles / 8u;
-        if (jb.bias_a == 0u && (QB & 7u) != 0u && QB >= 24u && QB <= 128u && sp >= 6u && QB * sp > 2u * dev.n_cu && QB * sp <= slots && !jb.cnt_q && !jb.cnt_t &&
+        if (jb.bias_a == 0u && (QB & 7u) != 0u && QB >= 24u && QB <= 128u && sp >= 6u && QB * sp > (res - 1u) * dev.n_cu && QB * sp <= slots && !jb.cnt_q && !jb.cnt_t &&
             (uint32_t)target_blocks == slots) {
             const uint32_t den = sp * 256u;
-            const uint32_t a = bias_a < 64 ? (uint32_t)bias_a : (nt_tiles * (uint32_t)bias_a + den / 2u) / den;
-            const uint32_t b = bias_b < 64 ? (uint32_t)bias_b : (nt_tiles * (uint32_t)bias_b + den / 2u) / den;
+            const uint32_t a = bias_a < 64 ? (uint32_t)bias_a : std::min((nt_tiles * (uint32_t)bias_a + den / 2u) / den, 255u);
+            const uint32_t b = res == 2u ? 1u : bias_b < 64 ? (uint32_t)bias_b : (nt_tiles * (uint32_t)bias_b + den / 2u) / den;
             bool ok = a >= 1u && b >= 1u && a <= 255u && b <= 255u;
             for (uint32_t q = 0; ok && q < QB; ++q) {
                 const uint32_t n0 = std::min((dev.n_cu - q + QB - 1u) / QB, sp);
-                const uint32_t n1 = std::min((2u * dev.n_cu - q + QB - 1u) / QB, sp) - n0;
+                const uint32_t n1 = std::min(((res - 1u) * dev.n_cu - q + QB - 1u) / QB, sp) - n0;
                 const uint32_t n2 = sp - n0 - n1;
                 const uint32_t used = n0 * a + n1 * b;
                 ok = n2 >= 1u && used < nt_tiles && (nt_tiles - used + n2 - 1u) / n2 <= 255u && (nt_tiles - used) / n2 >= 2u;
             }
             if (ok) {
-                jb.bias_a = a; jb.bias_b = b;
+                jb.bias_a = a; jb.bias_b = res == 2u ? 0u : b;
                 jb.bias_magic = (uint32_t)((0x100000000ull + QB - 1u) / QB);
                 jb.slot_wgs = dev.n_cu;
                 jb.splits = sp;
@@ -631,6 +634,88 @@
     return plan;
 }
 
+static void k2nn_fill_list(K2nnJobList& list, const K2nnJobDev* jobs, const int cnt, const int formulation, uint32_t& grid_x, uint32_t& max_nq, uint32_t& max_nq_empty)
+{
+    grid_x = 0; max_nq = 0; max_nq_empty = 0;
+    for (int j = 0; j < cnt; ++j) {
+        list.j[j] = jobs[j];
+        const uint32_t qb = formulation == K2NN_POPCOUNT ? list.j[j].qblocks : ((list.j[j].qblocks + 7u) & ~7u);
+        const uint32_t gx = list.j[j].nt ? qb * list.j[j].splits : 0u;
+        if (gx > grid_x) grid_x = gx;
+        if (list.j[j].nq > max_nq) max_nq = list.j[j].nq;
+        if (list.j[j].nt == 0u && list.j[j].nq > max_nq_empty) max_nq_empty = list.j[j].nq;
+    }
+    for (int j = cnt; j < kK2nnJobsPerLaunch; ++j) list.j[j] = K2nnJobDev{};
+    for (uint32_t& e : list.bias_tab) e = 0u;
+    if (cnt == 1 && list.j[0].bias_a != 0u && list.j[0].bias_magic != 0u && formulation != K2NN_POPCOUNT) {
+        const K2nnJobDev& jb = list.j[0];
+        const uint32_t QB = jb.qblocks, nt_tiles = (jb.nt + 31u) >> 5;
+        for (uint32_t q = 0; q < QB && q < 128u; ++q) {
+            const uint32_t n0 = std::min((jb.slot_wgs - q + QB - 1u) / QB, jb.splits);
+            const uint32_t n1 = std::min(((jb.slot_n - 1u) * jb.slot_wgs - q + QB - 1u) / QB, jb.splits) - n0;
+            const uint32_t n2 = jb.splits - n0 - n1;
+            const uint32_t used = n0 * jb.bias_a + n1 * jb.bias_b;
+            const uint32_t rest = nt_tiles > used ? nt_tiles - used : 0u;
+            const uint32_t c = n2 ? rest / n2 : 0u, extra = n2 ? rest - c * n2 : 0u;
+            list.bias_tab[q] = n0 | (n1 << 8) | (std::min(c, 255u) << 16) | (std::min(extra, 255u) << 24);
+        }
+        grid_x = QB * jb.splits;
+    } else
+    if (cnt == 1 && list.j[0].bias_a != 0u && formulation != K2NN_POPCOUNT) {
+        const K2nnJobDev& jb = list.j[0];
+        const uint32_t nqx = jb.qblocks >> 3, nt_tiles = (jb.nt + 31u) >> 5;
+        for (uint32_t w = 0; w < nqx * jb.splits && w < 96u; ++w) {
+            const uint32_t ql = w % nqx, k = w / nqx;
+            const uint32_t n0 = std::min((jb.slot_wgs - ql + nqx - 1u) / nqx, jb.splits);
+            const uint32_t n1 = std::min(((jb.slot_n - 1u) * jb.slot_wgs - ql + nqx - 1u) / nqx, jb.splits) - n0;
+            const uint32_t n2 = jb.splits - n0 - n1;
+            const uint32_t used = n0 * jb.bias_a + n1 * jb.bias_b;
+            const uint32_t rest = nt_tiles > used ? nt_tiles - used : 0u;
+            const uint32_t c = n2 ? rest / n2 : 0u, extra = n2 ? rest - c * n2 : 0u;
+            const uint32_t k0 = std::min(k, n0), k1 = std::min(k - k0, n1), k2 = k - k0 - k1;
+            const uint32_t begin = k0 * jb.bias_a + k1 * jb.bias_b + k2 * c + std::min(k2, extra);
+            uint32_t size = k < n0 ? jb.bias_a : (k < n0 + n1 ? jb.bias_b : c + (k2 < extra ? 1u : 0u));
+            if (k + 1u == jb.splits) size = nt_tiles > begin ? nt_tiles - begin : 0u;
+            list.bias_tab[w] = (ql & kBiasQlMask) | (std::min(begin, kBiasBeginMask) << kBiasBeginShift) | (std::min(size, kBiasSizeMax) << kBiasSizeShift);
+        }
+    }
+}
+
+int k2nn_plan_table(const K2nnJobDev& job, int32_t* rows, const int cap)
+{
+    K2nnJobList list;
+    uint32_t grid_x, max_nq, max_nq_empty;
+    k2nn_fill_list(list, &job, 1, K2NN_MATRIX, grid_x, max_nq, max_nq_empty);
+    const K2nnJobDev& jb = list.j[0];
+    const bool biased = jb.bias_a != 0u, global_order = biased && jb.bias_magic != 0u;
+    for (uint32_t id = 0; id < grid_x && (int)id < cap; ++id) {
+        const uint32_t within = id >> 3;
+        const uint32_t bias_k = global_order ? (uint32_t)(((uint64_t)id * jb.bias_magic) >> 32) : 0u;
+        const uint32_t bias_q = id - bias_k * jb.qblocks;
+        const uint32_t e = biased ? list.bias_tab[global_order ? (bias_q & 127u) : (within < 96u ? within : 95u)] : 0u;
+        const uint32_t qblock = global_order ? bias_q : (biased ? ((id + 8u - jb.xcd_rot) & 7u) + 8u * (e & kBiasQlMask) : ((id + 8u - jb.xcd_rot) & 7u) + 8u * (within / jb.splits));
+        const uint32_t split = global_order ? bias_k : (biased ? 0u : within % jb.splits);
+        int32_t* r = rows + 3 * (size_t)id;
+        r[0] = -1; r[1] = r[2] = 0;
+        if (qblock >= jb.qblocks || (global_order && split >= jb.splits) || (biased && !global_order && within >= (jb.qblocks >> 3) * jb.splits)) continue;
+        uint32_t s0 = std::min(split * jb.t_per_split, jb.nt), s1 = std::min(s0 + jb.t_per_split, jb.nt);
+        if (biased && !global_order) {
+            s0 = std::min(((e >> kBiasBeginShift) & kBiasBeginMask) * 32u, jb.nt);
+            s1 = std::min(s0 + (e >> kBiasSizeShift) * 32u, jb.nt);
+        }
+        if (global_order) {
+            const uint32_t n0 = e & 0xFFu, n1 = (e >> 8) & 0xFFu, c = (e >> 16) & 0xFFu, extra = e >> 24;
+            const uint32_t k0 = std::min(split, n0), k1 = std::min(split - k0, n1), k2 = split - k0 - k1;
+            const uint32_t begin = k0 * jb.bias_a + k1 * jb.bias_b + k2 * c + std::min(k2, extra);
+            const uint32_t size = split < n0 ? jb.bias_a : (split < n0 + n1 ? jb.bias_b : c + (k2 < extra ? 1u : 0u));
+            s0 = std::min(begin * 32u, jb.nt);
+            s1 = split + 1u == jb.splits ? jb.nt : std::min(s0 + size * 32u, jb.nt);
+        }
+        r[0] = (int32_t)qblock; r[1] = (int32_t)(s0 >> 5); r[2] = (int32_t)((s1 - s0 + 31u) >> 5);
+    }
+    return (int)grid_x;
+}
+
 hipError_t launch_k2nn(const K2nnJobDev* jobs, int njobs, uint2* d_partial, hipStream_t stream, Profiler* prof, int formulation,
                        uint64_t* d_stamps, bool probe)
 {
@@ -639,49 +724,8 @@
         while (cnt < kK2nnJobsPerLaunch && base + cnt < njobs && jobs[base + cnt].rule == jobs[base].rule) ++cnt;
         const bool ratio = jobs[base].rule == K2NN_RULE_RATIO;
         K2nnJobList list;
-        uint32_t grid_x = 0, max_nq = 0, max_nq_empty = 0;
-        for (int j = 0; j < cnt; ++j) {
-            list.j[j] = jobs[base + j];
-            const uint32_t qb = formulation == K2NN_POPCOUNT ? list.j[j].qblocks : ((list.j[j].qblocks + 7u) & ~7u);
-            const uint32_t gx = list.j[j].nt ? qb * list.j[j].splits : 0u;
-            if (gx > grid_x) grid_x = gx;
-            if (list.j[j].nq > max_nq) max_nq = list.j[j].nq;
-            if (list.j[j].nt == 0u && list.j[j].nq > max_nq_empty) max_nq_empty = list.j[j].nq;
-        }
-        for (int j = cnt; j < kK2nnJobsPerLaunch; ++j) list.j[j] = K2nnJobDev{};
-        for (uint32_t& e : list.bias_tab) e = 0u;
-        if (cnt == 1 && list.j[0].bias_a != 0u && list.j[0].bias_magic != 0u && formulation != K2NN_POPCOUNT) {
-            const K2nnJobDev& jb = list.j[0];
-            const uint32_t QB = jb.qblocks, nt_tiles = (jb.nt + 31u) >> 5;
-            for (uint32_t q = 0; q < QB && q < 128u; ++q) {
-                const uint32_t n0 = std::min((jb.slot_wgs - q + QB - 1u) / QB, jb.splits);
-                const uint32_t n1 = std::min((2u * jb.slot_wgs - q + QB - 1u) / QB, jb.splits) - n0;
-                const uint32_t n2 = jb.splits - n0 - n1;
-                const uint32_t used = n0 * jb.bias_a + n1 * jb.bias_b;
-                const uint32_t rest = nt_tiles > used ? nt_tiles - used : 0u;
-                const uint32_t c = n2 ? rest / n2 : 0u, extra = n2 ? rest - c * n2 : 0u;
-                list.bias_tab[q] = n0 | (n1 << 8) | (std::min(c, 255u) << 16) | (std::min(extra, 255u) << 24);
-            }
-            grid_x = QB * jb.splits;
-        } else
-        if (cnt == 1 && list.j[0].bias_a != 0u && formulation != K2NN_POPCOUNT) {
-            const K2nnJobDev& jb = list.j[0];
-            const uint32_t nqx = jb.qblocks >> 3, nt_tiles = (jb.nt + 31u) >> 5;
-            for (uint32_t w = 0; w < nqx * jb.splits && w < 96u; ++w) {
-                const uint32_t ql = w % nqx, k = w / nqx;
-                const uint32_t n0 = std::min((jb.slot_wgs - ql + nqx - 1u) / nqx, jb.splits);
-                const uint32_t n1 = std::min((2u * jb.slot_wgs - ql + nqx - 1u) / nqx, jb.splits) - n0;
-                const uint32_t n2 = jb.splits - n0 - n1;
-                const uint32_t used = n0 * jb.bias_a + n1 * jb.bias_b;
-                const uint32_t rest = nt_tiles > used ? nt_tiles - used : 0u;
-                const uint32_t c = n2 ? rest / n2 : 0u, extra = n2 ? rest - c * n2 : 0u;
-                const uint32_t k0 = std::min(k, n0), k1 = std::min(k - k0, n1), k2 = k - k0 - k1;
-                const uint32_t begin = k0 * jb.bias_a + k1 * jb.bias_b + k2 * c + std::min(k2, extra);
-                uint32_t size = k < n0 ? jb.bias_a : (k < n0 + n1 ? jb.bias_b : c + (k2 < extra ? 1u : 0u));
-                if (k + 1u == jb.splits) size = nt_tiles > begin ? nt_tiles - begin : 0u;
-                list.bias_tab[w] = (ql & kBiasQlMask) | (std::min(begin, kBiasBeginMask) << kBiasBeginShift) | (std::min(size, kBiasSizeMax) << kBiasSizeShift);
-            }
-        }
+        uint32_t grid_x, max_nq, max_nq_empty;
+        k2nn_fill_list(list, jobs + base, cnt, formulation, grid_x, max_nq, max_nq_empty);
         if (max_nq == 0) continue;
         if (grid_x > 0) {
             prof_mark(prof, CLC_KERNEL_K2NN_SWEEP, true, stream);
diff --git a/include/coloc_hip.h b/include/coloc_hip.h
--- a/include/coloc_hip.h
+++ b/include/coloc_hip.h
@@ -147,6 +147,7 @@
 int clc_k2nn_set_formulation(clc_ctx* ctx, int formulation);
 int clc_k2nn_queries_per_block(const clc_ctx* ctx);
 int clc_k2nn_plan_query(const clc_ctx* ctx, int nq, int nt, int32_t* info);
+int clc_k2nn_plan_table(const clc_ctx* ctx, int nq, int nt, int32_t* rows, int cap);
 int clc_k2nn_device_info(const clc_ctx* ctx, int32_t* info, float* probe_us);
 
 int clc_k2nn_clock_check(clc_ctx* ctx, const void* d_q, int nq, const void* d_t, int nt, int32_t* d_match, void* stream,
```

Measured after the change: 1.264 million, median of 6. No clear change (+0.7%).
